# cbs228/sameold

Hardware: AMD Instinct MI355X
Metric: Msamples/s demodulated (batched 22.05 kHz channels) + % HBM roofline, 1/8 GPU (higher is better)
Workload: dtype f32

## Files before the change

sameold_amd/csrc/same_batch.cpp:

```cpp
#include <hip/hip_runtime.h>

#include <algorithm>
#include <chrono>
#include <cstdarg>
#include <cstdio>
#include <cstdlib>
#include <condition_variable>
#include <cstring>
#include <deque>
#include <functional>
#include <mutex>
#include <new>
#include <string>
#include <thread>
#include <utility>
#include <vector>

#include "../../include/same_rx.h"
#include "same_config.h"
#include "same_device.h"
#include "same_hipmem.h"
#include "same_launch.h"
#include "same_resets.h"
#include "same_transport.h"

namespace {

thread_local std::string g_last_error;

int fail(int code, const char *fmt, ...)
{
    char buf[512];
    va_list ap;
    va_start(ap, fmt);
    vsnprintf(buf, sizeof(buf), fmt, ap);
    va_end(ap);
    g_last_error = buf;
    return code;
}

#define HIP_TRY(expr)                                                                      \
    do {                                                                                   \
        hipError_t _e = (expr);                                                            \
        if (_e != hipSuccess)                                                              \
            return fail(SAME_EHIP, "%s failed: %s (%s:%d)", #expr, hipGetErrorString(_e),  \
                        __FILE__, __LINE__);                                               \
    } while (0)

}

struct QEvent {
    uint32_t kind, channel;
    uint64_t sample_counter, symbol_count;
    uint32_t len, aux, aux2;
    uint32_t n_bytes;
    uint64_t payload;
};
static_assert(sizeof(QEvent) == 48, "compact event record");
template <typename T>
struct PodQueue {
    T *buf = nullptr;
    size_t n = 0, cap = 0;
    size_t base = 0;
    ~PodQueue() { std::free(buf); }
    PodQueue() = default;
    PodQueue(const PodQueue &) = delete;
    PodQueue &operator=(const PodQueue &) = delete;
    size_t size() const { return n; }
    T *data() { return buf; }
    const T *data() const { return buf; }
    void clear() { base += n; n = 0; }
    size_t compact(size_t head)
    {
        if (head == 0) return 0;
        if (head < n) std::memmove(buf, buf + head, (n - head) * sizeof(T));
        n -= head;
        base += head;
        return 0;
    }
    T *grow(size_t extra)
    {
        if (n + extra > cap) {
            const size_t want = (n + extra) + (n + extra) / 2 + 64;
            void *p = std::realloc(buf, want * sizeof(T));
            if (!p) return nullptr;
            buf = static_cast<T *>(p);
            cap = want;
        }
        T *at = buf + n;
        n += extra;
        return at;
    }
};
using EventQueue = PodQueue<QEvent>;
struct AudioChunk {
    uint32_t channel, flags;
    uint64_t sample_counter, n;
    uint64_t at;
};
using ByteArena = PodQueue<uint8_t>;
#ifdef SAME_HOST_PROF
#include <x86intrin.h>
static uint64_t g_hp[8];
static const char *const g_hp_name[8] = {"range sort", "poll synthesis", "queue record + payload", "transport: burst", "transport: other", "after_event", "stitch scan", "-"};
struct HpScope { int k; uint64_t t0; explicit HpScope(int k_) : k(k_), t0(__rdtsc()) {} ~HpScope() { g_hp[k] += __rdtsc() - t0; } };
#define HP(k) HpScope hp_scope_##k(k)
#else
#define HP(k) do {} while (0)
#endif
struct HarvestPart {
    std::vector<QEvent> out;
    std::vector<uint8_t> bytes;
    std::vector<uint32_t> rearm;
    std::vector<uint32_t> bursts;
};
static void materialise(const QEvent &q, const uint8_t *arena, size_t arena_base, same_rx_event *ev)
{
    std::memset(ev, 0, sizeof(*ev));
    ev->kind = q.kind; ev->channel = q.channel; ev->sample_counter = q.sample_counter; ev->symbol_count = q.symbol_count;
    ev->len = q.len; ev->aux = q.aux; ev->aux2 = q.aux2;
    if (q.n_bytes) std::memcpy(ev->bytes, arena + (q.payload - arena_base), q.n_bytes);
}

using same::TickSynth;

class WorkerPool {
public:
    ~WorkerPool()
    {
        { std::lock_guard<std::mutex> g(mu_); stop_ = true; }
        cv_.notify_all();
        for (std::thread &t : threads_) t.join();
    }
    void run(size_t n, const std::function<void(size_t)> &fn)
    {
        if (n <= 1) { if (n) fn(0); return; }
        while (threads_.size() + 1 < n) threads_.emplace_back([this] { loop(); });
        {
            std::lock_guard<std::mutex> g(mu_);
            fn_ = &fn; next_ = 0; count_ = n; pending_ = n; ++generation_;
        }
        cv_.notify_all();
        work();
        std::unique_lock<std::mutex> lk(mu_);
        done_.wait(lk, [this] { return pending_ == 0; });
        fn_ = nullptr;
    }

private:
    void work()
    {
        for (;;) {
            size_t i;
            const std::function<void(size_t)> *fn;
            {
                std::lock_guard<std::mutex> g(mu_);
                if (!fn_ || next_ >= count_) return;
                i = next_++; fn = fn_;
            }
            (*fn)(i);
            std::lock_guard<std::mutex> g(mu_);
            if (--pending_ == 0) done_.notify_all();
        }
    }
    void loop()
    {
        uint64_t seen = 0;
        for (;;) {
            {
                std::unique_lock<std::mutex> lk(mu_);
                cv_.wait(lk, [&] { return stop_ || generation_ != seen; });
                if (stop_) return;
                seen = generation_;
            }
            work();
        }
    }
    std::vector<std::thread> threads_;
    std::mutex mu_;
    std::condition_variable cv_, done_;
    const std::function<void(size_t)> *fn_ = nullptr;
    size_t next_ = 0, count_ = 0, pending_ = 0;
    uint64_t generation_ = 0;
    bool stop_ = false;
};

struct same_batch {
    same_rx_builder builder{};
    same::Params P{};
    same::State S{};
    int device = 0;
    uint32_t flags = 0;
    uint64_t counter = 0;
    hipStream_t own_stream = nullptr;
    hipStream_t last_stream = nullptr;
    same::DevBuf<float4> d_taps;
    same::DevBuf<void> d_state_blob;
    struct Slot {
        same::DevBuf<same::DevEvent> d_events;
        uint32_t event_cap() const { return (uint32_t)d_events.size(); }
        same::DevBuf<uint32_t> d_sort;
        same::PinnedBuf<uint32_t> h_sort;
        same::DevBuf<same::DevEvent> d_sorted;
        uint32_t sort_bins = 0;
        same::DevBuf<uint8_t> d_bursts;
        uint32_t burst_cap() const { return (uint32_t)(d_bursts.size() / same::kBurstCap); }
        same::DevBuf<uint32_t> d_counters;
        same::MappedBuf<uint32_t> h_counters;
        same::Event ev_start, ev_stop, ev_done, ev_planned;
        same::Event ev_k0, ev_k1;
        bool have_k = false;
        bool timed = false;
        same::PinnedBuf<void> h_events, h_bursts;
        bool in_flight = false;
        uint64_t seq = 0;
        uint64_t end_counter = 0;
        bool chunked = false;
        same::ChunkGeom geom{};
        uint64_t end_blocks = 0;
        same::DevBuf<uint64_t> d_handover;
        same::PinnedBuf<uint64_t> h_handover;
        bool per_channel = false;
        same::DevBuf<uint32_t> d_geom;
        same::PinnedBuf<uint32_t> h_geom;
        same::CoherentBuf<uint32_t> h_reset;
        same::CoherentBuf<uint32_t> h_counts;
        same::PinnedBuf<uint64_t> h_wake_up;
        bool dev_transport = false;
        same::CoherentBuf<same::DevMessage> h_near;
        uint32_t near_cap() const { return (uint32_t)h_near.size(); }
        same::DevBuf<same::DevMessage> d_msgs;
        uint32_t msg_cap() const { return (uint32_t)d_msgs.size(); }
        same::PinnedBuf<void> h_msgs;
        bool captured = false;
        same::DevBuf<same::cap::Span> d_spans;
        uint32_t span_cap() const { return (uint32_t)d_spans.size(); }
        same::DevBuf<float> d_pool;
        same::DevBuf<same::cap::Cursors> d_cap_cur;
        same::MappedBuf<same::cap::Cursors> h_cap_cur;
        same::PinnedBuf<void> h_spans, h_pool;
    } slot[2];
    struct TimePar {
        bool enabled = false;
        uint32_t max_chunks = 0, min_own = 0, warmup = 0;
        uint32_t cap_columns = 0;
        uint32_t carved_columns = 0;
        int carved_family = -1;
        same::Params Pv{};
        same::State Sv{};
        same::DevBuf<void> blob;
        same::DevBuf<void> blob_fresh;
        size_t fresh_bytes = 0;
        same::DevBuf<same::StateArrayDesc> d_desc_in, d_desc_out;
        uint32_t n_desc = 0;
        same::DevBuf<uint32_t> d_final_col;
        same::DevBuf<float> d_energy;
        same::DevBuf<float> d_hist;
        same::Event ev_plan_prev; bool plan_recorded = false;
        int knob_plan_stream = 0;
        int sort_mode = -1;
        uint32_t last_chunks = 1;
        bool last_per_channel = false;
        same::Family family = same::Family::kPipe;
        int knob_prologue = 0;
        std::vector<int64_t> sym_off;
        std::vector<TickSynth> synth;
    } tp;
    uint64_t launch_seq = 0;
    hipStream_t copy_stream = nullptr;
    struct Windowed {
        bool on = false;
        uint32_t window = 0;
        uint32_t fill = 0;
        same::DevBuf<void> d_buf;
        same::Event ev_buf;
        hipStream_t buf_stream = nullptr; bool buf_used = false;
        same::Event ev_read[2];
        uint64_t n_reads = 0;
        hipStream_t read_stream = nullptr;
    } inv;
    hipStream_t plan_stream = nullptr;
    float last_ms = 0.0f;
    bool overflowed = false;
    std::string record_path;
    bool kernel_fault = false;
    same::Request want;
    same::Mode mode;
    same::Choice plain;
    same::Params Pfm{};
    same::Family last_family = same::Family::kGeneric;
    bool sym_launched = false;
    bool debug = false;
    int host_threads = 0;
    same::DevBuf<void> d_stage, d_stage2;
    same::DevBuf<void> d_upload;
    same::DevBuf<void> d_zero;
    same::Event ev_order;
    bool timing = false;
    bool have_timing = false;
    float last_demod_ms = 0.0f;
    EventQueue queue;
    size_t queue_head = 0;
    ByteArena arena;
    std::vector<same_rx_event> peeked;
    bool peeked_valid = false;
    bool peeked_release = false;
    size_t peeked_head = 0;
    std::vector<size_t> burst_seq;
    size_t burst_seq_head = 0;
    std::vector<HarvestPart> parts;
    WorkerPool workers;
    std::vector<same::TransportHot> thot;
    std::vector<same::TransportCold> tcold;
    same::TransportRef tr(uint32_t c) { return same::TransportRef(thot[c], tcold[c]); }
    same::PinnedBuf<uint64_t> h_wake;
    bool wake_ordered = false;
    std::vector<uint32_t> ragged_by;
    bool messages_only = false;
    bool dev_transport = false;
    bool last_dev_transport = false;
    same::DevBuf<void> d_thot, d_tcold;
    same::ResetLedger resets;
    std::vector<uint32_t> reset_list, reset_now, reset_cols;
    struct Audio {
        size_t per_launch = 0;
        same::DevBuf<same::cap::Rec> d_rec;
        std::vector<uint8_t> open;
        uint64_t flush_at = UINT64_MAX;
        PodQueue<AudioChunk> queue;
        size_t head = 0;
        PodQueue<float> samples;
        std::vector<same_audio_chunk> view;
    } audio;
};

static void release_stale_view(same_batch *rx);

namespace {

struct Carver {
    size_t off = 0;
    template <typename T> size_t take(size_t n)
    {
        off = (off + 255) & ~size_t(255);
        size_t o = off;
        off += n * sizeof(T);
        return o;
    }
};

#define SAME_STATE_ARRAYS(X, P)                                                                            \
    X(dc_ff_ring, float, (P).dc_len) X(dc_fb_ring, float, (P).dc_len)                                        \
    X(dc_sum0, float, 1) X(dc_sum1, float, 1) X(agc_gain, float, 1)                                          \
    X(win_ring, float, (P).win_ring)                                                                         \
    X(ted_clock, uint32_t, 1) X(until_next_ted, float, 1)                                                    \
    X(ted_h0, float, 1) X(ted_h1, float, 1) X(ted_h2, float, 1)                                              \
    X(period_avg, float, 1) X(period_inst, float, 1)                                                         \
    X(sq_data, uint32_t, 1) X(sq_power, float, 1) X(sq_phist, uint32_t, 1)                                   \
    X(sq_fill, uint32_t, 1) X(sq_clock, int32_t, 1) X(sq_symbols, uint64_t, 1)                               \
    X(sq_hist, float, same::kSquelchHist)                                                                    \
    X(eq_ffc, float, (P).eq_nff) X(eq_fbc, float, (P).eq_nfb)                                                \
    X(eq_ffw, float, (P).eq_nff) X(eq_fbw, float, (P).eq_nfb)                                                \
    X(eq_word, uint32_t, 1) X(eq_count, uint32_t, 1)                                                         \
    X(eq_snap_ffc, float, (P).eq_nff) X(eq_snap_fbc, float, (P).eq_nfb)                                      \
    X(eq_snap_ffw, float, (P).eq_nff) X(eq_snap_fbw, float, (P).eq_nfb)                                      \
    X(fr_word, uint32_t, 1) X(fr_count, uint32_t, 1) X(fr_invalid, uint32_t, 1) X(fr_len, uint32_t, 1)       \
    X(flags, uint32_t, 1)                                                                                    \
    X(tk_next, uint64_t, 1) X(tk_last, uint64_t, 1) X(tk_ring, uint64_t, same::kTickRing)                    \
    X(tk_n, uint32_t, 1) X(wake_sample, uint64_t, 1) X(wake_fired, uint64_t, 1)

size_t carve_state(const same::Params &P, char *base, same::State &S)
{
    const size_t C = P.n_channels;
    Carver cv;
#define CARVE(field, type, count) \
    do { size_t o = cv.take<type>(count); if (base) S.field = reinterpret_cast<type *>(base + o); } while (0)
#define CARVE_ROWS(field, type, rows) CARVE(field, type, (size_t)(rows) * C);
    SAME_STATE_ARRAYS(CARVE_ROWS, P)
#undef CARVE_ROWS
    CARVE(fr_msg, uint8_t, (size_t)same::kBurstCap * C);
    if (P.trace_cap) {
        CARVE(trace_n, uint32_t, C);
        CARVE(trace, float, (size_t)P.trace_cap * 4 * C);
        CARVE(trace_idx, uint64_t, (size_t)P.trace_cap * C);
    }
#undef CARVE
    return (cv.off + 255) & ~size_t(255);
}

void list_state_arrays(const same::Params &P, const same::State &src, const same::State &dst,
                       std::vector<same::StateArrayDesc> &out)
{
    out.clear();
#define DESC_ROWS(field, type, rows)                                                                     \
    out.push_back(same::StateArrayDesc{reinterpret_cast<char *>(src.field), reinterpret_cast<char *>(dst.field), \
                                       (uint32_t)(rows), (uint32_t)(sizeof(type) / 4)});
    SAME_STATE_ARRAYS(DESC_ROWS, P)
#undef DESC_ROWS
    static_assert(same::kBurstCap % 4 == 0, "framer rows are copied in words");
    out.push_back(same::StateArrayDesc{reinterpret_cast<char *>(src.fr_msg), reinterpret_cast<char *>(dst.fr_msg), 1u,
                                       (uint32_t)(same::kBurstCap / 4)});
}

void read_knobs(same_batch *rx)
{
    auto num = [](const char *name, int unset) { const char *e = std::getenv(name); return e ? std::atoi(e) : unset; };
    auto tri = [](const char *name) { const char *e = std::getenv(name); return e ? (std::atoi(e) ? 1 : -1) : 0; };
    rx->P.knob_pipe = tri("SAME_PIPE");
    rx->P.knob_pipe_lanes = num("SAME_PIPE_LANES", 0);
    rx->P.knob_pipe_split = tri("SAME_PIPE_SPLIT");
#ifdef SAME_PROFILE
    rx->P.knob_mirror = tri("SAME_MIRROR");
    rx->P.knob_pipe_share = tri("SAME_PIPE_SHARE");
    rx->P.knob_prio = num("SAME_PIPE_PRIO", 0);
#endif
    rx->P.knob_fast_dense = tri("SAME_FAST_DENSE");
    rx->P.knob_sym = tri("SAME_SYM");
    rx->want.sym_max_channels = (uint32_t)std::max(0, num("SAME_SYM_MAX", 1 << 30));
    rx->debug = std::getenv("SAME_DEBUG") != nullptr;
    { const char *e = std::getenv("SAME_RECORD_HARVEST"); rx->record_path = e ? e : ""; }
    rx->host_threads = std::max(0, num("SAME_HOST_THREADS", 0));
    rx->tp.sort_mode = num("SAME_TP_SORT", -1);
    rx->tp.knob_plan_stream = tri("SAME_TP_PLAN_STREAM");
    rx->tp.knob_prologue = tri("SAME_TP_PROLOGUE");
    rx->want.knob_relaxed = tri("SAME_RELAXED");
    { const char *e = std::getenv("SAME_RELAXED_KERNEL"); rx->P.knob_relaxed_kernel = !e ? 0 : (std::strcmp(e, "solo") == 0 ? 1 : (std::strcmp(e, "duo") == 0 ? 2 : 0)); }
    { const char *e = std::getenv("SAME_TP_KERNEL"); rx->want.knob_tp_kernel = !e ? 0 : (std::strcmp(e, "wave") == 0 ? 2 : (std::strcmp(e, "pipe") == 0 ? 1 : 0)); }
}

int ensure_output(same_batch *rx, same_batch::Slot &sl, size_t n_samples, same::Output &O, size_t n_columns = 0)
{
    const size_t n_ch = n_columns ? n_columns : rx->P.n_channels;
    const double symbols = (double)n_samples * 520.83 / (double)rx->P.input_rate;
    const size_t per_chan_events = (size_t)(symbols / 8.0) + 16;
    const size_t per_chan_bursts = (size_t)(symbols / 160.0) + 4;
    size_t ecap = std::min<size_t>(per_chan_events * n_ch, 0x7fffffffu / sizeof(same::DevEvent));
    size_t bcap = std::min<size_t>(per_chan_bursts * n_ch, 0x7fffffffu / same::kBurstCap);
    HIP_TRY(sl.d_events.ensure(ecap));
    HIP_TRY(sl.d_bursts.ensure(bcap * same::kBurstCap));
    if (rx->dev_transport && !n_columns) {
        HIP_TRY(sl.d_msgs.ensure(std::min<size_t>(bcap + 2 * n_ch, 0x7fffffffu / sizeof(same::DevMessage))));
        if (!sl.h_near) HIP_TRY(sl.h_near.ensure(std::max<uint32_t>(4096u, (uint32_t)(n_ch / 4u))));
        if (rx->audio.per_launch)
            HIP_TRY(sl.d_spans.ensure(std::min<size_t>(n_ch + (size_t)sl.near_cap() + sl.msg_cap(), 0x7fffffffu / sizeof(same::cap::Span))));
    }
    HIP_TRY(sl.d_sorted.ensure(sl.d_events.size()));
    HIP_TRY(sl.d_sort.ensure(2 * n_ch + 1 + same::event_sort_extra_words((uint32_t)n_ch)));
    HIP_TRY(sl.h_sort.ensure(n_ch + 1));
    sl.sort_bins = (uint32_t)n_ch;
    O.events = sl.d_events; O.event_cap = sl.event_cap();
    O.bursts = sl.d_bursts; O.burst_cap = sl.burst_cap();
    O.n_events = sl.d_counters; O.n_bursts = sl.d_counters + 1; O.overflow = sl.d_counters + 2;
    return SAME_OK;
}

template <typename SampleT>
hipError_t launch_family(same::Family f, const same::Params &P, const same::State &S, const same::Output &O, const float4 *taps, const SampleT *x,
                         uint32_t n_blocks, uint64_t counter0, hipStream_t stream, const same::PipeChunks &pc = same::PipeChunks{})
{
    switch (f) {
    case same::Family::kSym: return same::launch_demod_sym(P, S, O, taps, x, n_blocks, counter0, stream, pc);
    case same::Family::kPipeFastmath: return same::launch_demod_pipe(P, S, O, taps, x, n_blocks, counter0, stream, pc, true);
    case same::Family::kPipe: return same::launch_demod_pipe(P, S, O, taps, x, n_blocks, counter0, stream, pc, false);
    case same::Family::kWaveRelaxed: return same::launch_demod_relaxed(P, S, O, taps, x, n_blocks, counter0, stream, pc);
    case same::Family::kFast: return same::launch_demod_fast(P, S, O, taps, x, n_blocks, counter0, stream);
    case same::Family::kGeneric: break;
    }
    return hipErrorInvalidValue;
}

void reset_channel_host(same_batch *rx, uint32_t c, uint64_t pos)
{
    if (!rx->thot.empty()) rx->tr(c).reset();
    if (rx->tp.enabled) {
        rx->tp.sym_off[c] = 0;
        rx->tp.synth[c].reset();
        rx->tp.synth[c].a_t = pos;
    }
    if (rx->h_wake) rx->h_wake[c] = 0;
}

int launch_pending_resets(same_batch *rx, same_batch::Slot &sl, hipStream_t stream)
{
    if (rx->resets.device.empty()) return SAME_OK;
    std::vector<uint32_t> &cols = rx->reset_cols;
    rx->resets.take_device(cols);
    const uint32_t n = (uint32_t)cols.size();
    if (n > sl.h_reset.size()) HIP_TRY(sl.h_reset.ensure(std::max<uint32_t>(256u, n + n / 2u)));
    std::memcpy(sl.h_reset, cols.data(), (size_t)n * sizeof(uint32_t));
    hipError_t e = same::launch_reset_columns(rx->P, rx->S, sl.h_reset.dev(), n, stream);
    if (e == hipSuccess && rx->dev_transport)
        e = same::launch_transport_reset(rx->d_thot, rx->d_tcold, rx->P.n_channels, sl.h_reset.dev(), n, 0, stream, rx->audio.d_rec);
    if (e != hipSuccess) return fail(SAME_EHIP, "channel reset launch failed: %s", hipGetErrorString(e));
    return SAME_OK;
}

void prepare_queue_append(same_batch *rx)
{
    rx->peeked_valid = false;
    release_stale_view(rx);
    if (rx->queue_head && rx->queue_head >= rx->queue.size() - rx->queue_head) {
        rx->queue_head = rx->queue.compact(rx->queue_head);
        size_t keep_from = rx->arena.base + rx->arena.size();
        for (size_t i = 0; i < rx->queue.size(); ++i)
            if (rx->queue.data()[i].n_bytes) { keep_from = (size_t)rx->queue.data()[i].payload; break; }
        rx->arena.compact(keep_from - rx->arena.base);
    }
}

struct HarvestTimes { std::chrono::steady_clock::time_point sorted, replayed; uint32_t n_threads = 1; };
struct HarvestInput {
    const uint32_t *first;
    same::DevEvent *events;
    const uint8_t *bursts;
    const uint64_t *handover;
    const uint32_t *geom;
};
int harvest_host(same_batch *rx, same_batch::Slot &sl, const HarvestInput &in, uint32_t n_events, uint32_t n_bursts, std::vector<uint32_t> &rearm,
                 HarvestTimes &times)
{
    const bool dbg = rx->debug;
    const same::DevEvent *evs = in.events;
    const uint8_t *bursts = in.bursts;
    const uint32_t n_ch = rx->P.n_channels;
    const uint32_t n_bins = sl.chunked ? sl.geom.n_chunks * n_ch : n_ch;
    std::vector<uint32_t> first(in.first, in.first + n_bins + 1u);
    same::DevEvent *evs_mut = in.events;
    const uint32_t n_real = first[n_bins];
    if (n_real > n_events) return fail(SAME_EHIP, "internal: event sort counted %u of %u events", n_real, n_events);
    struct Identity { uint32_t operator[](uint32_t i) const { return i; } } order;
    if (dbg && sl.chunked && sl.per_channel) {
        const same::ChunkGeom &g = sl.geom;
        const uint32_t *own = in.geom, *rows = in.geom + n_bins;
        double len_sum = 0, run_sum = 0; uint64_t len_max = 0, run_max = 0, n_len = 0, n_run = 0, n_inf = 0, n_late = 0;
        uint32_t worst_c = 0;
        for (uint32_t k = 0; k + 1u < g.n_chunks; ++k)
            for (uint32_t c = 0; c < n_ch; ++c) {
                const uint64_t end = own[(size_t)(k + 1u) * n_ch + c], len = end - rows[(size_t)k * n_ch + c];
                len_sum += (double)len; if (len > len_max) { len_max = len; worst_c = c; } ++n_len;
                const uint64_t h = in.handover[(size_t)k * n_ch + c];
                if (h == same::kNoHandover) { ++n_inf; continue; }
                const uint64_t run = h - g.counter0 > end ? h - g.counter0 - end : 0;
                run_sum += (double)run; run_max = std::max(run_max, run); ++n_run; n_late += run > 2u * g.block_len;
            }
        std::fprintf(stderr, "[same] longest piece on channel %u, its cuts:", worst_c);
        for (uint32_t k = 0; k < g.n_chunks; ++k) std::fprintf(stderr, " %u", own[(size_t)k * n_ch + worst_c]);
        std::fprintf(stderr, "\n");
        std::fprintf(stderr, "[same] per-channel chunks: length mean %.0f max %llu samples; run-on mean %.0f max %llu, %llu of %llu columns ran on "
                             "more than two blocks, %llu never handed over\n", len_sum / std::max<uint64_t>(n_len, 1), (unsigned long long)len_max,
                     run_sum / std::max<uint64_t>(n_run, 1), (unsigned long long)run_max, (unsigned long long)n_late, (unsigned long long)n_run,
                     (unsigned long long)n_inf);
    }
    std::vector<uint32_t> chan_first;
    if (sl.chunked) {
        chan_first.assign(n_ch + 1u, 0u);
        for (uint32_t k = 0; k < sl.geom.n_chunks; ++k)
            for (uint32_t c = 0; c < n_ch; ++c) chan_first[c + 1u] += first[k * n_ch + c + 1u] - first[k * n_ch + c];
        for (uint32_t c = 0; c < n_ch; ++c) chan_first[c + 1u] += chan_first[c];
    }
    const std::vector<uint32_t> &cfirst = sl.chunked ? chan_first : first;
    const bool link_only = (rx->flags & SAME_BATCH_LINK_ONLY) != 0;
    const bool tp = rx->tp.enabled;
    times.sorted = std::chrono::steady_clock::now();

    using Part = HarvestPart;
    const double sps = (double)rx->P.input_rate / 520.83;
    const uint64_t interburst = same::max_interburst_symbols(), history = same::max_history_duration();
    const bool msgs_only = rx->messages_only;
    auto push_transport = [&](Part &part, const same_rx_event &tev, uint32_t c) {
        if (msgs_only && tev.kind != SAME_TRANSPORT_MSG_START && tev.kind != SAME_TRANSPORT_MSG_END) return;
        QEvent q{};
        q.kind = tev.kind; q.channel = c; q.sample_counter = rx->resets.rebase(c, tev.sample_counter); q.symbol_count = tev.symbol_count;
        q.len = tev.len; q.aux = tev.aux; q.aux2 = tev.aux2;
        q.n_bytes = std::min<uint32_t>(tev.len, SAME_EVENT_MAX_BYTES);
        if (tev.kind != SAME_TRANSPORT_MSG_START) q.n_bytes = 0;
        q.payload = part.bytes.size();
        if (q.n_bytes) part.bytes.insert(part.bytes.end(), tev.bytes, tev.bytes + q.n_bytes);
        part.out.push_back(q);
    };
    auto feed = [&](Part &part, same_rx_event &tev, const same::DevEvent &d, uint32_t c, int64_t off) {
        const uint64_t sym = (uint64_t)((int64_t)d.symbol_count + off);
        auto poll = [&](uint64_t psym, uint64_t pt) {
            if (rx->tr(c).on_link_event(same::kDevTick, pt, psym, nullptr, 0, rx->P.input_rate, &tev)) push_transport(part, tev, c);
        };
        if (tp && !link_only) {
            HP(1);
            rx->tp.synth[c].run_until(sym, d.sample_counter, sps, rx->tr(c).force_eom_at(), poll);
        }
        QEvent q{};
        const uint8_t *payload = nullptr;
        {
        HP(2);
        q.kind = d.kind; q.channel = c; q.sample_counter = rx->resets.rebase(c, d.sample_counter); q.symbol_count = sym;
        if (d.kind == SAME_LINK_BURST) {
            q.len = d.burst_len;
            if (d.burst_slot < n_bursts) {
                q.n_bytes = std::min<uint32_t>(d.burst_len, SAME_EVENT_MAX_BYTES);
                payload = bursts + (size_t)d.burst_slot * same::kBurstCap;
                q.payload = part.bytes.size();
                if (!msgs_only) part.bytes.insert(part.bytes.end(), payload, payload + q.n_bytes);
            } else {
                q.len = 0;
            }
            if (!msgs_only) part.bursts.push_back((uint32_t)part.out.size());
        }
        if (d.kind <= SAME_LINK_BURST && !msgs_only) part.out.push_back(q);
        }
        if (!link_only) {
#ifdef SAME_HOST_PROF
            HpScope hp_tr(d.kind == SAME_LINK_BURST ? 3 : 4);
#endif
            if (rx->tr(c).on_link_event(d.kind, d.sample_counter, sym, payload, q.n_bytes, rx->P.input_rate, &tev)) push_transport(part, tev, c);
            if (!tp && rx->tr(c).force_eom_dirty()) part.rearm.push_back(c);
        }
        { HP(5); if (tp && d.kind <= SAME_LINK_BURST) rx->tp.synth[c].after_event(d.kind, sym, d.sample_counter, interburst, history); }
    };
    auto stitch = [&](Part &part, same_rx_event &ev, uint32_t c) {
        const same::ChunkGeom &g = sl.geom;
        const uint64_t *hand = in.handover;
        const uint32_t *own = sl.per_channel ? in.geom : nullptr, *rows = sl.per_channel ? in.geom + n_bins : nullptr;
        auto owner_of = [&](uint64_t h) -> uint32_t {
            if (!own) return g.owner_of(h);
            uint32_t k = 0;
            while (k + 1u < g.n_chunks && g.counter0 + own[(size_t)(k + 1u) * n_ch + c] <= h) ++k;
            return k;
        };
        TickSynth &ts = rx->tp.synth[c];
        int64_t off = rx->tp.sym_off[c];
        uint32_t cur = 0;
        uint64_t keep_after = 0;
        for (;;) {
            const uint32_t col = cur * n_ch + c;
            const uint64_t h = hand[col];
            const uint64_t upto = std::min(h, sl.end_blocks);
            bool rebased = cur == 0;
            for (uint32_t i = first[col]; i < first[col + 1u]; ++i) {
                const same::DevEvent &d = evs[order[i]];
                if (d.sample_counter <= keep_after) continue;
                if (d.sample_counter > upto) break;
                if (!rebased) {
                    const int64_t est = (int64_t)ts.a_sym + (int64_t)((double)(d.sample_counter - ts.a_t) / sps + 0.5);
                    off = est - (int64_t)d.symbol_count;
                    rebased = true;
                }
                feed(part, ev, d, c, off);
            }
            if (!rebased) {
                const uint64_t row0 = rows ? g.counter0 + rows[col] : g.counter0 + (uint64_t)cur * g.stride_blocks * g.block_len;
                const int64_t est_end = (int64_t)ts.a_sym + (int64_t)((double)(sl.end_blocks - ts.a_t) / sps + 0.5);
                off = est_end - (int64_t)((double)(sl.end_blocks - row0) / sps + 0.5);
            }
            if (h == same::kNoHandover) break;
            const uint32_t nxt = owner_of(h);
            if (nxt <= cur) break;
            const uint32_t ncol = nxt * n_ch + c;
            uint32_t st = 0, j = first[ncol];
            for (; j < first[ncol + 1u] && evs[order[j]].sample_counter <= h; ++j)
                if (evs[order[j]].kind <= SAME_LINK_BURST) st = evs[order[j]].kind;
            keep_after = h;
            if (st == SAME_LINK_READING || st == SAME_LINK_BURST) {
                for (; j < first[ncol + 1u]; ++j)
                    if (evs[order[j]].kind == SAME_LINK_NO_CARRIER) { keep_after = evs[order[j]].sample_counter; break; }
            } else if (st == SAME_LINK_SEARCHING && ts.link == SAME_LINK_NO_CARRIER) {
                same::DevEvent inj{};
                inj.channel = ncol; inj.kind = SAME_LINK_SEARCHING; inj.sample_counter = h;
                inj.symbol_count = ts.a_sym + (uint64_t)((double)(h > ts.a_t ? h - ts.a_t : 0) / sps + 0.5);
                inj.burst_slot = 0xffffffffu;
                feed(part, ev, inj, c, 0);
            }
            cur = nxt;
        }
        for (uint32_t i = first[c]; i < first[c + 1u]; ++i)
            if (evs[order[i]].sample_counter > sl.end_blocks) feed(part, ev, evs[order[i]], c, off);
        rx->tp.sym_off[c] = off;
    };
    auto run_range = [&](uint32_t c0, uint32_t c1, Part &part) {
        part.out.clear(); part.bytes.clear(); part.rearm.clear(); part.bursts.clear();
        part.out.reserve((size_t)(cfirst[c1] - cfirst[c0]) * 3 / 2 + 4);
        same_rx_event ev;
        std::memset(&ev, 0, sizeof(ev));
        for (uint32_t c = c0; c < c1; ++c) {
            if (!link_only && c + 1u < c1) {
                __builtin_prefetch(&rx->thot[c + 1u]);
                if (!sl.chunked) {
                    bool burst = false;
                    for (uint32_t k = first[c + 1u]; k < first[c + 2u]; ++k) burst |= evs[k].kind == SAME_LINK_BURST;
                    const char *nx = reinterpret_cast<const char *>(&rx->tcold[c + 1u]);
                    if (burst) for (size_t o = 0; o < sizeof(same::TransportCold); o += 64) __builtin_prefetch(nx + o);
                }
            }
            { HP(0);
            for (uint32_t col = c; col < n_bins; col += n_ch)
                if (first[col + 1u] - first[col] > 1u)
                    std::sort(evs_mut + first[col], evs_mut + first[col + 1u],
                              [](const same::DevEvent &a, const same::DevEvent &b) { return a.channel < b.channel; });
            }
            if (sl.chunked) stitch(part, ev, c);
            else
                for (uint32_t k = first[c]; k < first[c + 1u]; ++k)
                    feed(part, ev, evs[order[k]], c, tp ? rx->tp.sym_off[c] : 0);
            if (tp && !link_only) {
                TickSynth &ts = rx->tp.synth[c];
                if (ts.link == SAME_LINK_NO_CARRIER && sl.end_counter > ts.a_t) {
                    const uint64_t sym_end = ts.a_sym + (uint64_t)((double)(sl.end_counter - ts.a_t) / sps);
                    auto poll = [&](uint64_t psym, uint64_t pt) {
                        if (rx->tr(c).on_link_event(same::kDevTick, pt, psym, nullptr, 0, rx->P.input_rate, &ev)) push_transport(part, ev, c);
                    };
                    ts.run_until(sym_end + 1u, sl.end_counter + 1u, sps, rx->tr(c).force_eom_at(), poll);
                }
            }
        }
    };
    uint32_t n_threads = 1;
    if (n_real >= 16384u && n_ch >= 64u) {
        const unsigned hw = std::thread::hardware_concurrency();
        n_threads = std::min<uint32_t>({32u, std::max(16u, hw / 8u), hw ? hw : 1u, n_ch / 32u});
        if (rx->host_threads > 0) n_threads = (uint32_t)rx->host_threads;
    }
    if (rx->parts.size() < n_threads) rx->parts.resize(n_threads);
    std::vector<Part> &parts = rx->parts;
    for (Part &p : parts) { p.out.clear(); p.bytes.clear(); p.rearm.clear(); p.bursts.clear(); }
    if (n_threads == 1) {
        run_range(0, n_ch, parts[0]);
    } else {
        std::vector<uint32_t> cut(n_threads + 1u, n_ch);
        cut[0] = 0;
        for (uint32_t t = 1; t < n_threads; ++t) {
            const uint32_t target = (uint32_t)((uint64_t)n_real * t / n_threads);
            cut[t] = (uint32_t)(std::lower_bound(cfirst.begin(), cfirst.end(), target) - cfirst.begin());
            cut[t] = std::min(std::max(cut[t], cut[t - 1u]), n_ch);
        }
        rx->workers.run(n_threads, [&](size_t t) { run_range(cut[t], cut[t + 1u], parts[t]); });
    }
    times.replayed = std::chrono::steady_clock::now();
    times.n_threads = n_threads;
    size_t total = 0, total_bytes = 0;
    for (const Part &p : parts) { total += p.out.size(); total_bytes += p.bytes.size(); }
    prepare_queue_append(rx);
    QEvent *dst = rx->queue.grow(total);
    if (total && !dst) return fail(SAME_ENOMEM, "event queue");
    uint8_t *bdst = rx->arena.grow(total_bytes);
    if (total_bytes && !bdst) return fail(SAME_ENOMEM, "event payloads");
    {
        size_t at = 0, bat = 0;
        if (rx->burst_seq_head > 4096 && rx->burst_seq_head * 2 > rx->burst_seq.size()) {
            rx->burst_seq.erase(rx->burst_seq.begin(), rx->burst_seq.begin() + (std::ptrdiff_t)rx->burst_seq_head);
            rx->burst_seq_head = 0;
        }
        const size_t seq0 = rx->queue.base + (size_t)(dst - rx->queue.data());
        const size_t byte0 = rx->arena.base + (size_t)(bdst - rx->arena.data());
        struct Job { QEvent *q; uint8_t *b; Part *p; size_t byte_off; };
        std::vector<Job> jobs;
        for (size_t t = 0; t < parts.size(); ++t) {
            Part &p = parts[t];
            if (p.out.empty()) continue;
            for (uint32_t i : p.bursts) rx->burst_seq.push_back(seq0 + at + i);
            jobs.push_back(Job{dst + at, bdst + bat, &p, byte0 + bat});
            at += p.out.size(); bat += p.bytes.size();
        }
        rx->workers.run(jobs.size(), [&](size_t j) {
            const Job &job = jobs[j];
            for (QEvent &q : job.p->out) q.payload += job.byte_off;
            std::memcpy(job.q, job.p->out.data(), job.p->out.size() * sizeof(QEvent));
            if (!job.p->bytes.empty()) std::memcpy(job.b, job.p->bytes.data(), job.p->bytes.size());
// ... 46 lines not shown
        const uint64_t keep_from = A.queue.size() ? A.queue.data()[0].at : A.samples.base + A.samples.size();
        A.samples.compact((size_t)(keep_from - A.samples.base));
    }
    AudioChunk *dst = A.queue.grow(n_chunks);
    if (n_chunks && !dst) return nullptr;
    float *sdst = A.samples.grow(n_samples);
    if (n_samples && !sdst) { A.queue.n -= n_chunks; return nullptr; }
    *samples_at = sdst;
    *at = A.samples.base + (A.samples.size() - n_samples);
    return dst;
}

int audio_end_reset(same_batch *rx, const std::vector<uint32_t> &chans, uint64_t pos)
{
    same_batch::Audio &A = rx->audio;
    if (!A.per_launch) return SAME_OK;
    size_t n = 0;
    for (uint32_t c : chans) n += A.open[c];
    if (!n) return SAME_OK;
    float *sdst = nullptr;
    uint64_t at = 0;
    AudioChunk *dst = audio_grow(rx, n, 0, &sdst, &at);
    if (!dst) return fail(SAME_ENOMEM, "audio queue");
    for (uint32_t c : chans) {
        if (!A.open[c]) continue;
        *dst++ = AudioChunk{c, SAME_AUDIO_END_RESET, rx->resets.rebase(c, pos), 0, at};
        A.open[c] = 0;
    }
    return SAME_OK;
}

int harvest_audio(same_batch *rx, same_batch::Slot &sl)
{
    sl.captured = false;
    same_batch::Audio &A = rx->audio;
    const same::cap::Cursors cur = *sl.h_cap_cur.get();
    if (cur.overflow) rx->overflowed = true;
    const uint32_t n_spans = std::min(cur.n_spans, sl.span_cap());
    if (!n_spans) return SAME_OK;
    const size_t used = (size_t)std::min<unsigned long long>(cur.pool_used, (unsigned long long)A.per_launch);
    HIP_TRY(grow_pinned(sl.h_spans, (size_t)n_spans * sizeof(same::cap::Span)));
    HIP_TRY(hipMemcpyAsync(sl.h_spans, sl.d_spans, (size_t)n_spans * sizeof(same::cap::Span), hipMemcpyDeviceToHost, rx->copy_stream));
    if (used) {
        HIP_TRY(grow_pinned(sl.h_pool, used * sizeof(float)));
        HIP_TRY(hipMemcpyAsync(sl.h_pool, sl.d_pool, used * sizeof(float), hipMemcpyDeviceToHost, rx->copy_stream));
    }
    HIP_TRY(hipStreamSynchronize(rx->copy_stream));
    const same::cap::Span *sp = static_cast<const same::cap::Span *>(sl.h_spans.get());
    const float *pool = static_cast<const float *>(sl.h_pool.get());
    std::vector<uint32_t> order(n_spans);
    size_t n_samples = 0;
    for (uint32_t i = 0; i < n_spans; ++i) {
        order[i] = i;
        if (sp[i].n && sp[i].off + sp[i].n <= used) n_samples += sp[i].n;
    }
    std::sort(order.begin(), order.end(), [&](uint32_t a, uint32_t b) { return sp[a].channel != sp[b].channel ? sp[a].channel < sp[b].channel : a < b; });
    float *sdst = nullptr;
    uint64_t at = 0;
    AudioChunk *dst = audio_grow(rx, n_spans, n_samples, &sdst, &at);
    if (!dst) return fail(SAME_ENOMEM, "audio queue");
    for (uint32_t k = 0; k < n_spans; ++k) {
        const same::cap::Span &s = sp[order[k]];
        const uint32_t n = s.n && s.off + s.n <= used ? s.n : 0;
        uint32_t flags = s.flags;
        if (n < s.n) flags |= SAME_AUDIO_TRUNCATED;
        dst[k] = AudioChunk{s.channel, flags, rx->resets.rebase(s.channel, s.counter), n, at};
        if (n) { std::memcpy(sdst, pool + s.off, (size_t)n * sizeof(float)); sdst += n; at += n; }
        if (flags & SAME_AUDIO_FIRST) A.open[s.channel] = 1;
        if (flags & (SAME_AUDIO_END_MESSAGE | SAME_AUDIO_END_FLUSH | SAME_AUDIO_END_RESET)) A.open[s.channel] = 0;
    }
    if (rx->debug)
        std::fprintf(stderr, "[same] audio: %u chunks, %zu samples (pool %zu of %zu)%s\n", n_spans, n_samples, used, A.per_launch,
                     cur.overflow ? ", truncated" : "");
    return SAME_OK;
}

int harvest_messages(same_batch *rx, same_batch::Slot &sl, std::chrono::steady_clock::time_point t_begin,
                     std::chrono::steady_clock::time_point t_waited)
{
    const uint32_t n_msgs = std::min(sl.h_counters[3], sl.near_cap() + sl.msg_cap());
    const uint32_t n_near = std::min(n_msgs, sl.near_cap()), n_far = n_msgs - n_near;
    const size_t far_bytes = (size_t)n_far * sizeof(same::DevMessage);
    if (n_far) {
        HIP_TRY(grow_pinned(sl.h_msgs, far_bytes));
        HIP_TRY(hipMemcpyAsync(sl.h_msgs, sl.d_msgs, far_bytes, hipMemcpyDeviceToHost, rx->copy_stream));
        HIP_TRY(hipStreamSynchronize(rx->copy_stream));
    }
    auto t_copied = std::chrono::steady_clock::now();
    const same::DevMessage *far = static_cast<const same::DevMessage *>(sl.h_msgs.get());
    auto rec = [&](uint32_t i) -> const same::DevMessage & { return i < n_near ? sl.h_near[i] : far[i - n_near]; };
    std::vector<uint32_t> order(n_msgs);
    size_t n_bytes = 0;
    for (uint32_t i = 0; i < n_msgs; ++i) {
        order[i] = i;
        if (rec(i).kind == SAME_TRANSPORT_MSG_START) n_bytes += std::min<uint32_t>(rec(i).len, same::kDevMessageText);
    }
    std::sort(order.begin(), order.end(), [&](uint32_t a, uint32_t b) {
        const same::DevMessage &x = rec(a), &y = rec(b);
        return x.channel != y.channel ? x.channel < y.channel : x.seq < y.seq;
    });
    prepare_queue_append(rx);
    QEvent *dst = rx->queue.grow(n_msgs);
    if (n_msgs && !dst) return fail(SAME_ENOMEM, "event queue");
    uint8_t *bdst = rx->arena.grow(n_bytes);
    if (n_bytes && !bdst) return fail(SAME_ENOMEM, "event payloads");
    size_t at = n_bytes ? rx->arena.base + (size_t)(bdst - rx->arena.data()) : 0;
    for (uint32_t k = 0; k < n_msgs; ++k) {
        const same::DevMessage &d = rec(order[k]);
        QEvent q{};
        q.kind = d.kind; q.channel = d.channel; q.sample_counter = rx->resets.rebase(d.channel, d.sample_counter);
        q.symbol_count = d.symbol_count; q.len = d.len; q.aux = d.aux; q.aux2 = d.aux2;
        if (d.kind == SAME_TRANSPORT_MSG_START && d.len) {
            q.n_bytes = std::min<uint32_t>(d.len, same::kDevMessageText);
            q.payload = at;
            std::memcpy(bdst, d.text, q.n_bytes);
            bdst += q.n_bytes; at += q.n_bytes;
        }
        dst[k] = q;
    }
    if (sl.captured) {
        const int arc = harvest_audio(rx, sl);
        if (arc) return arc;
    }
    const int si = (int)(&sl - rx->slot);
    rx->resets.shift_due(si);
    rx->resets.done_shift(si);
    if (const int arc = audio_end_reset(rx, rx->resets.slot[si & 1].channels, rx->resets.rec_pos(si))) return arc;
    for (uint32_t c : rx->resets.host_due(si)) reset_channel_host(rx, c, rx->resets.rec_pos(si));
    rx->resets.done_host(si);
    if (rx->debug) {
        auto t_end = std::chrono::steady_clock::now();
        auto ms = [](auto a, auto b) { return std::chrono::duration<double, std::milli>(b - a).count(); };
        std::fprintf(stderr, "[same] harvest timing: wait %.2f ms, copy %.2f ms, %u messages queued in %.2f ms (transport layer on the device)\n",
                     ms(t_begin, t_waited), ms(t_waited, t_copied), n_msgs, ms(t_copied, t_end));
    }
    return SAME_OK;
}

int upload_wake_ordered(same_batch *rx, same_batch::Slot &sl)
{
    const uint32_t C = rx->P.n_channels;
    HIP_TRY(sl.h_wake_up.ensure(C));
    same_batch::Slot &other = rx->slot[(&sl - rx->slot) ^ 1];
    const int oi = (int)(&other - rx->slot);
    for (uint32_t c = 0; c < C; ++c) {
        const uint64_t w = rx->h_wake[c];
        sl.h_wake_up[c] = w && other.in_flight ? w + rx->resets.pending_shift(oi, c) : w;
    }
    if (other.in_flight) {
        HIP_TRY(hipMemcpyAsync(rx->S.wake_sample, sl.h_wake_up, (size_t)C * sizeof(uint64_t), hipMemcpyHostToDevice, rx->last_stream));
        HIP_TRY(hipEventRecord(other.ev_done, rx->last_stream));
    } else {
        HIP_TRY(hipMemcpyAsync(rx->S.wake_sample, sl.h_wake_up, (size_t)C * sizeof(uint64_t), hipMemcpyHostToDevice, rx->copy_stream));
        HIP_TRY(hipStreamSynchronize(rx->copy_stream));
    }
    return SAME_OK;
}

int harvest_slot(same_batch *rx, same_batch::Slot &sl)
{
    if (!sl.in_flight) return SAME_OK;
    const bool dbg = rx->debug;
    auto t_begin = std::chrono::steady_clock::now();
    HIP_TRY(hipEventSynchronize(sl.ev_done));
    sl.in_flight = false;
    if (sl.timed) {
        HIP_TRY(hipEventElapsedTime(&rx->last_ms, sl.ev_start, sl.ev_stop));
        rx->last_demod_ms = rx->last_ms;
        if (sl.have_k) HIP_TRY(hipEventElapsedTime(&rx->last_demod_ms, sl.ev_k0, sl.ev_k1));
        rx->have_timing = true;
    }
    auto t_waited = std::chrono::steady_clock::now();
    const uint32_t n_events = std::min(sl.h_counters[0], sl.event_cap());
    if (dbg)
        std::fprintf(stderr, "[same] harvest: %u device events (%u bursts), cap %u/%u\n", sl.h_counters[0],
                     sl.h_counters[1], sl.event_cap(), sl.burst_cap());
    const uint32_t n_bursts = std::min(sl.h_counters[1], sl.burst_cap());
    if (sl.h_counters[2] & (3u | same::kMessageLogOverflow)) rx->overflowed = true;
    if (sl.h_counters[2] & 4u) rx->kernel_fault = true;
    if (sl.dev_transport) return harvest_messages(rx, sl, t_begin, t_waited);
    const size_t ev_bytes = (size_t)n_events * sizeof(same::DevEvent), bu_bytes = (size_t)n_bursts * same::kBurstCap;
    HIP_TRY(grow_pinned(sl.h_events, ev_bytes));
    HIP_TRY(grow_pinned(sl.h_bursts, bu_bytes));
    const uint32_t n_ch = rx->P.n_channels;
    const uint32_t n_bins = sl.chunked ? sl.geom.n_chunks * n_ch : n_ch;
    if (n_bins != sl.sort_bins) return fail(SAME_EINVAL, "internal: event sort made for %u columns, launch has %u", sl.sort_bins, n_bins);
    HIP_TRY(hipMemcpyAsync(sl.h_sort, sl.d_sort + n_bins, ((size_t)n_bins + 1) * sizeof(uint32_t), hipMemcpyDeviceToHost, rx->copy_stream));
    if (n_events) HIP_TRY(hipMemcpyAsync(sl.h_events, sl.d_sorted, ev_bytes, hipMemcpyDeviceToHost, rx->copy_stream));
    HIP_TRY(hipStreamSynchronize(rx->copy_stream));
    if (n_bursts) HIP_TRY(hipMemcpyAsync(sl.h_bursts, sl.d_bursts, bu_bytes, hipMemcpyDeviceToHost, rx->copy_stream));
    if (sl.chunked) {
        HIP_TRY(hipMemcpyAsync(sl.h_handover, sl.d_handover, (size_t)n_bins * sizeof(uint64_t), hipMemcpyDeviceToHost, rx->copy_stream));
        if (sl.per_channel)
            HIP_TRY(hipMemcpyAsync(sl.h_geom, sl.d_geom, (size_t)2 * n_bins * sizeof(uint32_t), hipMemcpyDeviceToHost, rx->copy_stream));
    }
    if (n_bursts || sl.chunked) HIP_TRY(hipStreamSynchronize(rx->copy_stream));
    auto t_copied = std::chrono::steady_clock::now();
    if (!rx->record_path.empty()) { const int rrc = record_harvest(rx, sl, n_events, n_bursts, rx->record_path.c_str()); if (rrc != SAME_OK) return rrc; }
    std::vector<uint32_t> rearm;
    HarvestTimes times;
    const HarvestInput in{sl.h_sort, static_cast<same::DevEvent *>(sl.h_events.get()), static_cast<const uint8_t *>(sl.h_bursts.get()),
                          sl.h_handover, sl.h_geom};
    int rc = harvest_host(rx, sl, in, n_events, n_bursts, rearm, times);
    if (rc) return rc;
    {
        const int si = (int)(&sl - rx->slot);
        const same::ResetLedger::SlotShift &sh = rx->resets.shift_due(si);
        if (!rx->thot.empty())
            for (size_t i = 0; i < sh.channels.size(); ++i)
                if (rx->tr(sh.channels[i]).shift_force_eom(sh.by[i])) rearm.push_back(sh.channels[i]);
        rx->resets.done_shift(si);
    }
    {
        const int si = (int)(&sl - rx->slot);
        const std::vector<uint32_t> &due = rx->resets.host_due(si);
        for (uint32_t c : due) reset_channel_host(rx, c, rx->resets.rec_pos(si));
        rx->resets.done_host(si);
    }
    if (!rearm.empty()) {
        if (!rx->h_wake) {
            HIP_TRY(rx->h_wake.ensure(rx->P.n_channels));
            std::memset(rx->h_wake, 0, (size_t)rx->P.n_channels * sizeof(uint64_t));
        }
        for (uint32_t c : rearm) rx->h_wake[c] = rx->tr(c).force_eom_at();
        if (rx->wake_ordered) {
            int rc2 = upload_wake_ordered(rx, sl);
            if (rc2) return rc2;
        } else {
        HIP_TRY(hipMemcpyAsync(rx->S.wake_sample, rx->h_wake, (size_t)rx->P.n_channels * sizeof(uint64_t), hipMemcpyHostToDevice, rx->copy_stream));
        HIP_TRY(hipStreamSynchronize(rx->copy_stream));
        }
    }
    if (dbg) {
        auto t_end = std::chrono::steady_clock::now();
        auto ms = [](auto a, auto b) { return std::chrono::duration<double, std::milli>(b - a).count(); };
        std::fprintf(stderr, "[same] harvest timing: wait %.2f ms, copy %.2f ms, sort %.2f ms, replay on %u threads %.2f ms, "
                             "queue %.2f ms\n",
                     ms(t_begin, t_waited), ms(t_waited, t_copied), ms(t_copied, times.sorted), times.n_threads,
                     ms(times.sorted, times.replayed), ms(times.replayed, t_end));
    }
    return SAME_OK;
}

int harvest(same_batch *rx)
{
    same_batch::Slot *order[2] = {&rx->slot[0], &rx->slot[1]};
    if (order[0]->seq > order[1]->seq) std::swap(order[0], order[1]);
    for (same_batch::Slot *sl : order) {
        int rc = harvest_slot(rx, *sl);
        if (rc) return rc;
    }
    return SAME_OK;
}

uint32_t plan_chunks(same_batch *rx, size_t n, same::ChunkGeom &geom, same::PipeChunks &pc, uint32_t column_cap = same::kTpColumnCap, bool channel_major = false)
{
    same_batch::TimePar &tp = rx->tp;
    const uint32_t C = rx->P.n_channels;
    const double sps = (double)rx->P.input_rate / 520.83;
    auto fill = [&](uint32_t K, uint32_t fb) -> bool {
        const uint32_t warm = tp.warmup ? tp.warmup : (uint32_t)(64.0 * sps + 0.5);
        const uint32_t WB = (warm + fb - 1u) / fb;
        const uint64_t TB = n / fb;
        if (TB <= WB) return false;
        const uint64_t SB = (TB - WB) / K;
        const uint64_t min_own = tp.min_own ? tp.min_own : 4ull * WB * fb;
        if (SB == 0 || SB * fb < min_own) return false;
        geom.counter0 = rx->counter;
        geom.n_chunks = K; geom.block_len = fb; geom.stride_blocks = (uint32_t)SB; geom.warmup_blocks = WB;
        pc.n_chunks = K; pc.in_channels = C; pc.stride_blocks = (uint32_t)SB; pc.nominal_blocks = (uint32_t)SB + WB;
        pc.handover = nullptr;
        return true;
    };
    const same::TpRule rule = same::tp_rule(rx->P, rx->mode, rx->want, tp.max_chunks, column_cap, channel_major);
    for (uint32_t K = rule.k_max; K >= 2u; --K) {
        same::Choice c;
        if (same::tp_candidate(rx->P, rule, K, c) && fill(K, c.block_len)) { tp.family = c.family; return K; }
    }
    return 1;
}

int ensure_handover(same_batch::Slot &sl, uint32_t columns)
{
    HIP_TRY(sl.d_handover.ensure(columns));
    HIP_TRY(sl.h_handover.ensure(columns));
    return SAME_OK;
}

int ensure_wide_state(same_batch *rx, uint32_t columns)
{
    same_batch::TimePar &tp = rx->tp;
    if (tp.carved_columns == columns && tp.carved_family == (int)tp.family) return SAME_OK;
    int rc = harvest(rx);
    if (rc) return rc;
    HIP_TRY(hipDeviceSynchronize());
    tp.Pv = same::wide_params(rx->P, columns, same::is_fastmath(tp.family), same::tp_more_than_one_round(columns));
    if (columns > tp.cap_columns) {
        tp.cap_columns = 0;
        HIP_TRY(tp.blob.reset());
        HIP_TRY(tp.blob_fresh.reset());
        const size_t bytes = carve_state(tp.Pv, nullptr, tp.Sv);
        HIP_TRY(tp.blob.ensure(bytes));
        HIP_TRY(hipMemset(tp.blob, 0, bytes));
        HIP_TRY(tp.blob_fresh.ensure(bytes));
        tp.cap_columns = columns;
    }
    const size_t blob_bytes = carve_state(tp.Pv, (char *)tp.blob.get(), tp.Sv);
    {
        same::State Sf{};
        carve_state(tp.Pv, (char *)tp.blob_fresh.get(), Sf);
        HIP_TRY(hipMemset(tp.blob_fresh, 0, blob_bytes));
        HIP_TRY(same::launch_init_state(tp.Pv, Sf, 0, nullptr, 0));
        HIP_TRY(hipDeviceSynchronize());
        tp.fresh_bytes = (size_t)(reinterpret_cast<char *>(tp.Sv.fr_msg) - static_cast<char *>(tp.blob.get()));
    }
    std::vector<same::StateArrayDesc> in, out;
    list_state_arrays(rx->P, rx->S, tp.Sv, in);
    list_state_arrays(rx->P, tp.Sv, rx->S, out);
    tp.n_desc = (uint32_t)in.size();
    HIP_TRY(tp.d_desc_in.ensure(in.size()));
    HIP_TRY(tp.d_desc_out.ensure(out.size()));
    HIP_TRY(tp.d_final_col.ensure(rx->P.n_channels));
    HIP_TRY(hipMemcpy(tp.d_desc_in, in.data(), in.size() * sizeof(same::StateArrayDesc), hipMemcpyHostToDevice));
    HIP_TRY(hipMemcpy(tp.d_desc_out, out.data(), out.size() * sizeof(same::StateArrayDesc), hipMemcpyHostToDevice));
    tp.carved_columns = columns;
    tp.carved_family = (int)tp.family;
    return SAME_OK;
}

struct Ragged {
    const uint32_t *counts = nullptr;
    uint32_t m = 0;
    uint32_t row_off = 0;
};

struct RaggedLaunch {
    uint32_t row0 = 0;
    size_t n_lock = 0;
};


int begin_launch(same_batch *rx, same_batch::Slot &sl, const same_batch::Slot &prev, hipStream_t stream)
{
    int rc = harvest_slot(rx, sl);
    if (rc) return rc;
    if (prev.in_flight && rx->last_stream != stream) HIP_TRY(hipStreamWaitEvent(stream, prev.ev_done, 0));
    return launch_pending_resets(rx, sl, stream);
}

int begin_timing(same_batch *rx, same_batch::Slot &sl, hipStream_t stream)
{
    sl.timed = rx->timing;
    if (sl.timed) HIP_TRY(hipEventRecord(sl.ev_start, stream));
    return SAME_OK;
}

int tp_reserve(same_batch *rx, same_batch::Slot &sl, uint32_t columns, size_t n, const same::PipeChunks &pc, uint32_t block_len, same::Output &O)
{
    int rc = ensure_wide_state(rx, columns);
    if (rc) return rc;
    rc = ensure_output(rx, sl, std::min<size_t>(n, 3 * (size_t)pc.nominal_blocks * block_len + 65536), O, columns);
    if (rc) return rc;
    return ensure_handover(sl, columns);
}

int tp_start(same_batch *rx, same_batch::Slot &sl, uint32_t columns, const char *layout, hipStream_t stream, bool *sort_bins_empty)
{
    same_batch::TimePar &tp = rx->tp;
    const uint32_t C = rx->P.n_channels;
    *sort_bins_empty = false;
    if (tp.knob_prologue >= 0) {
        HIP_TRY(same::launch_tp_prologue(tp.blob, tp.blob_fresh, tp.fresh_bytes, sl.d_handover, sl.d_sort, columns, sl.d_counters, stream));
        *sort_bins_empty = sl.sort_bins == columns;
    } else {
        HIP_TRY(same::launch_counters(sl.d_counters, sl.h_counters.dev(), 0, stream));
        HIP_TRY(same::launch_init_state(tp.Pv, tp.Sv, 0, stream, C));
        HIP_TRY(same::launch_fill_u64(sl.d_handover, columns, same::kNoHandover, stream));
    }
    if (rx->debug) std::fprintf(stderr, "[same] time-parallel launch: %u columns (%s), start-up: %s\n", columns, layout,
                                tp.knob_prologue >= 0 ? "prologue kernel" : "separate launches");
    HIP_TRY(same::launch_copy_state_columns(tp.d_desc_in, tp.n_desc, C, columns, nullptr, C, stream));
    return SAME_OK;
}

int tp_hand_back(same_batch *rx, same_batch::Slot &sl, const same::ChunkGeom &geom, const uint32_t *own_start, hipStream_t stream)
{
    same_batch::TimePar &tp = rx->tp;
    const uint32_t C = rx->P.n_channels;
    if (own_start) HIP_TRY(same::launch_chunk_final_column_pc(sl.d_handover, own_start, C, geom.n_chunks, rx->counter, tp.d_final_col, stream));
    else HIP_TRY(same::launch_chunk_final_column(sl.d_handover, C, geom, tp.d_final_col, stream));
    HIP_TRY(same::launch_copy_state_columns(tp.d_desc_out, tp.n_desc, geom.n_chunks * C, C, tp.d_final_col, C, stream));
    return SAME_OK;
}

template <typename SampleT>
int demod_tail(same_batch *rx, const same::Output &O, const SampleT *rows, size_t n, uint64_t counter0, hipStream_t stream)
{
    const hipError_t e = same::launch_demod(rx->P, rx->S, O, rx->d_taps, rows, (uint32_t)n, counter0, stream);
    if (e != hipSuccess) return fail(SAME_EHIP, "demod kernel launch failed: %s", hipGetErrorString(e));
    return SAME_OK;
}
int demod_tail_corner(same_batch *rx, const same::Output &O, const float *corner, size_t pitch, size_t r, uint64_t counter0, hipStream_t stream)
{
    const uint32_t C = rx->P.n_channels;
    HIP_TRY(rx->d_stage.ensure(r * C * sizeof(float)));
    HIP_TRY(rx->d_stage2.ensure(r * C * sizeof(float)));
    float *staged = static_cast<float *>(rx->d_stage.get()), *rows = static_cast<float *>(rx->d_stage2.get());
    HIP_TRY(hipMemcpy2DAsync(staged, r * sizeof(float), corner, pitch * sizeof(float), r * sizeof(float), C, hipMemcpyDeviceToDevice, stream));
    const hipError_t e = same::launch_transpose(staged, rows, C, (uint32_t)r, stream);
    if (e != hipSuccess) return fail(SAME_EHIP, "demod kernel launch failed: %s", hipGetErrorString(e));
    return demod_tail(rx, O, rows, r, counter0, stream);
}

template <typename SampleT>
int end_launch(same_batch *rx, same_batch::Slot &sl, same_batch::Slot &prev, hipStream_t stream, const SampleT *rows, size_t n,
               bool sort_bins_empty, const RaggedLaunch *rl = nullptr)
{
    if (sl.timed) HIP_TRY(hipEventRecord(sl.ev_stop, stream));
    HIP_TRY(same::launch_event_sort(sl.d_events, sl.d_counters, sl.event_cap(), sl.sort_bins, sl.d_sort, sl.d_sort + sl.sort_bins,
                                    sl.d_sorted, stream, sort_bins_empty));
    sl.dev_transport = rx->dev_transport && !sl.chunked;
    rx->last_dev_transport = sl.dev_transport;
    if (sl.dev_transport) {
        same::TransportLaunch T{};
        T.n_channels = rx->P.n_channels; T.input_rate = rx->P.input_rate;
        T.first = sl.d_sort + sl.sort_bins; T.sorted = sl.d_sorted; T.counters = sl.d_counters;
        T.bursts = sl.d_bursts; T.burst_cap = sl.burst_cap();
        T.hot = rx->d_thot; T.cold = rx->d_tcold; T.wake_sample = rx->S.wake_sample;
        T.near = sl.h_near.dev(); T.near_cap = sl.near_cap();
        T.log = sl.d_msgs; T.log_cap = sl.msg_cap(); T.log_cursor = sl.d_counters + 3; T.overflow = sl.d_counters + 2;
        sl.captured = rx->audio.per_launch != 0;
        if (sl.captured) {
            same::cap::Launch &K = T.cap;
            const uint64_t fa = rx->audio.flush_at;
            K.start = rx->counter; K.n_rows = (uint32_t)n;
            K.flush_row = fa >= rx->counter + n ? same::cap::kNoFlush : (uint32_t)(fa > rx->counter ? fa - rx->counter : 0);
            K.rec = rx->audio.d_rec; K.spans = sl.d_spans; K.span_cap = sl.span_cap();
            K.n_spans = &sl.d_cap_cur->n_spans; K.pool_used = &sl.d_cap_cur->pool_used; K.pool_cap = rx->audio.per_launch;
            K.overflow = &sl.d_cap_cur->overflow;
        }
        if (rl && rl->n_lock < n)
            HIP_TRY(same::launch_transport_ragged(T, sl.h_counts.dev(), rl->row0, (uint32_t)n, stream));
        else
            HIP_TRY(same::launch_transport(T, stream));
        if (sl.captured) {
            const hipError_t e = same::launch_capture(sl.d_spans, sl.d_cap_cur, sl.span_cap(), sl.d_pool, rx->audio.per_launch, rows,
                                                      rx->P.n_channels, (uint32_t)n, sl.h_cap_cur.dev(), stream);
            if (e != hipSuccess) return fail(SAME_EHIP, "capture kernel launch failed: %s", hipGetErrorString(e));
        }
    }
    HIP_TRY(same::launch_counters(sl.d_counters, sl.h_counters.dev(), 1, stream));
    HIP_TRY(hipEventRecord(sl.ev_done, stream));
    sl.in_flight = true;
    sl.seq = ++rx->launch_seq;
    rx->last_stream = stream;
    if (rl) rx->resets.shift(rx->ragged_by.data(), rx->counter + n, (int)(&sl - rx->slot));
    rx->counter += n;
    sl.end_counter = rx->counter;
    return harvest_slot(rx, prev);
}

template <typename SampleT>
int process_time_major_launches(same_batch *rx, const SampleT *d_x, size_t n_samples, hipStream_t stream, const Ragged *rg = nullptr)
{
    const size_t kMaxChunk = std::min<size_t>((size_t)1 << 22, (size_t)rx->P.input_rate * 45);
    size_t done = 0;
    while (done < n_samples) {
        const size_t n = std::min(kMaxChunk, n_samples - done);
        same_batch::Slot &sl = rx->slot[rx->launch_seq & 1];
        same_batch::Slot &prev = rx->slot[(rx->launch_seq & 1) ^ 1];
        int rc = begin_launch(rx, sl, prev, stream);
        if (rc) return rc;
        size_t n_lock = n;
        if (rg) {
            const size_t row0 = (size_t)rg->row_off + done;
            n_lock = rg->m > row0 ? std::min<size_t>(rg->m - row0, n) : 0;
            const uint32_t C = rx->P.n_channels;
            HIP_TRY(sl.h_counts.ensure(C));
            std::memcpy(sl.h_counts, rg->counts, (size_t)C * sizeof(uint32_t));
            rx->ragged_by.resize(C);
            for (uint32_t c = 0; c < C; ++c) {
                const size_t have = rg->counts[c] > row0 ? std::min<size_t>(rg->counts[c] - row0, n) : 0;
                rx->ragged_by[c] = (uint32_t)(n - have);
            }
        }
        same::ChunkGeom geom{};
        same::PipeChunks pc{};
        const uint32_t n_chunks = rg ? 1u : plan_chunks(rx, n, geom, pc);
        rx->tp.last_chunks = n_chunks;
        sl.have_k = false;
        bool sort_bins_empty = false;
        same::Output O{};
        if (n_chunks > 1u) {
            const uint32_t C = rx->P.n_channels, columns = n_chunks * C;
            const size_t fbk = geom.block_len;
            rc = tp_reserve(rx, sl, columns, n, pc, geom.block_len, O);
            if (rc) return rc;
            pc.handover = sl.d_handover;
            same_batch::TimePar &tp = rx->tp;
            rc = begin_timing(rx, sl, stream);
            if (rc) return rc;
            rc = tp_start(rx, sl, columns, "time-major", stream, &sort_bins_empty);
            if (rc) return rc;
            const SampleT *xp = d_x + done * C;
            const uint32_t total_blocks = (uint32_t)(n / fbk);
            const hipError_t e = launch_family(tp.family, tp.Pv, tp.Sv, O, rx->d_taps, xp, total_blocks, rx->counter, stream, pc);
            rx->last_family = tp.family;
            if (e != hipSuccess) return fail(SAME_EHIP, "time-parallel demod kernel launch failed: %s", hipGetErrorString(e));
            rc = tp_hand_back(rx, sl, geom, nullptr, stream);
            if (rc) return rc;
            const size_t n_whole = (size_t)total_blocks * fbk;
            if (n_whole < n && (rc = demod_tail(rx, O, xp + n_whole * C, n - n_whole, rx->counter + n_whole, stream)) != SAME_OK) return rc;
            sl.chunked = true; sl.per_channel = false;
            sl.geom = geom;
            sl.end_blocks = rx->counter + n_whole;
            rx->tp.last_per_channel = false;
        } else {
        sl.chunked = false; sl.per_channel = false;
        rc = ensure_output(rx, sl, n, O);
        if (rc) return rc;
        HIP_TRY(same::launch_counters(sl.d_counters, sl.h_counters.dev(), 0, stream));
        rc = begin_timing(rx, sl, stream);
        if (rc) return rc;
        const SampleT *xp = d_x + done * rx->P.n_channels;
        hipError_t e = hipSuccess;
        const same::Choice &plain = rx->plain;
        const size_t fb = plain.block_len;
        const size_t n_fast = fb ? (n_lock / fb) * fb : 0;
        if (n_fast) {
            e = launch_family(plain.family, same::is_fastmath(plain.family) ? rx->Pfm : rx->P, rx->S, O, rx->d_taps, xp, (uint32_t)(n_fast / fb), rx->counter, stream);
            if (e != hipSuccess) return fail(SAME_EHIP, "%s launch failed: %s", same::family_name(plain.family, rx->P.block_len), hipGetErrorString(e));
            rx->sym_launched |= plain.family == same::Family::kSym;
        }
        rx->last_family = plain.family == same::Family::kSym && !rx->sym_launched ? same::Family::kPipeFastmath : plain.family;
        if (n_fast < n_lock &&
            (rc = demod_tail(rx, O, xp + n_fast * rx->P.n_channels, n_lock - n_fast, rx->counter + n_fast, stream)) != SAME_OK) return rc;
        if (n_lock < n) {
            e = same::launch_demod_ragged(rx->P, rx->S, O, rx->d_taps, xp + n_lock * rx->P.n_channels, (uint32_t)(n - n_lock), sl.h_counts.dev(),
                                          (uint32_t)(rg->row_off + done + n_lock), rx->counter + n_lock, stream);
            if (e != hipSuccess) return fail(SAME_EHIP, "ragged demod kernel launch failed: %s", hipGetErrorString(e));
        }
        }
        const RaggedLaunch rl{rg ? (uint32_t)(rg->row_off + done) : 0u, n_lock};
        rc = end_launch(rx, sl, prev, stream, d_x + done * rx->P.n_channels, n, sort_bins_empty, rg ? &rl : nullptr);
        if (rc) return rc;
        done += n;
    }
    return SAME_OK;
}

constexpr uint32_t kInvWindow = 18432;
constexpr uint32_t kInvWindowTimeParallel = 73728;
static int inv_buffer_wait(same_batch *rx, hipStream_t stream)
{
    same_batch::Windowed &iv = rx->inv;
    if (iv.buf_used && iv.buf_stream != stream) HIP_TRY(hipStreamWaitEvent(stream, iv.ev_buf, 0));
    return SAME_OK;
}
static int inv_buffer_done(same_batch *rx, hipStream_t stream)
{
    same_batch::Windowed &iv = rx->inv;
    HIP_TRY(iv.ev_buf.ensure());
    HIP_TRY(hipEventRecord(iv.ev_buf, stream));
    iv.buf_stream = stream; iv.buf_used = true;
    return SAME_OK;
}
static int inv_copy(const float *d_x, float *dst, size_t n, hipStream_t stream)
{
    HIP_TRY(hipMemcpyAsync(dst, d_x, n * sizeof(float), hipMemcpyDeviceToDevice, stream));
    return SAME_OK;
}
static int inv_copy(const int16_t *d_x, float *dst, size_t n, hipStream_t stream)
{
    const hipError_t e = same::launch_cast_i16_f32(d_x, dst, n, stream);
    if (e != hipSuccess) return fail(SAME_EHIP, "cast launch failed: %s", hipGetErrorString(e));
    return SAME_OK;
}
template <typename SampleT>
static int inv_append(same_batch *rx, const SampleT *d_x, size_t n, hipStream_t stream)
{
    same_batch::Windowed &iv = rx->inv;
    const size_t C = rx->P.n_channels;
    HIP_TRY(iv.d_buf.ensure((size_t)iv.window * C * sizeof(float)));
    int rc = inv_buffer_wait(rx, stream);
    if (rc) return rc;
    rc = inv_copy(d_x, static_cast<float *>(iv.d_buf.get()) + (size_t)iv.fill * C, n * C, stream);
    if (rc) return rc;
    iv.fill += (uint32_t)n;
    return inv_buffer_done(rx, stream);
}
static int inv_launch_waiting(same_batch *rx, hipStream_t stream)
{
    same_batch::Windowed &iv = rx->inv;
    if (!iv.fill) return SAME_OK;
    int rc = inv_buffer_wait(rx, stream);
    if (rc) return rc;
    const uint32_t n = iv.fill;
    iv.fill = 0;
    rc = process_time_major_launches<float>(rx, static_cast<const float *>(iv.d_buf.get()), n, stream);
    if (rc) return rc;
    return inv_buffer_done(rx, stream);
}
static int inv_reads_begin(same_batch *rx, hipStream_t stream)
{
    same_batch::Windowed &iv = rx->inv;
    if (iv.n_reads && iv.read_stream != stream) HIP_TRY(hipStreamWaitEvent(stream, iv.ev_read[(iv.n_reads - 1) & 1], 0));
    return SAME_OK;
}
static int inv_reads_end(same_batch *rx, hipStream_t stream)
{
    same_batch::Windowed &iv = rx->inv;
    same::Event &ev = iv.ev_read[iv.n_reads & 1];
    if (!ev) HIP_TRY(ev.ensure());
    else HIP_TRY(hipEventSynchronize(ev));
    HIP_TRY(hipEventRecord(ev, stream));
    iv.read_stream = stream;
    ++iv.n_reads;
    return SAME_OK;
}
static int inv_reads_wait(same_batch *rx)
{
    same_batch::Windowed &iv = rx->inv;
    if (iv.n_reads) HIP_TRY(hipEventSynchronize(iv.ev_read[(iv.n_reads - 1) & 1]));
    return SAME_OK;
}
template <typename SampleT>
int process_time_major(same_batch *rx, const SampleT *d_x, size_t n_samples, hipStream_t stream)
{
    same_batch::Windowed &iv = rx->inv;
    if (!iv.on) return process_time_major_launches(rx, d_x, n_samples, stream);
    const size_t C = rx->P.n_channels;
    size_t pos = 0;
    if (iv.fill) {
        const size_t take = std::min<size_t>(iv.window - iv.fill, n_samples);
        int rc = inv_append(rx, d_x, take, stream);
        if (rc) return rc;
        pos = take;
        if (iv.fill < iv.window) return SAME_OK;
        rc = inv_launch_waiting(rx, stream);
        if (rc) return rc;
    }
    while (n_samples - pos >= iv.window) {
        int rc = process_time_major_launches(rx, d_x + pos * C, iv.window, stream);
        if (rc) return rc;
        pos += iv.window;
    }
    if (pos < n_samples) return inv_append(rx, d_x + pos * C, n_samples - pos, stream);
    return SAME_OK;
}

int process_channel_major_native(same_batch *rx, const float *d_x, size_t n, hipStream_t stream)
{
    same_batch::TimePar &tp = rx->tp;
    if (!tp.enabled || n > ((size_t)1 << 22)) return 0;
    if (rx->P.ntaps != 42u) return 0;
    same::ChunkGeom geom{};
    same::PipeChunks pc{};
    const uint32_t n_chunks = plan_chunks(rx, n, geom, pc, same::tp_native_column_cap(rx->P, rx->mode, tp.max_chunks), true);
    if (n_chunks < 2u) return 0;
    const uint32_t C = rx->P.n_channels, columns = n_chunks * C, fb = geom.block_len;
    const bool wave = tp.family == same::Family::kWaveRelaxed;
    const same::Params Pv = same::wide_params(rx->P, columns, same::is_fastmath(tp.family), true);
    const size_t n_call = n;
    n -= n % fb;
    if (n_call % 4 != 0 || ((uintptr_t)d_x & 15u) != 0u || n < 64u * (size_t)same::tp_scout_block() || n / same::tp_scout_block() > 7000u || n_chunks > 63u || C % same::kWave != 0u) return 0;
    if (wave ? fb % 2 != 0 : (fb % 4 != 0 || same::pipe_workgroup_channels(Pv) != (uint32_t)same::kWave)) return 0;
    same_batch::Slot &sl = rx->slot[rx->launch_seq & 1];
    same_batch::Slot &prev = rx->slot[(rx->launch_seq & 1) ^ 1];
    int rc = begin_launch(rx, sl, prev, stream);
    if (rc) return rc;
    same::Output O{};
    rc = tp_reserve(rx, sl, columns, n, pc, fb, O);
    if (rc) return rc;
    HIP_TRY(sl.d_geom.ensure((size_t)5 * columns + 3 * (columns / same::kWave)));
    HIP_TRY(sl.h_geom.ensure((size_t)2 * columns));
    same::TpPlan plan{};
    plan.channels = C; plan.n_chunks = n_chunks; plan.block_len = fb;
    {
        const double sps = (double)rx->P.input_rate / 520.83;
        const uint32_t warm = tp.warmup ? tp.warmup : (uint32_t)(40.0 * sps + 0.5);
        plan.warmup_samples = std::min(geom.warmup_blocks, (warm + fb - 1u) / fb) * fb;
    }
    plan.whole_samples = (uint32_t)n; plan.in_samples = n_call;
    plan.scout_blocks = (uint32_t)(n / same::tp_scout_block());
    HIP_TRY(tp.d_energy.ensure((size_t)C * plan.scout_blocks));
    uint32_t *d_own = sl.d_geom, *d_row0 = sl.d_geom + columns, *d_nom = sl.d_geom + 2 * (size_t)columns,
             *d_perm = sl.d_geom + 3 * (size_t)columns, *d_wg = sl.d_geom + 4 * (size_t)columns,
             *d_wg2 = d_wg + columns / same::kWave, *d_perm2 = d_wg2 + 2 * (columns / same::kWave);
    const bool pair_groups = tp.sort_mode == 2 && tp.family == same::Family::kSym;
    const int sort_mode = pair_groups ? 0 : (tp.sort_mode >= 0 ? (tp.sort_mode ? 1 : 0) : (same::tp_more_than_one_round(columns) ? 1 : 0));
    rc = begin_timing(rx, sl, stream);
    if (rc) return rc;
    const bool lpt = sort_mode != 0 || pair_groups;
    const bool side = stream == rx->own_stream && tp.knob_plan_stream >= 0;
    hipStream_t ps = side ? rx->plan_stream : stream;
    if (tp.plan_recorded) HIP_TRY(hipStreamWaitEvent(ps, tp.ev_plan_prev, 0));
    HIP_TRY(same::launch_tp_plan(d_x, plan, tp.d_energy, d_own, d_row0, d_nom, d_perm, d_wg, sort_mode != 0, ps,
                                 lpt ? d_perm2 : nullptr, lpt ? d_wg2 : nullptr, pair_groups));
    HIP_TRY(tp.ev_plan_prev.ensure());
    HIP_TRY(hipEventRecord(tp.ev_plan_prev, ps));
    tp.plan_recorded = true;
    if (side) {
        HIP_TRY(hipEventRecord(sl.ev_planned, ps));
        HIP_TRY(hipStreamWaitEvent(stream, sl.ev_planned, 0));
    }
    if (lpt) { d_perm = d_perm2; d_wg = d_wg2; }
    bool sort_bins_empty = false;
    rc = tp_start(rx, sl, columns, "channel-major", stream, &sort_bins_empty);
    if (rc) return rc;
    pc.handover = sl.d_handover;
    pc.col_row0 = d_row0; pc.col_nominal = d_nom; pc.wg_blocks = d_wg; pc.col_perm = (sort_mode != 0 || pair_groups) ? d_perm : nullptr;
    pc.in_samples = n_call; pc.whole_samples = (uint32_t)n;
    pc.hist_scratch = nullptr;
    if (pc.col_perm && tp.family == same::Family::kSym) {
        HIP_TRY(tp.d_hist.ensure((size_t)columns * same::kSquelchHist));
        pc.hist_scratch = tp.d_hist;
    }
    sl.have_k = sl.timed;
    if (sl.timed) HIP_TRY(hipEventRecord(sl.ev_k0, stream));
    const hipError_t e = launch_family(tp.family, tp.Pv, tp.Sv, O, rx->d_taps, d_x, (uint32_t)(n / fb), rx->counter, stream, pc);
    rx->last_family = tp.family;
    if (e != hipSuccess) return fail(SAME_EHIP, "time-parallel demod kernel launch failed: %s", hipGetErrorString(e));
    if (sl.timed) HIP_TRY(hipEventRecord(sl.ev_k1, stream));
    rc = tp_hand_back(rx, sl, geom, d_own, stream);
    if (rc) return rc;
    if (n < n_call && (rc = demod_tail_corner(rx, O, d_x + n, n_call, n_call - n, rx->counter + n, stream)) != SAME_OK) return rc;
    sl.chunked = true; sl.per_channel = true;
    sl.geom = geom;
    sl.end_blocks = rx->counter + n;
    tp.last_chunks = n_chunks; tp.last_per_channel = true;
    rc = end_launch<float>(rx, sl, prev, stream, nullptr, n_call, sort_bins_empty);
    return rc ? rc : 1;
}
int process_channel_major_native(same_batch *, const int16_t *, size_t, hipStream_t) { return 0; }

template <typename SampleT, typename Launch>
int transpose_in_slabs(same_batch *rx, const SampleT *d_x, size_t pitch, size_t n_rows, hipStream_t stream, Launch &&launch)
{
    const uint32_t C = rx->P.n_channels;
    for (same_batch::Slot &sl : rx->slot)
        if (sl.in_flight && rx->last_stream != stream) HIP_TRY(hipStreamWaitEvent(stream, sl.ev_done, 0));
    const size_t slab = std::min<size_t>(n_rows, (size_t)65520);
    HIP_TRY(rx->d_stage2.ensure(slab * C * sizeof(SampleT)));
    for (size_t t0 = 0; t0 < n_rows; t0 += slab) {
        const size_t n = std::min(slab, n_rows - t0);
        HIP_TRY(rx->d_stage.ensure(n * C * sizeof(SampleT)));
        SampleT *staged = static_cast<SampleT *>(rx->d_stage.get()), *rows = static_cast<SampleT *>(rx->d_stage2.get());
        HIP_TRY(hipMemcpy2DAsync(staged, n * sizeof(SampleT), d_x + t0, pitch * sizeof(SampleT), n * sizeof(SampleT), C,
                                 hipMemcpyDeviceToDevice, stream));
        const hipError_t e = same::launch_transpose(staged, rows, C, (uint32_t)n, stream);
        if (e != hipSuccess) return fail(SAME_EHIP, "transpose launch failed: %s", hipGetErrorString(e));
        const int rc = launch(rows, n, t0);
        if (rc) return rc;
    }
    return SAME_OK;
}

template <typename SampleT>
int process_device_on(same_batch *rx, const SampleT *d_x, size_t n_samples, uint32_t layout, hipStream_t stream);
template <typename SampleT>
int process_device_any(same_batch *rx, const SampleT *d_x, size_t n_samples, uint32_t layout, void *hip_stream)
{
    if (!rx || (!d_x && n_samples)) return fail(SAME_EINVAL, "null argument");
    if (n_samples == 0) return SAME_OK;
    HIP_TRY(hipSetDevice(rx->device));
    hipStream_t stream = hip_stream == SAME_STREAM_OWN ? rx->own_stream : (hipStream_t)hip_stream;
    if (!rx->inv.on) return process_device_on(rx, d_x, n_samples, layout, stream);
    int rc = inv_reads_begin(rx, stream);
    if (rc == SAME_OK) rc = process_device_on(rx, d_x, n_samples, layout, stream);
    const int rc_end = inv_reads_end(rx, stream);
    return rc ? rc : rc_end;
}
template <typename SampleT>
int process_device_on(same_batch *rx, const SampleT *d_x, size_t n_samples, uint32_t layout, hipStream_t stream)
{
    if (layout == SAME_LAYOUT_TIME_MAJOR) return process_time_major(rx, d_x, n_samples, stream);
    if (layout != SAME_LAYOUT_CHANNEL_MAJOR) return fail(SAME_EINVAL, "unknown layout %u", layout);
    const int done = rx->inv.on ? 0 : process_channel_major_native(rx, d_x, n_samples, stream);
    if (done) return done < 0 ? done : SAME_OK;
    return transpose_in_slabs(rx, d_x, n_samples, n_samples, stream,
                              [&](const SampleT *rows, size_t n, size_t) { return process_time_major(rx, rows, n, stream); });
}

template <typename SampleT, typename Process>
int upload_in_slabs(same_batch *rx, const SampleT *h_x, size_t pitch, size_t n_rows, uint32_t layout, Process &&process)
{
    const size_t C = rx->P.n_channels;
    const size_t slab = std::max<size_t>(1, std::min<size_t>(n_rows, ((size_t)256 << 20) / (C * sizeof(SampleT))));
    HIP_TRY(rx->d_upload.ensure(slab * C * sizeof(SampleT)));
    SampleT *d_in = static_cast<SampleT *>(rx->d_upload.get());
    int rc = SAME_OK;
    for (size_t t0 = 0; t0 < n_rows && rc == SAME_OK; t0 += slab) {
        const size_t n = std::min(slab, n_rows - t0);
        if (rx->inv.on && (rc = inv_reads_wait(rx)) != SAME_OK) break;
        const hipError_t e = layout == SAME_LAYOUT_TIME_MAJOR
                                 ? hipMemcpy(d_in, h_x + t0 * C, n * C * sizeof(SampleT), hipMemcpyHostToDevice)
                                 : hipMemcpy2D(d_in, n * sizeof(SampleT), h_x + t0, pitch * sizeof(SampleT), n * sizeof(SampleT), C,
                                               hipMemcpyHostToDevice);
        if (e != hipSuccess) { rc = fail(SAME_EHIP, "upload failed: %s", hipGetErrorString(e)); break; }
        rc = process(d_in, n, t0);
        if (rc == SAME_OK) rc = harvest(rx);
    }
    if (rc == SAME_OK && rx->kernel_fault) return fail(SAME_EKERNEL, "a demodulation kernel's wavefronts lost step (internal hand-over timed out)");
    if (rc == SAME_OK && rx->overflowed) return fail(SAME_EOVERFLOW, "event/burst pool overflow");
    return rc;
}

template <typename SampleT>
int process_host_any(same_batch *rx, const SampleT *h_x, size_t n_samples, uint32_t layout)
{
    if (!rx || (!h_x && n_samples)) return fail(SAME_EINVAL, "null argument");
    if (n_samples == 0) return SAME_OK;
    HIP_TRY(hipSetDevice(rx->device));
    return upload_in_slabs(rx, h_x, n_samples, n_samples, layout, [&](const SampleT *d_in, size_t n, size_t) {
        return process_device_any(rx, d_in, n, layout, SAME_STREAM_OWN);
    });
}

int ragged_check(same_batch *rx, size_t n_rows, const uint32_t *counts, uint32_t layout, uint32_t *m_out, uint32_t *M_out)
{
    if (!rx) return fail(SAME_EINVAL, "null handle");
    if (!counts) return fail(SAME_EINVAL, "null counts");
    if (layout != SAME_LAYOUT_TIME_MAJOR && layout != SAME_LAYOUT_CHANNEL_MAJOR) return fail(SAME_EINVAL, "unknown layout %u", layout);
    if (rx->tp.enabled) return fail(SAME_EINVAL, "ragged calls: a SAME_BATCH_TIME_PARALLEL batch plans its cuts over one common row range");
    if (rx->inv.on) return fail(SAME_EINVAL, "ragged calls: SAME_BATCH_CALL_INVARIANT windows begin at positions of one common stream");
    if (rx->P.trace_cap) return fail(SAME_EINVAL, "ragged calls: SAME_BATCH_TRACE_SYMBOLS records batch sample positions");
    if (n_rows > 0xffffffffull) return fail(SAME_EINVAL, "ragged calls: n_rows beyond 2^32 - 1");
    uint32_t m = UINT32_MAX, M = 0;
    for (uint32_t c = 0; c < rx->P.n_channels; ++c) {
        if (counts[c] > n_rows) return fail(SAME_EINVAL, "counts[%u] = %u exceeds n_rows = %zu; nothing was consumed", c, counts[c], n_rows);
        m = std::min(m, counts[c]); M = std::max(M, counts[c]);
    }
    *m_out = m; *M_out = M;
    return SAME_OK;
}

template <typename SampleT>
int process_ragged_on(same_batch *rx, const SampleT *d_x, size_t pitch, size_t n_buf, size_t row_base, const uint32_t *counts,
                      uint32_t m, uint32_t M, uint32_t layout, hipStream_t stream)
{
    const size_t n_p = std::min<size_t>(M, row_base + n_buf) - row_base;
    Ragged rg; rg.counts = counts; rg.m = m;
    if (layout == SAME_LAYOUT_TIME_MAJOR) {
        if (m == M) return process_time_major_launches(rx, d_x, n_p, stream);
        rg.row_off = (uint32_t)row_base;
        return process_time_major_launches(rx, d_x, n_p, stream, &rg);
    }
    return transpose_in_slabs(rx, d_x, pitch, n_p, stream, [&](const SampleT *rows, size_t n, size_t t0) {
        if (m == M) return process_time_major_launches(rx, rows, n, stream);
        rg.row_off = (uint32_t)(row_base + t0);
        return process_time_major_launches(rx, rows, n, stream, &rg);
    });
}

template <typename SampleT>
int process_ragged_device(same_batch *rx, const SampleT *d_x, size_t n_rows, const uint32_t *counts, uint32_t layout, void *hip_stream)
{
    uint32_t m = 0, M = 0;
    int rc = ragged_check(rx, n_rows, counts, layout, &m, &M);
    if (rc) return rc;
    if (M == 0) return SAME_OK;
    if (!d_x) return fail(SAME_EINVAL, "null argument");
    if (m == M && M == n_rows) return process_device_any(rx, d_x, n_rows, layout, hip_stream);
    HIP_TRY(hipSetDevice(rx->device));
    hipStream_t stream = hip_stream == SAME_STREAM_OWN ? rx->own_stream : (hipStream_t)hip_stream;
    if (m != M) rx->wake_ordered = true;
    return process_ragged_on(rx, d_x, n_rows, n_rows, 0, counts, m, M, layout, stream);
}

template <typename SampleT>
int process_ragged_host(same_batch *rx, const SampleT *h_x, size_t n_rows, const uint32_t *counts, uint32_t layout)
{
    uint32_t m = 0, M = 0;
    int rc = ragged_check(rx, n_rows, counts, layout, &m, &M);
    if (rc) return rc;
    if (M == 0) return SAME_OK;
    if (!h_x) return fail(SAME_EINVAL, "null argument");
    if (m == M && M == n_rows) return process_host_any(rx, h_x, n_rows, layout);
    HIP_TRY(hipSetDevice(rx->device));
    if (m != M) rx->wake_ordered = true;
    rc = harvest(rx);
    if (rc) return rc;
    return upload_in_slabs(rx, h_x, n_rows, M, layout, [&](const SampleT *d_in, size_t n, size_t t0) {
        return process_ragged_on(rx, d_in, n, n, t0, counts, m, M, layout, rx->own_stream);
    });
}

}

extern "C" {

const char *same_last_error(void) { return g_last_error.c_str(); }

#ifndef SAME_SOURCE_HASH
#define SAME_SOURCE_HASH "unknown"
#endif
const char *same_rx_source_hash(void) { return "SAME_SOURCE_HASH=" SAME_SOURCE_HASH; }

int same_batch_new(const same_rx_builder *b, uint32_t n_channels, int device, uint32_t flags,
                   same_batch **out)
{
    if (!b || !out || n_channels == 0) return fail(SAME_EINVAL, "null builder/out or zero channels");
    *out = nullptr;
    int ndev = 0;
    if (hipGetDeviceCount(&ndev) != hipSuccess || ndev <= 0)
        return fail(SAME_ENODEVICE, "no HIP device visible (this library has no CPU path)");
    if (device < 0 || device >= ndev) return fail(SAME_ENODEVICE, "device %d out of range (%d visible)", device, ndev);
    same_batch *rx = new (std::nothrow) same_batch;
    if (!rx) return fail(SAME_ENOMEM, "out of memory");
    rx->builder = *b;
    rx->device = device;
    rx->flags = flags;
    rx->inv.on = (flags & SAME_BATCH_CALL_INVARIANT) != 0;
    rx->inv.window = (flags & SAME_BATCH_TIME_PARALLEL) ? kInvWindowTimeParallel : kInvWindow;
    if (const char *e = std::getenv("SAME_INV_WINDOW")) { const long v = std::atol(e); if (v >= 64 && v <= (1 << 22)) rx->inv.window = (uint32_t)v; }
    std::vector<float> taps;
    int rc = same::derive_params(*b, n_channels, rx->P, taps);
    if (rc) { delete rx; return fail(rc, "builder rejected (code %d)", rc); }
    read_knobs(rx);
    rx->P.trace_cap = (flags & SAME_BATCH_TRACE_SYMBOLS) ? 4096u : 0u;
    if ((flags & SAME_BATCH_TIME_PARALLEL) && (flags & SAME_BATCH_TRACE_SYMBOLS)) {
        delete rx;
        return fail(SAME_EINVAL, "SAME_BATCH_TIME_PARALLEL cannot record a symbol trace");
    }
    if ((flags & SAME_BATCH_MESSAGES_ONLY) && (flags & SAME_BATCH_LINK_ONLY)) {
        delete rx;
        return fail(SAME_EINVAL, "SAME_BATCH_MESSAGES_ONLY needs the transport layer that SAME_BATCH_LINK_ONLY skips");
    }
    rx->tp.enabled = (flags & SAME_BATCH_TIME_PARALLEL) != 0;
    rx->messages_only = (flags & SAME_BATCH_MESSAGES_ONLY) != 0;
    rx->dev_transport = rx->messages_only && !rx->tp.enabled;
    rx->P.ticks = ((flags & SAME_BATCH_LINK_ONLY) || rx->tp.enabled) ? 0u : 1u;
    rx->P.tick_interburst = (uint32_t)same::max_interburst_symbols();
    rx->P.tick_history = (uint32_t)same::max_history_duration();

    auto cleanup = [&](int code) { same_batch_free(rx); return code; };
#define TRY_OR_CLEAN(expr)                                                                     \
    do {                                                                                       \
        hipError_t _e = (expr);                                                                \
        if (_e != hipSuccess)                                                                  \
            return cleanup(fail(SAME_EHIP, "%s failed: %s", #expr, hipGetErrorString(_e)));    \
    } while (0)
    TRY_OR_CLEAN(hipSetDevice(device));
    hipDeviceProp_t prop;
    TRY_OR_CLEAN(hipGetDeviceProperties(&prop, device));
    if (std::strncmp(prop.gcnArchName, "gfx950", 6) != 0)
        return cleanup(fail(SAME_ENODEVICE, "device %d is %s; this build carries gfx950 code only", device, prop.gcnArchName));
    rx->want.relaxed = (flags & SAME_BATCH_RELAXED) != 0;
    rx->want.time_parallel = rx->tp.enabled;
    rx->want.generic = (flags & SAME_BATCH_GENERIC_KERNEL) != 0;
    rx->mode = same::select_mode(rx->P, rx->want);
    rx->plain = same::select_plain(rx->P, rx->mode, rx->want);
    rx->Pfm = same::fm_params(rx->P);
    rx->last_family = same::strict_family(rx->P, rx->mode);
    if (same::demod_lds_bytes(rx->P) > 160 * 1024)
        return cleanup(fail(SAME_EINVAL, "configuration needs %zu bytes of LDS per wavefront (limit 160 KiB)", same::demod_lds_bytes(rx->P)));
    TRY_OR_CLEAN(hipStreamCreateWithFlags(&rx->own_stream, hipStreamNonBlocking));
    TRY_OR_CLEAN(hipStreamCreateWithFlags(&rx->copy_stream, hipStreamNonBlocking));
    TRY_OR_CLEAN(hipStreamCreateWithFlags(&rx->plan_stream, hipStreamNonBlocking));
    TRY_OR_CLEAN(rx->ev_order.ensure());
    for (auto &sl : rx->slot) {
        TRY_OR_CLEAN(sl.ev_start.ensure(hipEventDefault));
        TRY_OR_CLEAN(sl.ev_stop.ensure(hipEventDefault));
        TRY_OR_CLEAN(sl.ev_k0.ensure(hipEventDefault));
        TRY_OR_CLEAN(sl.ev_k1.ensure(hipEventDefault));
        TRY_OR_CLEAN(sl.ev_done.ensure());
        TRY_OR_CLEAN(sl.ev_planned.ensure());
        TRY_OR_CLEAN(sl.d_counters.ensure(4));
        TRY_OR_CLEAN(sl.h_counters.ensure(4));
    }
    static_assert(sizeof(float4) == 4 * sizeof(float), "the taps are uploaded in fours");
    TRY_OR_CLEAN(rx->d_taps.ensure(taps.size() / 4));
    TRY_OR_CLEAN(hipMemcpy(rx->d_taps, taps.data(), taps.size() * sizeof(float), hipMemcpyHostToDevice));
    const size_t state_bytes = carve_state(rx->P, nullptr, rx->S);
    TRY_OR_CLEAN(rx->d_state_blob.ensure(state_bytes));
    TRY_OR_CLEAN(hipMemset(rx->d_state_blob, 0, state_bytes));
    carve_state(rx->P, (char *)rx->d_state_blob.get(), rx->S);
    TRY_OR_CLEAN(same::launch_init_state(rx->P, rx->S, 0, rx->own_stream));
    if (rx->dev_transport) {
        TRY_OR_CLEAN(rx->d_thot.ensure((size_t)n_channels * same::transport_hot_bytes()));
        TRY_OR_CLEAN(rx->d_tcold.ensure((size_t)n_channels * same::transport_cold_bytes()));
        TRY_OR_CLEAN(hipMemsetAsync(rx->d_tcold, 0, (size_t)n_channels * same::transport_cold_bytes(), rx->own_stream));
        TRY_OR_CLEAN(same::launch_transport_reset(rx->d_thot, rx->d_tcold, n_channels, nullptr, 0, 1, rx->own_stream));
    }
    TRY_OR_CLEAN(hipStreamSynchronize(rx->own_stream));
#undef TRY_OR_CLEAN
    if (!(flags & SAME_BATCH_LINK_ONLY) && !rx->dev_transport) { rx->thot.resize(n_channels); rx->tcold.resize(n_channels); }
    if (rx->tp.enabled) { rx->tp.sym_off.assign(n_channels, 0); rx->tp.synth.assign(n_channels, TickSynth{}); }
    rx->resets.init(n_channels);
    *out = rx;
    return SAME_OK;
}

void same_batch_free(same_batch *rx)
{
    if (!rx) return;
    (void)hipSetDevice(rx->device);
    if (rx->last_stream) (void)hipStreamSynchronize(rx->last_stream);
    const hipStream_t streams[3] = {rx->copy_stream, rx->plan_stream, rx->own_stream};
    delete rx;
    for (hipStream_t st : streams)
        if (st) (void)hipStreamDestroy(st);
}

int same_batch_reset(same_batch *rx)
{
    if (!rx) return fail(SAME_EINVAL, "null handle");
    HIP_TRY(hipSetDevice(rx->device));
    int rc = harvest(rx);
    if (rc) return rc;
    hipError_t e = same::launch_init_state(rx->P, rx->S, 1, rx->own_stream);
    if (e == hipSuccess && rx->dev_transport)
        e = same::launch_transport_reset(rx->d_thot, rx->d_tcold, rx->P.n_channels, nullptr, 0, 0, rx->own_stream, rx->audio.d_rec);
    if (e != hipSuccess) return fail(SAME_EHIP, "reset launch failed: %s", hipGetErrorString(e));
    HIP_TRY(hipStreamSynchronize(rx->own_stream));
    rx->counter = 0;
    rx->inv.fill = 0;
    rx->queue.clear(); rx->queue_head = 0;
    rx->arena.clear();
    rx->peeked_valid = false; rx->peeked_release = false; rx->peeked_head = 0;
    std::vector<same_rx_event>().swap(rx->peeked);
    rx->burst_seq.clear(); rx->burst_seq_head = 0;
    for (uint32_t c = 0; c < (uint32_t)rx->thot.size(); ++c) rx->tr(c).reset();
// ... 582 lines not shown
```

sameold_amd/csrc/same_device.h:

```cpp
#pragma once

#include <stddef.h>
#include <stdint.h>

namespace same {

constexpr int kWave = 64;
constexpr int kMaxEqTaps = 16;
constexpr int kBurstCap = 288;
constexpr int kSquelchHist = 64;
constexpr int kMaxTaps = 512;

struct Params {
    uint32_t n_channels;
    uint32_t input_rate;
    uint32_t dc_len;
    float dc_inv_len;
    float dc_k;
    float agc_bw, agc_min, agc_max, agc_gain0;
    uint32_t ntaps;
    uint32_t win_ring;
    float samples_per_ted, period_min, period_max;
    float alpha_unlocked, beta_unlocked, alpha_locked, beta_locked;
    uint32_t sync_word, sq_max_errors;
    float sq_power_open, sq_power_close, sq_bw;
    uint32_t eq_nff, eq_nfb;
    float eq_relaxation, eq_regularization;
    uint32_t fr_max_prefix_errors, fr_max_invalid;
    uint32_t block_len;
    uint32_t trace_cap;
    uint32_t ticks;
    uint32_t tick_interburst;
    uint32_t tick_history;
    int32_t knob_pipe;
    int32_t knob_pipe_lanes;
    int32_t knob_pipe_split;
    int32_t knob_mirror;
    int32_t knob_fast_dense;
    int32_t knob_pipe_share;
    int32_t knob_relaxed_kernel;
    int32_t knob_sym;
    int32_t knob_prio;
};

enum : uint32_t {
    F_AGC_LOCKED = 1u << 0,
    F_TED_PHASE = 1u << 1,
    F_BW_LOCKED = 1u << 2,
    F_SQ_LOCK = 1u << 3,
    F_EQ_MODE_SHIFT = 4,
    F_EQ_MODE_MASK = 3u << 4,
    F_FR_STATE_SHIFT = 6,
    F_FR_STATE_MASK = 3u << 6,
    F_LINK_SHIFT = 8,
    F_LINK_MASK = 3u << 8,
    F_TICK_AGAIN = 1u << 10,
    F_EQ_BITS_SHIFT = 16,
    F_EQ_BITS_MASK = 0xffu << 16,
};
constexpr int kTickRing = 8;

struct State {
    float *dc_ff_ring;
    float *dc_fb_ring;
    float *dc_sum0, *dc_sum1;
    float *agc_gain;
    float *win_ring;
    uint32_t *ted_clock;
    float *until_next_ted;
    float *ted_h0, *ted_h1, *ted_h2;
    float *period_avg, *period_inst;
    uint32_t *sq_data;
    float *sq_power;
    uint32_t *sq_phist;
    uint32_t *sq_fill;
    int32_t *sq_clock;
    uint64_t *sq_symbols;
    float *sq_hist;
    float *eq_ffc, *eq_fbc;
    float *eq_ffw, *eq_fbw;
    uint32_t *eq_word, *eq_count;
    float *eq_snap_ffc, *eq_snap_fbc, *eq_snap_ffw, *eq_snap_fbw;
    uint32_t *fr_word, *fr_count, *fr_invalid, *fr_len;
    uint8_t *fr_msg;
    uint32_t *flags;
    uint64_t *tk_next;
    uint64_t *tk_last;
    uint64_t *tk_ring;
    uint32_t *tk_n;
    uint64_t *wake_sample;
    uint64_t *wake_fired;
    uint32_t *trace_n;
    float *trace;
    uint64_t *trace_idx;
};

struct PipeChunks {
    uint32_t n_chunks;
    uint32_t in_channels;
    uint32_t stride_blocks;
    uint32_t nominal_blocks;
    uint64_t *handover;
    const uint32_t *col_row0;
    const uint32_t *col_nominal;
    const uint32_t *wg_blocks;
    const uint32_t *col_perm;
    float *hist_scratch;
    uint64_t in_samples;
    uint32_t whole_samples;
};

struct ChunkGeom {
    uint64_t counter0;
    uint32_t n_chunks, block_len, stride_blocks, warmup_blocks;
#if defined(__HIPCC__)
    __host__ __device__
#endif
    uint32_t owner_of(uint64_t h) const
    {
        const uint64_t blocks = (h - counter0) / block_len;
        if (blocks < warmup_blocks) return 0u;
        const uint64_t k = (blocks - warmup_blocks) / stride_blocks;
        return k >= n_chunks ? n_chunks - 1u : (uint32_t)k;
    }
#if defined(__HIPCC__)
    __host__ __device__
#endif
    uint64_t own_start(uint32_t k) const
    { return k == 0u ? counter0 : counter0 + ((uint64_t)k * stride_blocks + warmup_blocks) * block_len; }
};
constexpr uint64_t kNoHandover = ~0ull;

struct StateArrayDesc { char *src; char *dst; uint32_t rows; uint32_t elem_words; };

constexpr uint32_t kDevEventNone = 0xffffffffu;
struct DevEvent {
    uint32_t channel;
    uint32_t kind;
    uint64_t sample_counter;
    uint64_t symbol_count;
    uint32_t burst_len;
    uint32_t burst_slot;
};

constexpr uint32_t kDevMessageText = 272;
struct DevMessage {
    uint32_t channel;
    uint32_t kind;
    uint64_t sample_counter;
    uint64_t symbol_count;
    uint32_t len, aux, aux2;
    uint32_t seq;
    uint8_t text[kDevMessageText];
};

struct Output {
    DevEvent *events;
    uint32_t *n_events;
    uint32_t event_cap;
    uint8_t *bursts;
    uint32_t *n_bursts;
    uint32_t burst_cap;
    uint32_t *overflow;
};

}
```

sameold_amd/csrc/same_kernels_sym.hip:

```cpp
#include <hip/hip_runtime.h>

#include <cmath>
#include <cstdlib>
#include <mutex>
#include <set>
#include <type_traits>
#include <utility>

#include "same_dev_common.h"
#include "same_device.h"
#include "same_fast_common.h"
#include "same_launch.h"
#include "same_pipe_common.h"
#include "same_profile.h"
#include "same_relaxed_common.h"

namespace same {

constexpr int kSymSub = 36;
constexpr uint32_t kSymDrain = 5u;
constexpr uint32_t kSymOffMask = 255u;
template <int NT> struct SymGeom;
template <> struct SymGeom<42> { static constexpr int DCL = 16, NSUB = 1, HALVES = 2; };
template <> struct SymGeom<92> { static constexpr int DCL = 35, NSUB = 2, HALVES = 1; };
// ... 555 lines not shown
        for (uint32_t m = 1; m <= G; ++m) {
            const uint32_t g = (uint32_t)(counter1 - (uint64_t)m) & (G - 1u);
            const uint32_t j = wnext >= m ? wnext - m : wnext + (uint32_t)RING - m;
            float *row = S.win_ring + (size_t)g * C;
            row[c] = wcol[j * LP];
        }
    }
};

enum : uint32_t { YM_VALID = 1u, YM_READY = 2u, YM_ADJUSTED = 4u, YM_READING = 8u, YM_DROP = 16u, YM_BYTE_SHIFT = 8, YM_OFF_SHIFT = 16 };
enum : uint32_t { FB_VALID = 1u, FB_AGC = 2u, FB_BW = 4u, FB_END = 8u, FB_SQLOCK = 16u };

template <int NFF, int NFB>
struct SymSquelch {
    Lane L;
    uint32_t nsym;
    float ffc[NFF], ffw[NFF], fbc[NFB], fbw[NFB];
    float sffc[NFF], sffw[NFF], sfbc[NFB], sfbw[NFB];
    char *hbase;
    uint32_t hcol4, hrow4;
    float nxt0 = 0.0f, nxt1 = 0.0f;
    __device__ __forceinline__ float *hptr(uint32_t slot) const { return reinterpret_cast<float *>(hbase + (size_t)(__umul24(slot, hrow4) + hcol4)); }

    __device__ __forceinline__ void eq_reset()
    {
#pragma unroll
        for (int i = 0; i < NFF; ++i) { ffc[i] = (i == 0) ? 1.0f : 0.0f; ffw[i] = 0.0f; }
#pragma unroll
        for (int i = 0; i < NFB; ++i) { fbc[i] = (i == 0) ? 1.0f : 0.0f; fbw[i] = 0.0f; }
    }
    __device__ __forceinline__ void end()
    {
        L.flags &= ~(F_AGC_LOCKED | F_SQ_LOCK | F_BW_LOCKED);
        L.sq_clock = -1;
        eq_reset();
    }
    __device__ __forceinline__ uint32_t eq_step_masked(const Params &P, bool act, float in0, float in1)
    {
        const uint32_t mode = (L.flags & F_EQ_MODE_MASK) >> F_EQ_MODE_SHIFT;
        float w[NFF];
        if constexpr (NFF >= 2) {
#pragma unroll
            for (int i = 0; i + 2 < NFF; ++i) w[i] = ffw[i + 2];
            w[NFF - 2] = in0; w[NFF - 1] = in1;
        } else {
            w[0] = in1;
        }
        float f0 = 0.0f, f1 = 0.0f, q0 = 0.0f, q1 = 0.0f;
#pragma unroll
        for (int i = 0; i < NFF; ++i) {
            if (i & 1) { f1 = __builtin_fmaf(w[NFF - 1 - i], ffc[i], f1); q1 = __builtin_fmaf(w[i], w[i], q1); }
            else { f0 = __builtin_fmaf(w[NFF - 1 - i], ffc[i], f0); q0 = __builtin_fmaf(w[i], w[i], q0); }
        }
        constexpr auto fb_zero = [](int widx) { return ((NFB - 1 - widx) & 1) == 0; };
        float fbs = 0.0f, qb = 0.0f;
#pragma unroll
        for (int i = 0; i < NFB; ++i) {
            if (!fb_zero(NFB - 1 - i)) fbs = __builtin_fmaf(fbw[NFB - 1 - i], fbc[i], fbs);
            if (!fb_zero(i)) qb = __builtin_fmaf(fbw[i], fbw[i], qb);
        }
        const float sym_val = (f0 + f1) - fbs;
        const bool training = act & (mode == 2u), evolve = act & (mode != 0u);
        const float sym_est = (mode == 2u) ? ((L.eq_word & 1u) ? 1.0f : -1.0f) : rs_signum(sym_val);
        const float err = evolve ? sym_est - sym_val : 0.0f;
        L.eq_word = training ? L.eq_word >> 1 : L.eq_word;
        L.eq_count = training ? L.eq_count + 1u : L.eq_count;
        const uint32_t mode1 = (training && L.eq_count >= 32u) ? 1u : mode;
        const float gf = P.eq_relaxation * __builtin_amdgcn_rcpf(P.eq_regularization + (q0 + q1));
        const float gb = P.eq_relaxation * __builtin_amdgcn_rcpf(P.eq_regularization + qb);
        const float ge = gf * err, gn = -(gb * err);
#pragma unroll
        for (int i = 0; i < NFF; ++i) ffc[i] = __builtin_fmaf(ge, w[NFF - 1 - i], ffc[i]);
#pragma unroll
        for (int i = 0; i < NFB; ++i) { if (!fb_zero(NFB - 1 - i)) fbc[i] = __builtin_fmaf(gn, fbw[NFB - 1 - i], fbc[i]); }
#pragma unroll
        for (int i = 0; i < NFF; ++i) ffw[i] = act ? w[i] : ffw[i];
        if constexpr (NFB >= 2) {
#pragma unroll
            for (int i = 0; i + 2 < NFB; ++i) fbw[i] = act ? fbw[i + 2] : fbw[i];
            fbw[NFB - 2] = act ? sym_est : fbw[NFB - 2];
            fbw[NFB - 1] = act ? 0.0f : fbw[NFB - 1];
        } else {
            fbw[0] = act ? 0.0f : fbw[0];
        }
        L.flags = (L.flags & ~F_EQ_MODE_MASK) | (mode1 << F_EQ_MODE_SHIFT);
        return sym_est >= 0.0f ? 1u : 0u;
    }
    __device__ __forceinline__ void end_masked(bool m)
    {
        L.flags = m ? (L.flags & ~(F_AGC_LOCKED | F_SQ_LOCK | F_BW_LOCKED)) : L.flags;
        L.sq_clock = m ? -1 : L.sq_clock;
#pragma unroll
        for (int i = 0; i < NFF; ++i) { ffc[i] = m ? ((i == 0) ? 1.0f : 0.0f) : ffc[i]; ffw[i] = m ? 0.0f : ffw[i]; }
#pragma unroll
        for (int i = 0; i < NFB; ++i) { fbc[i] = m ? ((i == 0) ? 1.0f : 0.0f) : fbc[i]; fbw[i] = m ? 0.0f : fbw[i]; }
    }
    __device__ __forceinline__ uint32_t symbol_masked(const Params &P, bool valid, float zero, float sym, uint32_t off, uint32_t *fb)
    {
        const uint32_t before = L.flags & (F_AGC_LOCKED | F_BW_LOCKED);
        const uint32_t slot = (2u * nsym) & 63u;
        const float eq_in0 = nxt0, eq_in1 = nxt1;
        {
            float *pn = hptr((slot + 18u) & 63u), *pw = hptr(slot);
            const float l0 = pn[0], l1 = *reinterpret_cast<float *>(reinterpret_cast<char *>(pn) + hrow4);
            nxt0 = valid ? l0 : nxt0; nxt1 = valid ? l1 : nxt1;
            if (valid) { pw[0] = zero; *reinterpret_cast<float *>(reinterpret_cast<char *>(pw) + hrow4) = sym; }
        }
        const uint32_t fill = min(64u, L.sq_fill + 2u);
        L.sq_fill = valid ? fill : L.sq_fill;
        const uint32_t data = (L.sq_data >> 1) | ((sym >= 0.0f) ? 0x80000000u : 0u);
        L.sq_data = valid ? data : L.sq_data;
        const uint32_t nerr = __popc(P.sync_word ^ data);
        const float pwr = fmaxf(__builtin_fmaf(__builtin_fmaf(sym, sym, -L.sq_power), P.sq_bw, L.sq_power), 0.0f);
        L.sq_power = valid ? pwr : L.sq_power;
        const uint32_t phist = (L.sq_phist << 1) | ((pwr >= P.sq_power_close) ? 1u : 0u);
        L.sq_phist = valid ? phist : L.sq_phist;
        nsym += valid ? 1u : 0u;
        const int32_t clock_before = L.sq_clock;
        const bool full = valid & (fill >= 64u);
        const bool locked = (L.flags & F_SQ_LOCK) != 0u;
        const bool sync_now = full & !locked & (nerr <= P.sq_max_errors) & (pwr >= P.sq_power_open);
        const bool adjusted = sync_now & (clock_before != 0);
        const bool drop = full & !sync_now & (clock_before >= 0) & ((phist & 0x80000000u) == 0u);
        int32_t clk = sync_now ? 0 : clock_before;
        clk = drop ? -1 : clk;
        const bool ready = full & (clk == 0);
        const bool reading = full & (clk > 0);
        clk = ready ? 1 : (reading ? ((clk + 1) & 7) : clk);
        L.sq_clock = clk;
        const bool act = (clock_before >= 0) & !adjusted & (ready | reading);
        if (__builtin_expect(__builtin_amdgcn_ballot_w64(act) != 0ull, 1)) {
            const uint32_t j = (uint32_t)(clock_before + 7) & 7u;
            const uint32_t ebit = eq_step_masked(P, act, eq_in0, eq_in1);
            uint32_t bits = (j == 0u) ? 0u : ((L.flags & F_EQ_BITS_MASK) >> F_EQ_BITS_SHIFT);
            bits |= ebit << j;
            L.flags = act ? ((L.flags & ~F_EQ_BITS_MASK) | (bits << F_EQ_BITS_SHIFT)) : L.flags;
        }
        uint32_t byte = (L.flags & F_EQ_BITS_MASK) >> F_EQ_BITS_SHIFT;
        const bool train = ready & adjusted;
        if (__builtin_expect(__builtin_amdgcn_ballot_w64(train) != 0ull, 0)) {
            const bool back = train & (clock_before >= 0);
#pragma unroll
            for (int i = 0; i < NFF; ++i) { ffc[i] = back ? sffc[i] : ffc[i]; ffw[i] = back ? sffw[i] : ffw[i]; }
#pragma unroll
            for (int i = 0; i < NFB; ++i) { fbc[i] = back ? sfbc[i] : fbc[i]; fbw[i] = back ? sfbw[i] : fbw[i]; }
            L.flags = train ? ((L.flags & ~F_EQ_MODE_MASK) | (2u << F_EQ_MODE_SHIFT) | F_AGC_LOCKED | F_BW_LOCKED) : L.flags;
            L.eq_word = train ? P.sync_word : L.eq_word; L.eq_count = train ? 0u : L.eq_count;
            const uint32_t head = (2u * nsym) & 63u;
            float samples[16];
#pragma unroll
            for (int i = 0; i < 16; ++i) samples[i] = *hptr((head + (uint32_t)i) & 63u);
            uint32_t tb = 0u;
#pragma unroll 1
            for (int b = 0; b < 8; ++b) tb |= eq_step_masked(P, train, samples[2 * b], samples[2 * b + 1]) << b;
            byte = train ? tb : byte;
        }
        const bool snap = ready & ((L.flags & F_SQ_LOCK) == 0u);
        if (__builtin_amdgcn_ballot_w64(snap) != 0ull) {
#pragma unroll
            for (int i = 0; i < NFF; ++i) { sffc[i] = snap ? ffc[i] : sffc[i]; sffw[i] = snap ? ffw[i] : sffw[i]; }
#pragma unroll
            for (int i = 0; i < NFB; ++i) { sfbc[i] = snap ? fbc[i] : sfbc[i]; sfbw[i] = snap ? fbw[i] : sfbw[i]; }
        }
        if (__builtin_expect(__builtin_amdgcn_ballot_w64(drop) != 0ull, 0)) end_masked(drop);
        const uint32_t after = L.flags & (F_AGC_LOCKED | F_BW_LOCKED);
        *fb = (valid & ((after != before) | drop)) ? (FB_VALID | ((after & F_AGC_LOCKED) ? FB_AGC : 0u) | ((after & F_BW_LOCKED) ? FB_BW : 0u) | (drop ? FB_END : 0u) | (off << 8)) : 0u;
        return valid ? (YM_VALID | (ready ? YM_READY : 0u) | (adjusted ? YM_ADJUSTED : 0u) | (reading ? YM_READING : 0u) | (drop ? YM_DROP : 0u) |
                        (byte << YM_BYTE_SHIFT) | (off << YM_OFF_SHIFT)) : 0u;
    }
    __device__ __forceinline__ uint32_t symbol(const Params &P, float zero, float sym, uint32_t off, uint32_t *fb)
    {
        const uint32_t before = L.flags & (F_AGC_LOCKED | F_BW_LOCKED);
        const uint32_t slot = (2u * nsym) & 63u;
        const float eq_in0 = nxt0, eq_in1 = nxt1;
        {
            float *pn = hptr((slot + 18u) & 63u), *pw = hptr(slot);
            nxt0 = pn[0]; nxt1 = *reinterpret_cast<float *>(reinterpret_cast<char *>(pn) + hrow4);
            pw[0] = zero; *reinterpret_cast<float *>(reinterpret_cast<char *>(pw) + hrow4) = sym;
        }
        const uint32_t fill = min(64u, L.sq_fill + 2u);
        L.sq_fill = fill;
        L.sq_data = (L.sq_data >> 1) | ((sym >= 0.0f) ? 0x80000000u : 0u);
        const uint32_t nerr = __popc(P.sync_word ^ L.sq_data);
        const float pwr = fmaxf(__builtin_fmaf(__builtin_fmaf(sym, sym, -L.sq_power), P.sq_bw, L.sq_power), 0.0f);
        L.sq_power = pwr;
        L.sq_phist = (L.sq_phist << 1) | ((pwr >= P.sq_power_close) ? 1u : 0u);
        nsym += 1u;
        const int32_t clock_before = L.sq_clock;
        const bool full = fill >= 64u;
        const bool locked = (L.flags & F_SQ_LOCK) != 0u;
        const bool sync_now = full & !locked & (nerr <= P.sq_max_errors) & (pwr >= P.sq_power_open);
        const bool adjusted = sync_now & (clock_before != 0);
        const bool drop = full & !sync_now & (clock_before >= 0) & ((L.sq_phist & 0x80000000u) == 0u);
        int32_t clk = sync_now ? 0 : clock_before;
        clk = drop ? -1 : clk;
        const bool ready = full & (clk == 0);
        const bool reading = full & (clk > 0);
        clk = ready ? 1 : (reading ? ((clk + 1) & 7) : clk);
        L.sq_clock = clk;
        if ((clock_before >= 0) & !adjusted & (ready | reading)) {
            const uint32_t j = (uint32_t)(clock_before + 7) & 7u;
            const uint32_t ebit = eq_symbol_relaxed<NFF, NFB>(P, L, ffc, ffw, fbc, fbw, eq_in0, eq_in1);
            uint32_t bits = (j == 0u) ? 0u : ((L.flags & F_EQ_BITS_MASK) >> F_EQ_BITS_SHIFT);
            bits |= ebit << j;
            L.flags = (L.flags & ~F_EQ_BITS_MASK) | (bits << F_EQ_BITS_SHIFT);
        }
        uint32_t byte = (L.flags & F_EQ_BITS_MASK) >> F_EQ_BITS_SHIFT;
        if (ready & adjusted) {
            if (clock_before >= 0) {
#pragma unroll
                for (int i = 0; i < NFF; ++i) { ffc[i] = sffc[i]; ffw[i] = sffw[i]; }
#pragma unroll
                for (int i = 0; i < NFB; ++i) { fbc[i] = sfbc[i]; fbw[i] = sfbw[i]; }
            }
            L.flags |= F_AGC_LOCKED | F_BW_LOCKED;
            L.flags = (L.flags & ~F_EQ_MODE_MASK) | (2u << F_EQ_MODE_SHIFT);
            L.eq_word = P.sync_word; L.eq_count = 0;
            const uint32_t head = (2u * nsym) & 63u;
            float samples[16];
#pragma unroll
            for (int i = 0; i < 16; ++i) samples[i] = *hptr((head + (uint32_t)i) & 63u);
            byte = 0u;
#pragma unroll 1
            for (int b = 0; b < 8; ++b) byte |= eq_symbol_relaxed<NFF, NFB>(P, L, ffc, ffw, fbc, fbw, samples[2 * b], samples[2 * b + 1]) << b;
        }
        if (ready & !(L.flags & F_SQ_LOCK)) {
#pragma unroll
            for (int i = 0; i < NFF; ++i) { sffc[i] = ffc[i]; sffw[i] = ffw[i]; }
#pragma unroll
            for (int i = 0; i < NFB; ++i) { sfbc[i] = fbc[i]; sfbw[i] = fbw[i]; }
        }
        if (drop) end();
        const uint32_t after = L.flags & (F_AGC_LOCKED | F_BW_LOCKED);
        *fb = (after != before || drop) ? (FB_VALID | ((after & F_AGC_LOCKED) ? FB_AGC : 0u) | ((after & F_BW_LOCKED) ? FB_BW : 0u) | (drop ? FB_END : 0u) | (off << 8)) : 0u;
        return YM_VALID | (ready ? YM_READY : 0u) | (adjusted ? YM_ADJUSTED : 0u) | (reading ? YM_READING : 0u) | (drop ? YM_DROP : 0u) |
               (byte << YM_BYTE_SHIFT) | (off << YM_OFF_SHIFT);
    }
};

struct SymFramer { uint32_t st, last, word, count, invalid, len; };
__device__ __forceinline__ uint32_t sym_framer_step(const Params &P, SymFramer &F, uint8_t *row, uint32_t m, uint32_t *burst_len, uint32_t *fb2, bool *emit)
{
    const bool valid = (m & YM_VALID) != 0u, ready = (m & YM_READY) != 0u, reading = (m & YM_READING) != 0u;
    const uint32_t byte = (m >> YM_BYTE_SHIFT) & 0xffu;
    const bool restart = (m & (YM_READY | YM_ADJUSTED)) == (YM_READY | YM_ADJUSTED);
    const uint32_t st = F.st;
    const bool burst_at_restart = restart & (st == 2u);
    const uint32_t st1 = restart ? 1u : st;
    const uint32_t word0 = restart ? 0u : F.word, count0 = restart ? 0u : F.count;
    const bool searching = ready & (st1 == 1u), rd = ready & (st1 == 2u);
    const uint32_t word = (word0 << 8) | byte, count = count0 + 1u;
    const uint32_t e0 = __popc(word ^ 0x5a435a43u);
    const uint32_t e1 = __popc(word ^ 0x4e4e4e4eu);
    const bool found = searching & (min(e0, e1) <= P.fr_max_prefix_errors);
    const bool give_up = searching & !found & (count > 21u);
    const uint32_t invalid = F.invalid + (is_allowed_byte(byte) ? 0u : 1u);
    const bool over = rd & (invalid > P.fr_max_invalid);
    const bool keep = rd & !over;
    F.word = searching ? word : word0;
    F.count = searching ? count : count0;
    F.invalid = found ? 0u : (rd ? invalid : F.invalid);
    if (found) *reinterpret_cast<uint32_t *>(row) = __builtin_bswap32(word);
    if (keep && F.len < (uint32_t)kBurstCap) row[F.len] = (uint8_t)byte;
    const bool was_reading_burst = valid & !ready & !reading & (st == 2u);
    *burst_len = (over | burst_at_restart | was_reading_burst) ? F.len : 0u;
    F.len = found ? 4u : (keep ? F.len + 1u : F.len);
    const uint32_t nst = found ? 2u : ((give_up | over) ? 0u : st1);
    const uint32_t link_ready = restart ? (burst_at_restart ? 3u : 1u) : (over ? 3u : nst);
    const uint32_t link_quiet = reading ? st : (st == 2u ? 3u : 0u);
    const uint32_t link = ready ? link_ready : link_quiet;
    F.st = ready ? nst : ((valid & !reading) ? 0u : st);
    const uint32_t fb_end = FB_VALID | FB_END | (((m >> YM_OFF_SHIFT) & kSymOffMask) << 8);
    *fb2 = ready ? (link == 2u ? (uint32_t)FB_SQLOCK : ((link == 0u || link == 3u) ? fb_end : 0u)) : 0u;
    *emit = valid & ((link != F.last) | (link == 3u));
    F.last = *emit ? link : F.last;
    return link;
}

#ifndef SYM_PRIOS
#define SYM_PRIOS 0x0031322
#endif
constexpr int sym_prio_of(int k) { return (int)((SYM_PRIOS >> (4 * (6 - k))) & 3); }
#ifndef SYM_PRIOS_HI
#define SYM_PRIOS_HI 0x3321200
#endif
template <int NT> constexpr int sym_prio(int k) { return NT == 42 ? sym_prio_of(k) : (int)((SYM_PRIOS_HI >> (4 * (6 - k))) & 3); }
template <int PRIO> __device__ __forceinline__ void sym_setprio(const Params &P)
{
#ifdef SAME_PROFILE
    const uint32_t variant = ((uint32_t)P.knob_prio >> 12) & 3u;
    if (variant == 1u) return;
    if (variant == 2u) { __builtin_amdgcn_s_setprio(PRIO >= 2 ? 3 : 0); return; }
#else
    (void)P;
#endif
    __builtin_amdgcn_s_setprio(PRIO);
}

__device__ __forceinline__ float sym_next_fire(float s)
{
    return fmaxf(floorf(s - 0.5f) + 1.0f, 1.0f);
}

struct SymKernArgs { Params P; State S; Output O; const float4 *taps; const void *x; uint32_t n_blocks; uint64_t counter0; PipeChunks K; };
typedef const __attribute__((address_space(4))) char *sym_kernarg_ptr;
template <typename T> __device__ __forceinline__ T sym_fresh_arg(sym_kernarg_ptr ka, size_t off)
{
    uint64_t p = (uint64_t)(uintptr_t)ka + off;
    asm volatile("" : "+s"(p));
    T r;
    __builtin_memcpy(&r, reinterpret_cast<const __attribute__((address_space(4))) void *>(p), sizeof(T));
    return r;
}

constexpr int kSymRoles = 6;
template <int NT, int NFF, int NFB, typename SampleT, int CMODE>
__global__ __launch_bounds__(SymGeom<NT>::HALVES * kSymRoles * kWave, NT == 42 ? 3 : 2) void demod_sym_kernel(Params P, State S_arg_, Output O_arg_, const float4 *__restrict__ taps,
                                                                         const SampleT *__restrict__ x, uint32_t n_blocks, uint64_t counter0,
                                                                         PipeChunks K)
{
    (void)S_arg_; (void)O_arg_;
    const sym_kernarg_ptr ka = (sym_kernarg_ptr)__builtin_amdgcn_kernarg_segment_ptr();
    auto fresh_state = [&]() __attribute__((always_inline)) -> State { return sym_fresh_arg<State>(ka, offsetof(SymKernArgs, S)); };
    auto fresh_output = [&]() __attribute__((always_inline)) -> Output { return sym_fresh_arg<Output>(ka, offsetof(SymKernArgs, O)); };
    using LY = SymLayout<NT>;
    constexpr int kB = LY::B, RING = LY::RING, kSB = LY::SB, kNSUB = LY::NSUB;
    constexpr uint32_t kSymHalves = (uint32_t)LY::HALVES;
    constexpr uint32_t LP = kWave;
    static_assert(CMODE == 0 || std::is_same<SampleT, float>::value, "channel-major streams are f32");
    if constexpr (CMODE == 0) { K.col_row0 = nullptr; K.col_perm = nullptr; }
    extern __shared__ float lds_all[];
    const uint32_t lane = threadIdx.x & (kWave - 1u);
    const uint32_t wave = (uint32_t)__builtin_amdgcn_readfirstlane((int)(threadIdx.x >> 6));
    constexpr uint64_t kDeal0 = 0xdcba98543210ull;
#ifdef SAME_PROFILE
    const uint32_t deal = ((uint32_t)P.knob_prio >> 14) & 3u;
    constexpr uint64_t kDeal1 = 0x805d192ab3c4ull;
    constexpr uint64_t kDeal2 = 0x08d591a2b3c4ull;
    constexpr uint64_t kDeal3 = 0x2ad51908b3c4ull;
    const uint64_t tbl = deal == 0u ? kDeal0 : (deal == 1u ? kDeal1 : (deal == 2u ? kDeal2 : kDeal3));
#else
    constexpr uint64_t tbl = kDeal0;
#endif
    const uint32_t hr = LY::HALVES == 2 ? (uint32_t)(tbl >> (4u * wave)) & 15u : wave;
    const uint32_t half = LY::HALVES == 2 ? hr >> 3 : 0u;
    const uint32_t role = hr & 7u;
    const uint32_t C = P.n_channels;
    const uint32_t vwg = blockIdx.x * kSymHalves + half;
    if (vwg * kWave >= C) return;
    float *lds = lds_all + half * (uint32_t)(LY::lds_bytes / sizeof(float));
    const uint32_t c = (K.n_chunks > 1u && K.col_perm) ? K.col_perm[vwg * kWave + lane] : vwg * kWave + lane;
    uint32_t cin = c, Cin = C, n_nominal = n_blocks;
    bool may_leave = false;
    int32_t row_l = 0;
    const SampleT *xl = nullptr;
    uint32_t avail_l = 0;
    if (K.n_chunks > 1u) {
        Cin = K.in_channels;
        if (K.col_row0) {
            const uint32_t chunk_l = c / Cin;
            cin = c - chunk_l * Cin;
            may_leave = (uint32_t)__builtin_amdgcn_readfirstlane((int)chunk_l) + 1u < K.n_chunks;
            const uint32_t row_abs = K.col_row0[c];
            xl = x + (size_t)cin * K.in_samples + row_abs;
            avail_l = (K.whole_samples - row_abs) / (uint32_t)kSB;
            n_blocks = K.wg_blocks[vwg];
            n_nominal = may_leave ? K.col_nominal[c] : n_blocks;
            const uint32_t row_first = (uint32_t)__builtin_amdgcn_readfirstlane((int)row_abs);
            counter0 += (uint64_t)row_first;
            row_l = (int32_t)(row_abs - row_first);
        } else {
            const uint32_t wgs = K.in_channels / kWave;
            const uint32_t chunk = (uint32_t)__builtin_amdgcn_readfirstlane((int)(vwg / wgs));
            cin = (vwg - chunk * wgs) * kWave + lane;
            may_leave = chunk + 1u < K.n_chunks;
            const uint32_t first_block = chunk * K.stride_blocks;
            x += (size_t)first_block * kB * Cin;
            counter0 += (uint64_t)first_block * kB;
            n_blocks -= first_block;
            n_nominal = may_leave ? K.nominal_blocks : n_blocks;
        }
    }
    lds_u32 *mail = (lds_u32 *)(lds + LY::tap_floats);
    lds_u32 *symbox = mail;
    lds_u32 *ybox = symbox + 2u * LY::sym_words;
    lds_u32 *fb1box = ybox + 2u * kWave;
    lds_u32 *fb2box = fb1box + 2u * LY::fb_words;
    lds_u32 *iobox = fb2box + 2u * LY::fb_words;
    lds_u32 *phasebox = iobox + 2u * LY::io_words;
    lds_u32 *againbox = phasebox + kWave;
    lds_u32 *flagbox = againbox + kWave;
    lds_u32 *posbox = flagbox + kWave;
    lds_u32 *sabox = posbox + 2u * kWave;
    lds_u32 *tkbox = sabox + kWave;
    lds_u32 *donebox = tkbox + kIoRingWords;
    lds_u32 *chunkbox = fb1box + kWave + 2u;
    lds_u32 *seqbox = fb1box + kWave + 4u;
    static_assert((size_t)(2u * LY::sym_words + 2u * kWave + 4u * LY::fb_words + 2u * LY::io_words + 3u * kWave + 2u * kWave + kWave + kIoRingWords + kWave + kWave) <= LY::mail_words, "mailboxes");
    float *wring = lds + LY::tap_floats + LY::mail_words;
    float *wcol = wring + lane;
    const uint64_t counter1 = counter0 + (uint64_t)n_blocks * kB;
    const uint32_t last_e_step = n_blocks + kSymDrain;
    const uint32_t last_y1_step = last_e_step + 1u, last_y2_step = last_e_step + 2u, last_a_step = last_e_step + 3u;
    const uint32_t n_steps = last_e_step + 4u;
    auto sym_index = [&](uint32_t s_e, uint32_t off) __attribute__((always_inline)) -> int64_t {
        const int64_t base = s_e <= n_blocks ? (int64_t)s_e - 2 : (int64_t)n_blocks - 3;
        return (int64_t)kB * base + (int64_t)off;
    };
    lds_u32 *prog = donebox + kWave;
    lds_u32 *pos2box = prog + kWave + (SYM_TL_WORDS + 63u) / 64u * 64u;
    lds_u32 *partbox = pos2box + 2u * kWave;
#ifdef SAME_SYM_TL
    lds_u32 *tlbox = prog + kWave;
#endif
    const uint32_t prog_idx = lane < (uint32_t)kSymRoles ? lane : 0u;
    uint32_t *const err_flags = fresh_output().n_events + 2;
    uint32_t spin_limit = 1u << 22;
    auto gave_up = [&]() __attribute__((always_inline)) -> bool { return spin_limit != (1u << 22); };
    constexpr bool kPeek = NT != 42;
    uint32_t seen = 0u;
    auto peek = [&]() __attribute__((always_inline)) { if constexpr (kPeek) seen = prog[prog_idx]; };
    auto wait_for = [&](uint32_t s, uint32_t deps, uint32_t *w_y1, uint32_t *w_y2, auto nap_) __attribute__((always_inline)) {
        constexpr int NAP = decltype(nap_)::value;
        uint32_t v = seen, spins = 0;
        if constexpr (!kPeek) v = prog[prog_idx];
        for (;;) {
            const uint32_t ok = (uint32_t)__builtin_amdgcn_ballot_w64(v >= (s << 16));
            if ((ok & deps) == deps) break;
            if (!kPeek || spins != 0u) __builtin_amdgcn_s_sleep(NAP);
            if (++spins > spin_limit) { if (lane == 0u) atomicOr(err_flags, 4u); spin_limit = 8u; break; }
            v = prog[prog_idx];
        }
        if constexpr (kPeek) seen = v;
        asm volatile("" ::: "memory");
        *w_y1 = (uint32_t)__builtin_amdgcn_readlane((int)v, 4);
        *w_y2 = (uint32_t)__builtin_amdgcn_readlane((int)v, 5);
    };
    constexpr std::integral_constant<int, 1> kNapShort{};
    constexpr std::integral_constant<int, 4> kNapLong{};
    auto flags_of_last = [&](uint32_t w, uint32_t s) __attribute__((always_inline)) -> uint32_t { return s == 0u ? 0u : (w >> (8u * ((s - 1u) & 1u))) & 0xffu; };
    auto publish = [&](uint32_t s, uint32_t flags, uint32_t flags_before) __attribute__((always_inline)) {
        asm volatile("" ::: "memory");
        if (lane == 0u) prog[role] = ((s + 1u) << 16) | (flags << (8u * (s & 1u))) | (flags_before << (8u * ((s + 1u) & 1u)));
    };
    enum : uint32_t { R_S = 1u, R_T = 2u, R_A = 4u, R_E = 8u, R_Y1 = 16u, R_Y2 = 32u };
    enum : uint32_t { Y1F_ANY = 1u, Y2F_END = 1u, Y2F_LEAVE = 2u, Y2F_LOCK = 4u };
    constexpr uint32_t kDepsS = R_T | R_A | R_E | R_Y1 | R_Y2;
    if (role == 0u && lane < (uint32_t)kSymRoles) prog[lane] = 0u;

    if (role == 0u) {
        sym_setprio<sym_prio<NT>(0)>(P);
        SymAgc<NT> M;
        { const State S = fresh_state(); M.load(P, S, c, C, counter0, wcol); }
        lds_barrier();
        P3_T0();
        uint32_t stop_at = 0xffffffffu;
        bool left = false;
        for (uint32_t s = 0; s < n_steps; ++s) {
            uint32_t w1, w2;
            SYM_TRACE(0, s, 0);
            wait_for(s, kDepsS, &w1, &w2, kNapLong);
            SYM_TRACE(0, s, 1);
            P3_LAP(p3_wait);
            const uint32_t f1 = flags_of_last(w1, s), f2 = flags_of_last(w2, s);
            if (f2 & Y2F_LEAVE) stop_at = s;
            if ((f2 & Y2F_END) && s >= 1u) {
                if (fb2box[((s - 1u) & 1u) * LY::fb_words + lane] & FB_VALID) M.locked = false;
            }
            if ((f1 & Y1F_ANY) && s >= 1u) {
                const uint32_t v = fb1box[((s - 1u) & 1u) * LY::fb_words + lane];
                if (v & FB_VALID) {
                    const bool new_locked = (v & FB_AGC) != 0u;
                    if (new_locked && !M.locked) {
                        const int64_t idx = sym_index(s - 2u, v >> 8);
                        const uint32_t b = (uint32_t)(idx / kB);
                        M.gain = M.gain_at(P, wcol, b, (int)(idx - (int64_t)b * kB));
                    }
                    M.locked = new_locked;
                }
                P3_LAP(p3_fb);
            }
            if (s < n_blocks && !PROF_SKIP(P, 64)) M.block(P, wcol, s);
            SYM_TRACE(0, s, 2);
            peek();
            publish(s, 0u, 0u);
            P3_LAP(p3_work);
            if (s == stop_at) { left = true; break; }
        }
        SYM_REPORT(0);
        if (left || gave_up()) return;
        { const State S = fresh_state(); M.store(P, S, c, C, counter1, wcol); }
    } else if (role == 1u) {
        sym_setprio<sym_prio<NT>(1)>(P);
        if constexpr (NT != 42) {
            static_assert(CMODE == 0 && kNSUB == 2, "time-major rows, two sub-blocks a step");
            SymDcRot<SampleT, NT> D;
            const uint32_t n_sub = n_blocks * (uint32_t)kNSUB;
            { const State S = fresh_state(); D.load(S, x, c, C, cin, Cin, counter0, n_sub); }
            donebox[lane] = 0u;
            D.template sub<0>(P, wcol, x, 0u, n_sub, cin, Cin);
            D.template sub<1>(P, wcol, x, 1u, n_sub, cin, Cin);
            lds_barrier();
            P3_T0();
            uint32_t stop_at = 0xffffffffu;
            auto step = [&](uint32_t s, auto ph_) __attribute__((always_inline)) -> bool {
                constexpr int PH = 2 * decltype(ph_)::value;
                uint32_t w1, w2;
                SYM_TRACE(1, s, 0);
                wait_for(s, R_A | R_E, &w1, &w2, kNapLong);
                SYM_TRACE(1, s, 1);
                P3_LAP(p3_wait);
                if (s + 1u < n_blocks && !PROF_SKIP(P, 128)) {
                    D.template sub<PH>(P, wcol, x, 2u * (s + 1u), n_sub, cin, Cin);
                    D.template sub<PH + 1>(P, wcol, x, 2u * (s + 1u) + 1u, n_sub, cin, Cin);
                }
                if (may_leave) {
                    wait_for(s, R_Y2, &w1, &w2, kNapLong);
                    if (flags_of_last(w2, s) & Y2F_LEAVE) stop_at = s;
                }
                SYM_TRACE(1, s, 2);
                peek();
                publish(s, 0u, 0u);
                P3_LAP(p3_work);
                return s == stop_at;
            };
            bool left = false;
            for (uint32_t s = 0; s < n_steps && !left; s += 3u) {
                left = step(s, std::integral_constant<int, 1>{});
                if (!left && s + 1u < n_steps) left = step(s + 1u, std::integral_constant<int, 2>{});
                if (!left && s + 2u < n_steps) left = step(s + 2u, std::integral_constant<int, 0>{});
            }
            SYM_REPORT(1);
            if (left || gave_up()) return;
            { const State S = fresh_state(); D.store(S, c, C, counter1, n_sub - 1u); }
            return;
        } else {
        using Dc = SymDc<SampleT, CMODE, NT>;
        Dc D;
        D.xl = xl; D.avail = avail_l;
        const uint32_t n_sub = n_blocks * (uint32_t)kNSUB;
        { const State S = fresh_state(); D.load(S, x, c, C, cin, Cin, counter0, n_sub); }
        donebox[lane] = 0u;
        auto sub_tm = [&](uint32_t q, auto pb_) __attribute__((always_inline)) {
            typename Dc::Pairs X;
            if constexpr (decltype(pb_)::value == 0) { D.request(D.xb, x, q + 1u, n_sub, cin, Cin); D.template take<0>(D.xa, X); }
            else { D.request(D.xa, x, q + 1u, n_sub, cin, Cin); D.template take<0>(D.xb, X); }
            D.block(P, wcol, X, q);
        };
        {
            if constexpr (CMODE == 1) {
                typename Dc::Pairs X0;
                D.request(D.xb, x, 1u, n_sub, cin, Cin);
                D.template take<9>(D.xa, X0);
                D.block(P, wcol, X0, 0u);
                D.request(D.xa, x, 2u, n_sub, cin, Cin);
            } else {
                sub_tm(0u, std::integral_constant<int, 0>{});
                if constexpr (kNSUB == 2) sub_tm(1u, std::integral_constant<int, 1>{});
            }
        }
        lds_barrier();
        P3_T0();
        uint32_t stop_at = 0xffffffffu;
        auto step = [&](uint32_t s, auto buf) __attribute__((always_inline)) -> bool {
            constexpr int BUF = decltype(buf)::value;
            uint32_t w1, w2;
            SYM_TRACE(1, s, 0);
            wait_for(s, R_A | R_E, &w1, &w2, kNapLong);
            SYM_TRACE(1, s, 1);
            P3_LAP(p3_wait);
            if constexpr (CMODE == 1) D.done = donebox[lane] != 0u;
            if (s + 1u < n_blocks && !PROF_SKIP(P, 128)) {
                if constexpr (CMODE == 1) {
                    typename Dc::Pairs X;
                    if constexpr (BUF == 0) { D.template take<9>(D.xa, X); D.block(P, wcol, X, s + 1u); D.request(D.xa, x, s + 3u, n_sub, cin, Cin); }
                    else { D.template take<9>(D.xb, X); D.block(P, wcol, X, s + 1u); D.request(D.xb, x, s + 3u, n_sub, cin, Cin); }
                } else if constexpr (kNSUB == 1) {
                    sub_tm(s + 1u, buf);
                } else {
                    sub_tm(2u * (s + 1u), std::integral_constant<int, 0>{});
                    sub_tm(2u * (s + 1u) + 1u, std::integral_constant<int, 1>{});
                }
            }
            if (may_leave) {
                wait_for(s, R_Y2, &w1, &w2, kNapLong);
                if (flags_of_last(w2, s) & Y2F_LEAVE) stop_at = s;
            }
            SYM_TRACE(1, s, 2);
            peek();
            publish(s, 0u, 0u);
            P3_LAP(p3_work);
            return s == stop_at;
        };
        bool left = false;
        for (uint32_t s = 0; s < n_steps && !left; s += 2u) {
            left = step(s, std::integral_constant<int, 1>{});
            if (!left && s + 1u < n_steps) left = step(s + 1u, std::integral_constant<int, 0>{});
        }
        SYM_REPORT(1);
        if (left || gave_up()) return;
        { const State S = fresh_state(); D.store(S, c, C, counter1); }
        }
    } else if (role == 2u) {
        sym_setprio<sym_prio<NT>(2)>(P);
        const uint32_t wcol_lds = lds_addr(wcol);
        std::conditional_t<NT == 42, SymTaps<42>, SymHalfTaps<NT, 0, NT / 4>> TP;
        TP.load(taps);
        Lane L;
        IoCtxLds X;
        X.chunk = chunkbox;
        if (lane == 0u) { chunkbox[0] = 0u; chunkbox[1] = kEvChunk; seqbox[0] = 0u; }
        X.pending_slot = 0xffffffffu;
        X.tk = tkbox + lane;
        {
            const State S = fresh_state();
            lane_load(L, S, c);
            X.ring_load(P, S, c);
        }
        const State Snone{};
        Output O{};
        { const Output Of = fresh_output(); O.events = Of.events; O.n_events = Of.n_events; O.event_cap = Of.event_cap; }
        lds_barrier();
        P3_T0();
        uint32_t stop_at = 0xffffffffu;
        bool left = false;
        for (uint32_t s = 0; s < n_steps; ++s) {
            uint32_t w1, w2;
            SYM_TRACE(2, s, 0);
            wait_for(s, R_S | R_E, &w1, &w2, kNapShort);
            SYM_TRACE(2, s, 1);
            P3_LAP(p3_wait);
            if (s >= 1u && s <= last_e_step) {
                const uint32_t n1 = posbox[(s & 1u) * kWave + lane];
                if constexpr (NT == 42) {
                    if (__builtin_amdgcn_ballot_w64(n1 != 0xffffffffu) != 0ull) {
                        const float sa1 = PROF_SKIP(P, 256) ? 0.0f : TP.template demod<RING>(wcol_lds, n1 == 0xffffffffu ? 0 : (int)n1);
                        sabox[lane] = __float_as_uint(sa1);
                        if (lane == 0u) seqbox[0] = 2u * s + 1u;
                    }
                } else {
                    const uint32_t n2 = pos2box[(s & 1u) * kWave + lane];
                    if (__builtin_amdgcn_ballot_w64(n2 != 0xffffffffu) != 0ull) {
                        float2v r2 = {0.0f, 0.0f}, i2 = {0.0f, 0.0f}, r1 = {0.0f, 0.0f}, i1 = {0.0f, 0.0f};
                        if (!PROF_SKIP(P, 256)) {
                            TP.template partial<RING>(wcol_lds, n2 == 0xffffffffu ? 0 : (int)n2, r2, i2);
                            if (__builtin_amdgcn_ballot_w64(n1 != 0xffffffffu) != 0ull) TP.template partial<RING>(wcol_lds, n1 == 0xffffffffu ? 0 : (int)n1, r1, i1);
                        }
                        lds_u32 *pb = partbox + lane;
                        pb[0] = __float_as_uint(r2.x); pb[kWave] = __float_as_uint(r2.y); pb[2 * kWave] = __float_as_uint(i2.x); pb[3 * kWave] = __float_as_uint(i2.y);
                        pb[4 * kWave] = __float_as_uint(r1.x); pb[5 * kWave] = __float_as_uint(r1.y); pb[6 * kWave] = __float_as_uint(i1.x); pb[7 * kWave] = __float_as_uint(i1.y);
                        if (lane == 0u) seqbox[0] = 2u * s + 1u;
                    }
                }
            }
            SYM_TRACE(2, s, 3);
            sym_setprio<sym_prio<NT>(3)>(P);
            wait_for(s, R_Y2, &w1, &w2, kNapLong);
            if (flags_of_last(w2, s) & Y2F_LEAVE) stop_at = s;
            if (s >= 4u && s <= last_a_step && !PROF_SKIP(P, 8)) {
                const lds_u32 *io = iobox + ((s - 1u) & 1u) * LY::io_words + lane;
                const uint32_t io0 = io[0];
                if (io0 & 1u) {
                    L.sq_symbols += 1;
                    const uint32_t link = (io0 >> 1) & 3u, off = (io0 >> 4) & kSymOffMask;
                    const bool burst = (io0 & 8u) != 0u && link == 3u;
                    uint32_t burst_len = 0;
                    if (burst) { X.pending_slot = io[kWave]; burst_len = io[2 * kWave]; }
                    const uint64_t counter = counter0 + (int64_t)row_l + (uint64_t)sym_index(s - 3u, off) + 1u;
                    symbol_io(P, L, Snone, O, X, c, link, (io0 & 8u) != 0u, counter, burst_len);
                }
            }
            if (s + 1u == n_steps) againbox[lane] = L.flags & F_TICK_AGAIN;
            SYM_TRACE(2, s, 2);
            peek();
            publish(s, 0u, 0u);
            sym_setprio<sym_prio<NT>(2)>(P);
            P3_LAP(p3_work);
            if (s == stop_at) { left = true; break; }
        }
        SYM_REPORT(2);
        X.retire(O, lane, kWave);
        if (left || gave_up()) return;
        {
            const State S = fresh_state();
            S.tk_next[c] = L.tk_next; S.tk_last[c] = L.tk_last; S.wake_fired[c] = L.wake_fired;
            X.ring_store(P, S, c);
        }
    } else if (role == 3u) {
        sym_setprio<sym_prio<NT>(4)>(P);
        const uint32_t wcol_lds = lds_addr(wcol);
        std::conditional_t<NT == 42, SymTaps<42>, SymHalfTaps<NT, NT / 4, NT / 2>> TP;
        TP.load(taps);
        Lane L;
        { const State S = fresh_state(); lane_load(L, S, c); }
        const float inv_spt = 1.0f / P.samples_per_ted;
        int cstar = next_fire_count(L.until_next_ted, L.ted_clock);
        int rel = cstar - (int)L.ted_clock - 1;
        float cstar_f = (float)cstar;
        SYM_T_DECL();
        bool pl_typeA = false, pl_ready = false, pl_single = false;
        int pl_p2 = 0;
        uint32_t pl_n2 = 0, pl_n1 = 0xffffffffu;
        float pl_rem1 = 0.0f, pl_instA = 0.0f, pl_c2 = 0.0f;
        auto plan = [&](uint32_t s) __attribute__((always_inline)) {
            pl_single = s > n_blocks;
            const uint32_t wb = (min(s, n_blocks) % (uint32_t)LY::NBLK) * (uint32_t)kB;
            pl_typeA = !pl_single && (L.flags & F_TED_PHASE) != 0u;
            pl_rem1 = L.until_next_ted - cstar_f;
            pl_instA = L.period_inst + __builtin_amdgcn_fmed3f(pl_rem1, -0.5f, 0.5f);
            pl_c2 = sym_next_fire(pl_instA);
            pl_p2 = pl_typeA ? rel + (int)pl_c2 : rel;
            pl_ready = pl_p2 < 0 && s >= 1u && s <= last_e_step;
            auto slot = [&](int p) __attribute__((always_inline)) { int n = (int)wb + p; n += n < 0 ? RING : 0; return (uint32_t)n; };
            pl_n2 = pl_ready ? slot(pl_p2) : 0u;
            pl_n1 = (pl_ready && pl_typeA) ? slot(rel) : 0xffffffffu;
            posbox[(s & 1u) * kWave + lane] = pl_n1;
            if constexpr (NT != 42) pos2box[(s & 1u) * kWave + lane] = pl_ready ? pl_n2 : 0xffffffffu;
        };
        float sa1 = 0.0f, sa2 = 0.0f;
        auto filters = [&](uint32_t seq) __attribute__((always_inline)) {
            sa1 = 0.0f; sa2 = 0.0f;
            if (__builtin_amdgcn_ballot_w64(pl_ready) != 0ull) {
                SYM_T_BEGIN();
                SYM_TCOUNT(20, 1);
                auto wait_for_a = [&]() __attribute__((always_inline)) {
                    uint32_t spins = 0;
                    while ((int32_t)(seqbox[0] - seq) < 0) {
                        __builtin_amdgcn_s_sleep(1);
                        if (++spins > spin_limit) { if (lane == 0u) atomicOr(err_flags, 4u); spin_limit = 8u; break; }
                    }
                    asm volatile("" ::: "memory");
                };
                if constexpr (NT == 42) {
                    sa2 = PROF_SKIP(P, 512) ? 0.0f : TP.template demod<RING>(wcol_lds, (int)pl_n2);
                    SYM_T_LAP(22);
                    if (__builtin_amdgcn_ballot_w64(pl_ready && pl_typeA) != 0ull) {
                        wait_for_a();
                        sa1 = __uint_as_float(sabox[lane]);
                    }
                } else {
                    float2v r2 = {0.0f, 0.0f}, i2 = {0.0f, 0.0f}, r1 = {0.0f, 0.0f}, i1 = {0.0f, 0.0f};
                    const bool any_a = __builtin_amdgcn_ballot_w64(pl_n1 != 0xffffffffu) != 0ull;
                    if (!PROF_SKIP(P, 512)) {
                        TP.template partial<RING>(wcol_lds, (int)pl_n2, r2, i2);
                        if (any_a) TP.template partial<RING>(wcol_lds, pl_n1 == 0xffffffffu ? 0 : (int)pl_n1, r1, i1);
                    }
                    SYM_T_LAP(22);
                    wait_for_a();
                    const lds_u32 *pb = partbox + lane;
                    r2 += float2v{__uint_as_float(pb[0]), __uint_as_float(pb[kWave])}; i2 += float2v{__uint_as_float(pb[2 * kWave]), __uint_as_float(pb[3 * kWave])};
                    sa2 = sym_soft_sample(r2, i2);
                    if (any_a) {
                        r1 += float2v{__uint_as_float(pb[4 * kWave]), __uint_as_float(pb[5 * kWave])}; i1 += float2v{__uint_as_float(pb[6 * kWave]), __uint_as_float(pb[7 * kWave])};
                        sa1 = sym_soft_sample(r1, i1);
                    }
                }
                SYM_T_LAP(24);
            }
        };
        auto work = [&](uint32_t s) __attribute__((always_inline)) {
            SYM_T_BEGIN();
            const bool rdy = pl_ready, tA = pl_typeA;
            const float p1 = tA ? L.h2 : L.h1, p2 = tA ? sa1 : L.h2;
            const float inst_pre = tA ? pl_instA : L.period_inst;
            const float rem = tA ? pl_instA - pl_c2 : pl_rem1;
            const uint32_t flags_new = tA ? L.flags : (L.flags ^ F_TED_PHASE);
            const bool have = (flags_new & F_TED_PHASE) != 0u;
            const float dsg = rs_signum(p1) - rs_signum(sa2);
            const float te = p2 * dsg;
            const float offset = __builtin_amdgcn_fmed3f(rem, -0.5f, 0.5f);
            const float e = __builtin_amdgcn_fmed3f(__builtin_fmaf(-offset, inv_spt, te), -1.0f, 1.0f);
            const bool bw_locked = (L.flags & F_BW_LOCKED) != 0u;
            const float alpha = bw_locked ? P.alpha_locked : P.alpha_unlocked;
            const float beta = bw_locked ? P.beta_locked : P.beta_unlocked;
            const float avg1 = __builtin_amdgcn_fmed3f(__builtin_fmaf(beta, e, L.period_avg), P.period_min, P.period_max);
            float inst1 = __builtin_fmaf(alpha, e, avg1) + offset;
            inst1 = (inst1 < 0.0f) ? avg1 : inst1;
            const float inst_new = have ? inst1 : inst_pre + offset;
            const float cs = sym_next_fire(inst_new);
            const bool take = rdy & have;
            L.h0 = rdy ? p1 : L.h0; L.h1 = rdy ? p2 : L.h1; L.h2 = rdy ? sa2 : L.h2;
            L.flags = rdy ? flags_new : L.flags;
            L.period_avg = take ? avg1 : L.period_avg;
            L.period_inst = rdy ? inst_new : L.period_inst; L.until_next_ted = rdy ? inst_new : L.until_next_ted;
            cstar_f = rdy ? cs : cstar_f;
            rel = rdy ? pl_p2 + (int)cs : rel;
            const uint32_t hdr = take ? (1u | ((uint32_t)(pl_p2 + (pl_single ? 3 * kB : 2 * kB)) << 8)) : 0u;
            SYM_T_LAP(23);
            lds_u32 *sb = symbox + (s & 1u) * LY::sym_words + lane;
            sb[0] = hdr;
            sb[kWave] = __float_as_uint(p2); sb[2 * kWave] = __float_as_uint(sa2);
            if (P.trace_cap) { sb[3 * kWave] = __float_as_uint(te); sb[4 * kWave] = __float_as_uint(inst_new); }
        };
        auto late = [&](uint32_t v) __attribute__((always_inline)) {
            if (v & FB_VALID) {
                L.flags = (L.flags & ~F_BW_LOCKED) | ((v & FB_BW) ? F_BW_LOCKED : 0u);
                if (v & FB_END) {
                    L.flags &= ~F_TED_PHASE;
                    L.h0 = 0.0f; L.h1 = 0.0f; L.h2 = 0.0f;
                    L.period_avg = P.samples_per_ted; L.period_inst = P.samples_per_ted;
                }
            }
        };
        plan(0u);
        lds_barrier();
        P3_T0();
        uint32_t stop_at = 0xffffffffu;
        bool left = false;
        for (uint32_t s = 0; s < n_steps; ++s) {
            uint32_t w1, w2;
            SYM_TRACE(3, s, 0);
            wait_for(s, R_S, &w1, &w2, kNapShort);
            SYM_TRACE(3, s, 1);
            P3_LAP(p3_wait);
            if (!PROF_SKIP(P, 32)) filters(2u * s + 1u);
            wait_for(s, R_A | R_Y1 | R_Y2, &w1, &w2, kNapShort);
            SYM_TRACE(3, s, 3);
            const uint32_t f1 = flags_of_last(w1, s), f2 = flags_of_last(w2, s);
            if (f2 & Y2F_LEAVE) stop_at = s;
            uint32_t late1 = 0u, late2 = 0u;
            if ((f1 & Y1F_ANY) && s >= 1u) late1 = fb1box[((s - 1u) & 1u) * LY::fb_words + lane];
            if ((f2 & Y2F_END) && s >= 1u) late2 = fb2box[((s - 1u) & 1u) * LY::fb_words + lane];
            if (!PROF_SKIP(P, 32)) {
                work(s);
                if (__builtin_amdgcn_ballot_w64(((late1 | late2) & FB_VALID) != 0u) != 0ull) { late(late2); late(late1); }
                if (s + 1u <= n_blocks) rel -= kB;
                plan(s + 1u);
            }
            if (s + 1u == n_steps) phasebox[lane] = L.flags & F_TED_PHASE;
            SYM_TRACE(3, s, 2);
            peek();
            publish(s, 0u, 0u);
            P3_LAP(p3_work);
            if (s == stop_at) { left = true; break; }
        }
        SYM_REPORT(3);
        SYM_T_REPORT();
        if (left || gave_up()) return;
        L.ted_clock = (uint32_t)((int)cstar_f - rel - 1);
        {
            const State S = fresh_state();
            S.until_next_ted[c] = L.until_next_ted; S.ted_clock[c] = L.ted_clock;
            S.ted_h0[c] = L.h0; S.ted_h1[c] = L.h1; S.ted_h2[c] = L.h2;
            S.period_avg[c] = L.period_avg; S.period_inst[c] = L.period_inst;
        }
    } else if (role == 4u) {
        sym_setprio<sym_prio<NT>(5)>(P);
        SymSquelch<NFF, NFB> Q;
        uint64_t symbols0;
        const bool hist_copy = K.n_chunks > 1u && K.col_perm != nullptr && K.hist_scratch != nullptr;
        {
            const State S = fresh_state();
            lane_load(Q.L, S, c);
            symbols0 = Q.L.sq_symbols;
            Q.nsym = (uint32_t)symbols0;
            Q.hbase = reinterpret_cast<char *>(hist_copy ? K.hist_scratch : S.sq_hist);
            Q.hcol4 = (hist_copy ? vwg * kWave + lane : c) * 4u;
            Q.hrow4 = C * 4u;
            if (hist_copy) {
#pragma unroll 4
                for (int i = 0; i < kSquelchHist; ++i) *Q.hptr((uint32_t)i) = S.sq_hist[(size_t)i * C + c];
            }
#pragma unroll
            for (int i = 0; i < NFF; ++i) {
                Q.ffc[i] = S.eq_ffc[i * C + c]; Q.ffw[i] = S.eq_ffw[i * C + c];
                Q.sffc[i] = S.eq_snap_ffc[i * C + c]; Q.sffw[i] = S.eq_snap_ffw[i * C + c];
            }
#pragma unroll
            for (int i = 0; i < NFB; ++i) {
                Q.fbc[i] = S.eq_fbc[i * C + c]; Q.fbw[i] = S.eq_fbw[i * C + c];
                Q.sfbc[i] = S.eq_snap_fbc[i * C + c]; Q.sfbw[i] = S.eq_snap_fbw[i * C + c];
            }
            const uint32_t pslot = (2u * Q.nsym) & 63u;
            Q.nxt0 = *Q.hptr((pslot + 16u) & 63u); Q.nxt1 = *Q.hptr((pslot + 17u) & 63u);
        }
        lds_barrier();
        P3_T0();
        uint32_t stop_at = 0xffffffffu, flags_before = 0u, last_msg = 0u;
        bool left = false;
        for (uint32_t s = 0; s < n_steps; ++s) {
            uint32_t w1, w2;
            SYM_TRACE(4, s, 0);
            wait_for(s, R_E | R_Y2 | R_S, &w1, &w2, kNapShort);
            SYM_TRACE(4, s, 1);
            P3_LAP(p3_wait);
            const uint32_t f2 = flags_of_last(w2, s);
            if (f2 & Y2F_LEAVE) stop_at = s;
            if ((f2 & (Y2F_END | Y2F_LOCK)) && s >= 1u) {
                const uint32_t from_y2 = fb2box[((s - 1u) & 1u) * LY::fb_words + lane];
                const bool superseded = (last_msg & (YM_DROP | YM_ADJUSTED)) != 0u;
#ifdef SYM_Y1_SELECT
                Q.L.flags |= ((from_y2 & FB_SQLOCK) && !superseded) ? (uint32_t)F_SQ_LOCK : 0u;
                const bool y2_end = (from_y2 & FB_END) && !superseded;
                if (__builtin_expect(__builtin_amdgcn_ballot_w64(y2_end) != 0ull, 0)) Q.end_masked(y2_end);
#else
                if ((from_y2 & FB_SQLOCK) && !superseded) Q.L.flags |= F_SQ_LOCK;
                if ((from_y2 & FB_END) && !superseded) Q.end();
#endif
            }
            last_msg = 0u;
            uint32_t flags = 0u;
            if (s >= 2u && s <= last_y1_step) {
                const lds_u32 *sb = symbox + ((s - 1u) & 1u) * LY::sym_words + lane;
                const uint32_t hdr = sb[0], zero_w = sb[kWave], sym_w = sb[2 * kWave];
                uint32_t msg = 0u, fbv = 0u;
#ifdef SYM_Y1_SELECT
                {
                    const bool valid = (hdr & 1u) && !PROF_SKIP(P, 16);
                    const uint32_t off = hdr >> 8;
                    const float zero = __uint_as_float(zero_w), sym = __uint_as_float(sym_w);
                    if (P.trace_cap && valid) {
                        const State S = fresh_state();
                        const uint64_t counter = counter0 + (int64_t)row_l + (uint64_t)sym_index(s - 1u, off) + 1u;
                        const uint32_t n = S.trace_n[c];
                        if (n < P.trace_cap) {
                            float *t = S.trace + ((size_t)c * P.trace_cap + n) * 4;
                            t[0] = zero; t[1] = sym; t[2] = __uint_as_float(sb[3 * kWave]); t[3] = __uint_as_float(sb[4 * kWave]);
                            S.trace_idx[(size_t)c * P.trace_cap + n] = counter;
                        }
                        S.trace_n[c] = n + 1;
                    }
                    msg = Q.symbol_masked(P, valid, zero, sym, off, &fbv);
                }
#else
                if ((hdr & 1u) && !PROF_SKIP(P, 16)) {
                    const uint32_t off = hdr >> 8;
                    const float zero = __uint_as_float(zero_w), sym = __uint_as_float(sym_w);
                    if (P.trace_cap) {
                        const State S = fresh_state();
                        const uint64_t counter = counter0 + (int64_t)row_l + (uint64_t)sym_index(s - 1u, off) + 1u;
                        const uint32_t n = S.trace_n[c];
                        if (n < P.trace_cap) {
                            float *t = S.trace + ((size_t)c * P.trace_cap + n) * 4;
                            t[0] = zero; t[1] = sym; t[2] = __uint_as_float(sb[3 * kWave]); t[3] = __uint_as_float(sb[4 * kWave]);
                            S.trace_idx[(size_t)c * P.trace_cap + n] = counter;
                        }
                        S.trace_n[c] = n + 1;
                    }
                    msg = Q.symbol(P, zero, sym, off, &fbv);
                }
#endif
                ybox[(s & 1u) * kWave + lane] = msg;
                last_msg = msg;
                if (__builtin_amdgcn_ballot_w64(fbv != 0u) != 0ull) {
                    uint32_t u1, u2;
                    wait_for(s, R_S, &u1, &u2, kNapLong);
                    fb1box[(s & 1u) * LY::fb_words + lane] = fbv; flags = Y1F_ANY;
                }
            }
            if (s + 1u == n_steps) flagbox[lane] = Q.L.flags & (F_AGC_LOCKED | F_BW_LOCKED | F_SQ_LOCK | F_EQ_MODE_MASK | F_EQ_BITS_MASK);
            SYM_TRACE(4, s, 2);
            peek();
            publish(s, flags, flags_before);
            flags_before = flags;
            P3_LAP(p3_work);
            if (s == stop_at) { left = true; break; }
        }
        SYM_REPORT(4);
        if (left || gave_up()) return;
        const State S = fresh_state();
        S.sq_data[c] = Q.L.sq_data; S.sq_power[c] = Q.L.sq_power; S.sq_phist[c] = Q.L.sq_phist;
        S.sq_fill[c] = Q.L.sq_fill; S.sq_clock[c] = Q.L.sq_clock; S.sq_symbols[c] = symbols0 + (uint64_t)(Q.nsym - (uint32_t)symbols0);
        S.eq_word[c] = Q.L.eq_word; S.eq_count[c] = Q.L.eq_count;
        if (hist_copy) {
#pragma unroll 4
            for (int i = 0; i < kSquelchHist; ++i) S.sq_hist[(size_t)i * C + c] = *Q.hptr((uint32_t)i);
        }
#pragma unroll
        for (int i = 0; i < NFF; ++i) {
            S.eq_ffc[i * C + c] = Q.ffc[i]; S.eq_ffw[i * C + c] = Q.ffw[i];
            S.eq_snap_ffc[i * C + c] = Q.sffc[i]; S.eq_snap_ffw[i * C + c] = Q.sffw[i];
        }
#pragma unroll
        for (int i = 0; i < NFB; ++i) {
            S.eq_fbc[i * C + c] = Q.fbc[i]; S.eq_fbw[i * C + c] = Q.fbw[i];
            S.eq_snap_fbc[i * C + c] = Q.sfbc[i]; S.eq_snap_fbw[i * C + c] = Q.sfbw[i];
        }
    } else {
        sym_setprio<sym_prio<NT>(6)>(P);
        Lane L;
        SymFramer F;
        uint8_t *fr_rows;
        { const State S0 = fresh_state(); lane_load(L, S0, c); fr_rows = S0.fr_msg; }
        F.st = fr_state(L); F.last = (L.flags & F_LINK_MASK) >> F_LINK_SHIFT;
        F.word = L.fr_word; F.count = L.fr_count; F.invalid = L.fr_invalid; F.len = L.fr_len;
        uint8_t *const row = fr_rows + (size_t)c * kBurstCap;
        Output O{};
        { const Output Of = fresh_output(); O.n_events = Of.n_events; O.bursts = Of.bursts; O.burst_cap = Of.burst_cap; }
        lds_barrier();
        P3_T0();
        uint32_t stop_at = 0xffffffffu, flags_before = 0u;
        bool left = false, lane_done = false, leave_posted = false;
        for (uint32_t s = 0; s < n_steps; ++s) {
            uint32_t w1, w2;
            SYM_TRACE(5, s, 0);
            wait_for(s, R_Y1 | R_S | R_T | R_A | R_E, &w1, &w2, kNapShort);
            SYM_TRACE(5, s, 1);
            P3_LAP(p3_wait);
            uint32_t flags = 0u;
            if (s >= 3u && s <= last_y2_step) {
                const uint32_t m = PROF_SKIP(P, 1024) ? 0u : ybox[((s - 1u) & 1u) * kWave + lane];
                uint32_t fbv = 0, burst_len = 0, io1 = 0xffffffffu;
                bool emit = false;
                const uint32_t link = sym_framer_step(P, F, row, m, &burst_len, &fbv, &emit);
                const bool want_slot = emit & (link == 3u);
                const uint32_t io0 = (m & YM_VALID) ? (1u | (link << 1) | (emit ? 8u : 0u) | (((m >> YM_OFF_SHIFT) & kSymOffMask) << 4)) : 0u;
                uint64_t pend = __builtin_amdgcn_ballot_w64(want_slot);
                lds_u32 *io = iobox + (s & 1u) * LY::io_words + lane;
                if (pend != 0ull) {
                    const uint32_t n_new = (uint32_t)__popcll(pend);
                    uint32_t base = 0;
                    if (lane == 0u) base = atomicAdd(O.n_events + 1, n_new);
                    base = (uint32_t)__builtin_amdgcn_readfirstlane((int)base);
                    uint32_t k = 0;
                    while (pend != 0ull) {
                        const int j = __builtin_ctzll(pend);
                        pend &= pend - 1ull;
                        const uint32_t b = base + k++;
                        const uint32_t cj = (uint32_t)__builtin_amdgcn_readlane((int)c, j);
                        if (b < O.burst_cap) {
                            const uint32_t *src = reinterpret_cast<const uint32_t *>(fr_rows + (size_t)cj * kBurstCap);
                            uint32_t *dst = reinterpret_cast<uint32_t *>(O.bursts + (size_t)b * kBurstCap);
                            constexpr uint32_t kWords = (uint32_t)kBurstCap / 4u, kPer = (kWords + kWave - 1u) / kWave;
                            uint32_t t[kPer];
#pragma unroll
                            for (uint32_t i = 0; i < kPer; ++i) { const uint32_t w = lane + i * kWave; t[i] = w < kWords ? src[w] : 0u; }
#pragma unroll
                            for (uint32_t i = 0; i < kPer; ++i) { const uint32_t w = lane + i * kWave; if (w < kWords) dst[w] = t[i]; }
                            if ((int)lane == j) io1 = b;
                        } else {
                            if (lane == 0u) atomicOr(O.n_events + 2, 2u);
                            if ((int)lane == j) io1 = 0xffffffffu;
                        }
                    }
                    io[kWave] = io1; io[2 * kWave] = burst_len;
                }
                io[0] = io0;
                const bool any_end = __builtin_amdgcn_ballot_w64((fbv & FB_VALID) != 0u) != 0ull;
                const bool any_lock = __builtin_amdgcn_ballot_w64((fbv & FB_SQLOCK) != 0u) != 0ull;
                if (any_end || any_lock) fb2box[(s & 1u) * LY::fb_words + lane] = fbv;
                flags = (any_end ? Y2F_END : 0u) | (any_lock ? Y2F_LOCK : 0u);
                if (may_leave && !leave_posted) {
                    const uint32_t blk = min(s - 3u, n_blocks - 1u);
                    if (!lane_done && blk + 1u >= n_nominal && F.last == 0u && (xl == nullptr || blk < avail_l)) {
                        lane_done = true;
                        K.handover[c] = counter0 + (int64_t)row_l + (uint64_t)(blk + 1u) * kB;
                        donebox[lane] = 1u;
                    }
                    if (__builtin_amdgcn_ballot_w64(!lane_done) == 0ull) { flags |= Y2F_LEAVE; leave_posted = true; stop_at = s + 1u; }
                }
            }
            SYM_TRACE(5, s, 2);
            peek();
            publish(s, flags, flags_before);
            flags_before = flags;
            P3_LAP(p3_work);
            if (s == stop_at) { left = true; break; }
        }
        SYM_REPORT(5);
        SYM_COUNT(18, 1);
        SYM_COUNT(19, left ? stop_at + 1u : n_steps);
        if (left || gave_up()) return;
        uint32_t w1, w2;
        wait_for(n_steps, R_A | R_E | R_Y1, &w1, &w2, kNapShort);
        if (gave_up()) return;
        const uint32_t flags_out = (F.st << F_FR_STATE_SHIFT) | (F.last << F_LINK_SHIFT) | (phasebox[lane] & F_TED_PHASE) | (againbox[lane] & F_TICK_AGAIN) | flagbox[lane];
        const State S1 = fresh_state();
        S1.fr_word[c] = F.word; S1.fr_count[c] = F.count; S1.fr_invalid[c] = F.invalid;
        S1.fr_len[c] = F.len; S1.flags[c] = flags_out;
    }
}

#if !defined(SAME_PROFILE) && !defined(SAME_SYM_TL)
#define SYM_SPLIT_TU 1
#endif
static_assert(SymLayout<42>::B == kSymStep22 && SymLayout<92>::B == kSymStepHi && SymLayout<84>::B == kSymStepHi && SymLayout<42>::NBLK == kSymRingSteps &&
              SymLayout<92>::NBLK == kSymRingSteps, "same_select.h decides with these steps and this ring");

template <int NT, int NFF, int NFB, typename SampleT>
static hipError_t launch_sym_one(const Params &P, const State &S, const Output &O, const float4 *taps, const SampleT *x,
                                 uint32_t n_blocks, uint64_t counter0, hipStream_t stream, const PipeChunks &K)
{
    constexpr uint32_t kSymHalves = (uint32_t)SymLayout<NT>::HALVES;
    constexpr size_t lds = (size_t)kSymHalves * SymLayout<NT>::lds_bytes;
    static_assert(lds <= 160u * 1024u, "one workgroup per CU");
    const bool cm = K.n_chunks > 1u && K.col_row0 != nullptr;
    if (cm && (!std::is_same<SampleT, float>::value || NT != 42)) return hipErrorInvalidValue;
    if (K.n_chunks > 1u && (K.in_channels % kWave) != 0u) return hipErrorInvalidValue;
    if (n_blocks == 0u) return hipSuccess;
    auto go = [&](auto kernel) -> hipError_t {
        if (lds > 64u * 1024u) {
            static std::mutex mu;
            static std::set<std::pair<const void *, int>> opted_in;
            int dev = 0;
            if (hipGetDevice(&dev) != hipSuccess) return hipErrorInvalidDevice;
            const std::pair<const void *, int> key(reinterpret_cast<const void *>(kernel), dev);
            std::lock_guard<std::mutex> lock(mu);
            if (opted_in.find(key) == opted_in.end()) {
                const hipError_t e = hipFuncSetAttribute(key.first, hipFuncAttributeMaxDynamicSharedMemorySize, (int)lds);
                if (e != hipSuccess) return e;
                opted_in.insert(key);
            }
        }
        hipLaunchKernelGGL(kernel, dim3((P.n_channels / kWave + kSymHalves - 1u) / kSymHalves), dim3(kSymHalves * kSymRoles * kWave), lds, stream, P, S, O, taps, x, n_blocks, counter0, K);
        return hipGetLastError();
    };
    if constexpr (std::is_same<SampleT, float>::value && NT == 42) {
        if (cm) return go(demod_sym_kernel<NT, NFF, NFB, float, 1>);
    }
    return go(demod_sym_kernel<NT, NFF, NFB, SampleT, 0>);
}

template <typename SampleT>
static hipError_t launch_sym_hi_t(const Params &P, const State &S, const Output &O, const float4 *taps, const SampleT *x,
                                  uint32_t n_blocks, uint64_t counter0, hipStream_t stream, const PipeChunks &K)
{
    const bool eq = P.eq_nff == 6u && P.eq_nfb == 4u;
    if (standard_rate_taps(P) == 92u)
        return eq ? launch_sym_one<92, 6, 4, SampleT>(P, S, O, taps, x, n_blocks, counter0, stream, K) : launch_sym_one<92, 1, 1, SampleT>(P, S, O, taps, x, n_blocks, counter0, stream, K);
    return eq ? launch_sym_one<84, 6, 4, SampleT>(P, S, O, taps, x, n_blocks, counter0, stream, K) : launch_sym_one<84, 1, 1, SampleT>(P, S, O, taps, x, n_blocks, counter0, stream, K);
}
#if defined(SYM_TU_HI)
#if defined(SYM_SPLIT_TU)
hipError_t launch_demod_sym_hi(const Params &P, const State &S, const Output &O, const float4 *taps, const float *x,
                               uint32_t n_blocks, uint64_t counter0, hipStream_t stream, const PipeChunks &K)
{ return launch_sym_hi_t<float>(P, S, O, taps, x, n_blocks, counter0, stream, K); }
hipError_t launch_demod_sym_hi(const Params &P, const State &S, const Output &O, const float4 *taps, const int16_t *x,
                               uint32_t n_blocks, uint64_t counter0, hipStream_t stream, const PipeChunks &K)
{ return launch_sym_hi_t<int16_t>(P, S, O, taps, x, n_blocks, counter0, stream, K); }
#endif
#else
#if defined(SYM_SPLIT_TU)
hipError_t launch_demod_sym_hi(const Params &P, const State &S, const Output &O, const float4 *taps, const float *x,
                               uint32_t n_blocks, uint64_t counter0, hipStream_t stream, const PipeChunks &K);
hipError_t launch_demod_sym_hi(const Params &P, const State &S, const Output &O, const float4 *taps, const int16_t *x,
                               uint32_t n_blocks, uint64_t counter0, hipStream_t stream, const PipeChunks &K);
#else
template <typename SampleT>
static hipError_t launch_demod_sym_hi(const Params &P, const State &S, const Output &O, const float4 *taps, const SampleT *x,
                                      uint32_t n_blocks, uint64_t counter0, hipStream_t stream, const PipeChunks &K)
{ return launch_sym_hi_t<SampleT>(P, S, O, taps, x, n_blocks, counter0, stream, K); }
#endif
template <typename SampleT>
static hipError_t launch_sym_t(const Params &P, const State &S, const Output &O, const float4 *taps, const SampleT *x,
                               uint32_t n_blocks, uint64_t counter0, hipStream_t stream, const PipeChunks &K)
{
    if (!sym_kernel_supported(P)) return hipErrorInvalidValue;
    const bool eq = P.eq_nff == 6u && P.eq_nfb == 4u;
    if (standard_rate_taps(P) == 42u)
        return eq ? launch_sym_one<42, 6, 4, SampleT>(P, S, O, taps, x, n_blocks, counter0, stream, K) : launch_sym_one<42, 1, 1, SampleT>(P, S, O, taps, x, n_blocks, counter0, stream, K);
    return launch_demod_sym_hi(P, S, O, taps, x, n_blocks, counter0, stream, K);
}
hipError_t launch_demod_sym(const Params &P, const State &S, const Output &O, const float4 *taps, const float *x,
                            uint32_t n_blocks, uint64_t counter0, hipStream_t stream, const PipeChunks &K)
{ return launch_sym_t<float>(P, S, O, taps, x, n_blocks, counter0, stream, K); }
hipError_t launch_demod_sym(const Params &P, const State &S, const Output &O, const float4 *taps, const int16_t *x,
                            uint32_t n_blocks, uint64_t counter0, hipStream_t stream, const PipeChunks &K)
{ return launch_sym_t<int16_t>(P, S, O, taps, x, n_blocks, counter0, stream, K); }
#endif

}

#if !defined(SYM_TU_HI)
SYM_PROFILE_EXPORTS()
#endif
```

sameold_amd/csrc/same_launch.h:

```cpp
#pragma once

#include <hip/hip_runtime.h>

#include "same_capture_dev.h"
#include "same_device.h"
#include "same_select.h"

namespace same {

hipError_t launch_demod(const Params &P, const State &S, const Output &O, const float4 *taps,
                        const float *x, uint32_t n_samples, uint64_t counter0, hipStream_t stream);
hipError_t launch_demod(const Params &P, const State &S, const Output &O, const float4 *taps,
                        const int16_t *x, uint32_t n_samples, uint64_t counter0, hipStream_t stream);
hipError_t launch_demod_ragged(const Params &P, const State &S, const Output &O, const float4 *taps, const float *x,
                               uint32_t n_rows, const uint32_t *counts, uint32_t row_sub, uint64_t counter0, hipStream_t stream);
hipError_t launch_demod_ragged(const Params &P, const State &S, const Output &O, const float4 *taps, const int16_t *x,
                               uint32_t n_rows, const uint32_t *counts, uint32_t row_sub, uint64_t counter0, hipStream_t stream);
hipError_t launch_demod_pipe(const Params &P, const State &S, const Output &O, const float4 *taps,
                             const float *x, uint32_t n_blocks, uint64_t counter0, hipStream_t stream,
                             const PipeChunks &chunks = PipeChunks{}, bool relaxed = false);
hipError_t launch_demod_pipe(const Params &P, const State &S, const Output &O, const float4 *taps,
                             const int16_t *x, uint32_t n_blocks, uint64_t counter0, hipStream_t stream,
                             const PipeChunks &chunks = PipeChunks{}, bool relaxed = false);
hipError_t launch_demod_sym(const Params &P, const State &S, const Output &O, const float4 *taps,
                            const float *x, uint32_t n_blocks, uint64_t counter0, hipStream_t stream,
                            const PipeChunks &chunks = PipeChunks{});
hipError_t launch_demod_sym(const Params &P, const State &S, const Output &O, const float4 *taps,
                            const int16_t *x, uint32_t n_blocks, uint64_t counter0, hipStream_t stream,
                            const PipeChunks &chunks = PipeChunks{});
hipError_t launch_demod_relaxed(const Params &P, const State &S, const Output &O, const float4 *taps,
                                const float *x, uint32_t n_blocks, uint64_t counter0, hipStream_t stream,
                                const PipeChunks &chunks = PipeChunks{});
hipError_t launch_demod_relaxed(const Params &P, const State &S, const Output &O, const float4 *taps,
                                const int16_t *x, uint32_t n_blocks, uint64_t counter0, hipStream_t stream,
                                const PipeChunks &chunks = PipeChunks{});
hipError_t launch_demod_fast(const Params &P, const State &S, const Output &O, const float4 *taps,
                             const float *x, uint32_t n_blocks, uint64_t counter0, hipStream_t stream);
hipError_t launch_demod_fast(const Params &P, const State &S, const Output &O, const float4 *taps,
                             const int16_t *x, uint32_t n_blocks, uint64_t counter0, hipStream_t stream);
hipError_t launch_counters(uint32_t *dev, uint32_t *host_mapped, int publish, hipStream_t stream);
uint32_t event_sort_extra_words(uint32_t n_bins);
hipError_t launch_event_sort(const DevEvent *ev, const uint32_t *counters, uint32_t cap, uint32_t n_bins, uint32_t *cnt, uint32_t *first,
                             DevEvent *sorted, hipStream_t stream, bool cnt_is_zero = false);
hipError_t launch_init_state(const Params &P, const State &S, int is_reset, hipStream_t stream, uint32_t first_col = 0);
hipError_t launch_reset_columns(const Params &P, const State &S, const uint32_t *cols, uint32_t n, hipStream_t stream);
hipError_t launch_copy_state_columns(const StateArrayDesc *desc, uint32_t n_desc, uint32_t src_channels,
                                     uint32_t dst_channels, const uint32_t *src_col, uint32_t n_cols, hipStream_t stream,
                                     uint32_t src_base = 0);
hipError_t launch_chunk_final_column(const uint64_t *handover, uint32_t in_channels, ChunkGeom g, uint32_t *final_col,
                                     hipStream_t stream);
hipError_t launch_chunk_final_column_pc(const uint64_t *handover, const uint32_t *own_start, uint32_t in_channels, uint32_t n_chunks,
                                        uint64_t counter0, uint32_t *final_col, hipStream_t stream);
hipError_t launch_fill_u64(uint64_t *p, size_t n, uint64_t v, hipStream_t stream);
hipError_t launch_cast_i16_f32(const int16_t *in, float *out, size_t n, hipStream_t stream);
hipError_t launch_tp_prologue(void *blob, const void *fresh, size_t bytes, uint64_t *handover, uint32_t *sort_cnt, uint32_t n_cols,
                              uint32_t *counters, hipStream_t stream);
uint32_t tp_scout_block();
struct TpPlan {
    uint32_t channels, n_chunks, block_len, warmup_samples, whole_samples;
    uint64_t in_samples;
    uint32_t scout_blocks;
};
hipError_t launch_tp_plan(const float *x, const TpPlan &g, float *energy, uint32_t *own_start, uint32_t *row0,
                          uint32_t *nominal, uint32_t *perm, uint32_t *wg_blocks, bool sorted, hipStream_t stream,
                          uint32_t *perm_out = nullptr, uint32_t *wg_blocks_out = nullptr, bool pairs = false);
hipError_t launch_transpose(const float *in, float *out, uint32_t n_channels, uint32_t n_samples,
                            hipStream_t stream);
hipError_t launch_transpose(const int16_t *in, int16_t *out, uint32_t n_channels, uint32_t n_samples,
                            hipStream_t stream);

constexpr uint32_t kMessageLogOverflow = 8u;
struct TransportLaunch {
    uint32_t n_channels, input_rate;
    const uint32_t *first;
    DevEvent *sorted;
    const uint32_t *counters;
    const uint8_t *bursts; uint32_t burst_cap;
    void *hot, *cold;
    uint64_t *wake_sample;
    DevMessage *near; uint32_t near_cap;
    DevMessage *log; uint32_t log_cap;
    uint32_t *log_cursor, *overflow;
    cap::Launch cap;
};
size_t transport_hot_bytes();
size_t transport_cold_bytes();
hipError_t launch_transport(const TransportLaunch &T, hipStream_t stream);
hipError_t launch_transport_ragged(const TransportLaunch &T, const uint32_t *counts, uint32_t row_sub, uint32_t n_rows, hipStream_t stream);
hipError_t launch_transport_reset(void *hot, void *cold, uint32_t n_channels, const uint32_t *cols, uint32_t n, int fresh,
                                  hipStream_t stream, void *capture_rec = nullptr);
hipError_t launch_capture(const cap::Span *spans, cap::Cursors *cur, uint32_t span_cap, float *pool, uint64_t pool_cap,
                          const float *x, uint32_t n_channels, uint32_t n_rows, cap::Cursors *host, hipStream_t stream);
hipError_t launch_capture(const cap::Span *spans, cap::Cursors *cur, uint32_t span_cap, float *pool, uint64_t pool_cap,
                          const int16_t *x, uint32_t n_channels, uint32_t n_rows, cap::Cursors *host, hipStream_t stream);

struct SynthParams {
    uint32_t n_channels;
    uint32_t input_rate;
    uint64_t seed;
    float noise_sigma;
    uint32_t flags;
};
hipError_t launch_synth(const SynthParams &sp, float *x, size_t n_samples, hipStream_t stream);
struct TrialParams {
    uint32_t n_trials;
    uint32_t first_trial;
    uint32_t input_rate;
    uint32_t n_grid;
    uint64_t seed;
    float ebn0_db_lo, ebn0_db_step;
};
hipError_t launch_trials(const TrialParams &tp, float *x, size_t n_samples, hipStream_t stream);
uint32_t synth_payload(uint64_t seed, uint32_t channel, uint8_t *out, uint32_t cap);

}
```

sameold_amd/csrc/same_pipe_common.h:

```cpp
#pragma once

#include <hip/hip_runtime.h>

#include "same_dev_common.h"
#include "same_device.h"

namespace same {

typedef volatile __attribute__((address_space(3))) uint32_t lds_u32;

__device__ __forceinline__ void lds_barrier()
{
    asm volatile("s_waitcnt lgkmcnt(0)\n\ts_barrier" ::: "memory");
}

__device__ __forceinline__ uint32_t burst_to_pool(const State &S, const Output &O, uint32_t c)
{
    const uint32_t b = atomicAdd(O.n_events + 1, 1u);
    if (b >= O.burst_cap) { atomicOr(O.n_events + 2, 2u); return 0xffffffffu; }
    copy_burst_row(O.bursts + (size_t)b * kBurstCap, S.fr_msg + (size_t)c * kBurstCap);
    return b;
}

constexpr uint32_t kEvChunk = 64;
struct IoCtx : TickRingGlobal {
    lds_u32 *chunk;
    uint32_t pending_slot;
    __device__ __forceinline__ void mark(int) const {}
    __device__ __forceinline__ void emit(const Params &P, const State &S, const Output &O, uint32_t c, uint32_t kind,
                                         uint64_t sample_counter, uint64_t symbols, uint32_t burst_len)
    {
        const uint64_t act = __builtin_amdgcn_ballot_w64(true);
        const uint32_t n = (uint32_t)__popcll(act);
        const uint32_t rank = __builtin_amdgcn_mbcnt_hi((uint32_t)(act >> 32), __builtin_amdgcn_mbcnt_lo((uint32_t)act, 0u));
        uint32_t base = chunk[0], used = chunk[1];
        if (used + n > kEvChunk) {
            for (uint32_t i = used + rank; i < kEvChunk; i += n)
                if (base + i < O.event_cap) { O.events[base + i].channel = 0; O.events[base + i].kind = kDevEventNone; }
            uint32_t nb = 0;
            if (rank == 0u) nb = atomicAdd(O.n_events, kEvChunk);
            base = (uint32_t)__builtin_amdgcn_readfirstlane((int)nb);
            used = 0;
        }
        const uint32_t e = base + used + rank;
        chunk[0] = base; chunk[1] = used + n;
        if (e < O.event_cap) {
            DevEvent ev;
            ev.channel = c; ev.kind = kind; ev.sample_counter = sample_counter;
            ev.symbol_count = symbols; ev.burst_len = burst_len;
            ev.burst_slot = kind == 3u ? pending_slot : 0xffffffffu;
            O.events[e] = ev;
        } else {
            atomicOr(O.n_events + 2, 1u);
        }
    }
    __device__ __forceinline__ void retire(const Output &O, uint32_t lane, uint32_t lanes)
    {
        const uint32_t base = chunk[0], used = chunk[1];
        for (uint32_t i = used + lane; i < kEvChunk; i += lanes)
            if (base + i < O.event_cap) { O.events[base + i].channel = 0; O.events[base + i].kind = kDevEventNone; }
    }
};

constexpr uint32_t kIoRingWords = (2u * (uint32_t)kTickRing + 1u) * kWave;
struct IoCtxLds : IoCtx {
    lds_u32 *tk;
    __device__ __forceinline__ uint32_t tk_count(const State &, uint32_t) const { return tk[2 * kTickRing * kWave]; }
    __device__ __forceinline__ void tk_set_count(const State &, uint32_t, uint32_t n) const { tk[2 * kTickRing * kWave] = n; }
    __device__ __forceinline__ uint64_t tk_at(const State &, uint32_t, uint32_t, uint32_t i) const
    {
        return (uint64_t)tk[2u * i * kWave] | ((uint64_t)tk[(2u * i + 1u) * kWave] << 32);
    }
    __device__ __forceinline__ void tk_set(const State &, uint32_t, uint32_t, uint32_t i, uint64_t v) const
    {
        tk[2u * i * kWave] = (uint32_t)v; tk[(2u * i + 1u) * kWave] = (uint32_t)(v >> 32);
    }
    __device__ __forceinline__ void ring_load(const Params &P, const State &S, uint32_t c)
    {
        if (!P.ticks) return;
        const TickRingGlobal G;
#pragma unroll
        for (uint32_t i = 0; i < (uint32_t)kTickRing; ++i) tk_set(S, P.n_channels, c, i, G.tk_at(S, P.n_channels, c, i));
        tk_set_count(S, c, G.tk_count(S, c));
    }
    __device__ __forceinline__ void ring_store(const Params &P, const State &S, uint32_t c) const
    {
        if (!P.ticks) return;
        const TickRingGlobal G;
#pragma unroll
        for (uint32_t i = 0; i < (uint32_t)kTickRing; ++i) G.tk_set(S, P.n_channels, c, i, tk_at(S, P.n_channels, c, i));
        G.tk_set_count(S, c, tk_count(S, c));
    }
};

}
```

Baseline: 463,300.

## Read time-parallel start state in place instead of copying into wide blob

```diff
diff --git a/sameold_amd/csrc/same_batch.cpp b/sameold_amd/csrc/same_batch.cpp
--- a/sameold_amd/csrc/same_batch.cpp
+++ b/sameold_amd/csrc/same_batch.cpp
@@ -251,6 +251,10 @@
         same::DevBuf<void> blob;
         same::DevBuf<void> blob_fresh;
         size_t fresh_bytes = 0;
+        bool fresh_full = false;
+        same::DevBuf<void> blob_fresh64;
+        same::StartStates start{};
+        int knob_start_copies = 0;
         same::DevBuf<same::StateArrayDesc> d_desc_in, d_desc_out;
         uint32_t n_desc = 0;
         same::DevBuf<uint32_t> d_final_col;
@@ -423,6 +427,7 @@
     rx->tp.sort_mode = num("SAME_TP_SORT", -1);
     rx->tp.knob_plan_stream = tri("SAME_TP_PLAN_STREAM");
     rx->tp.knob_prologue = tri("SAME_TP_PROLOGUE");
+    rx->tp.knob_start_copies = tri("SAME_TP_START_COPIES");
     rx->want.knob_relaxed = tri("SAME_RELAXED");
     { const char *e = std::getenv("SAME_RELAXED_KERNEL"); rx->P.knob_relaxed_kernel = !e ? 0 : (std::strcmp(e, "solo") == 0 ? 1 : (std::strcmp(e, "duo") == 0 ? 2 : 0)); }
     { const char *e = std::getenv("SAME_TP_KERNEL"); rx->want.knob_tp_kernel = !e ? 0 : (std::strcmp(e, "wave") == 0 ? 2 : (std::strcmp(e, "pipe") == 0 ? 1 : 0)); }
@@ -456,10 +461,11 @@
 
 template <typename SampleT>
 hipError_t launch_family(same::Family f, const same::Params &P, const same::State &S, const same::Output &O, const float4 *taps, const SampleT *x,
-                         uint32_t n_blocks, uint64_t counter0, hipStream_t stream, const same::PipeChunks &pc = same::PipeChunks{})
+                         uint32_t n_blocks, uint64_t counter0, hipStream_t stream, const same::PipeChunks &pc = same::PipeChunks{},
+                         const same::StartStates *start = nullptr)
 {
     switch (f) {
-    case same::Family::kSym: return same::launch_demod_sym(P, S, O, taps, x, n_blocks, counter0, stream, pc);
+    case same::Family::kSym: return same::launch_demod_sym(P, S, O, taps, x, n_blocks, counter0, stream, pc, start);
     case same::Family::kPipeFastmath: return same::launch_demod_pipe(P, S, O, taps, x, n_blocks, counter0, stream, pc, true);
     case same::Family::kPipe: return same::launch_demod_pipe(P, S, O, taps, x, n_blocks, counter0, stream, pc, false);
     case same::Family::kWaveRelaxed: return same::launch_demod_relaxed(P, S, O, taps, x, n_blocks, counter0, stream, pc);
@@ -1112,17 +1118,20 @@
         const size_t bytes = carve_state(tp.Pv, nullptr, tp.Sv);
         HIP_TRY(tp.blob.ensure(bytes));
         HIP_TRY(hipMemset(tp.blob, 0, bytes));
-        HIP_TRY(tp.blob_fresh.ensure(bytes));
         tp.cap_columns = columns;
     }
-    const size_t blob_bytes = carve_state(tp.Pv, (char *)tp.blob.get(), tp.Sv);
+    carve_state(tp.Pv, (char *)tp.blob.get(), tp.Sv);
+    tp.fresh_full = false;
     {
-        same::State Sf{};
-        carve_state(tp.Pv, (char *)tp.blob_fresh.get(), Sf);
-        HIP_TRY(hipMemset(tp.blob_fresh, 0, blob_bytes));
-        HIP_TRY(same::launch_init_state(tp.Pv, Sf, 0, nullptr, 0));
+        same::Params P64 = tp.Pv;
+        P64.n_channels = (uint32_t)same::kWave;
+        const size_t bytes64 = carve_state(P64, nullptr, tp.start.fresh);
+        HIP_TRY(tp.blob_fresh64.ensure(bytes64));
+        carve_state(P64, (char *)tp.blob_fresh64.get(), tp.start.fresh);
+        HIP_TRY(hipMemset(tp.blob_fresh64, 0, bytes64));
+        HIP_TRY(same::launch_init_state(P64, tp.start.fresh, 0, nullptr, 0));
         HIP_TRY(hipDeviceSynchronize());
-        tp.fresh_bytes = (size_t)(reinterpret_cast<char *>(tp.Sv.fr_msg) - static_cast<char *>(tp.blob.get()));
+        tp.start.own = rx->S;
     }
     std::vector<same::StateArrayDesc> in, out;
     list_state_arrays(rx->P, rx->S, tp.Sv, in);
@@ -1138,6 +1147,29 @@
     return SAME_OK;
 }
 
+int ensure_full_template(same_batch *rx)
+{
+    same_batch::TimePar &tp = rx->tp;
+    if (tp.fresh_full) return SAME_OK;
+    HIP_TRY(hipDeviceSynchronize());
+    same::State Sf{};
+    const size_t bytes = carve_state(tp.Pv, nullptr, Sf);
+    HIP_TRY(tp.blob_fresh.ensure(bytes));
+    carve_state(tp.Pv, (char *)tp.blob_fresh.get(), Sf);
+    HIP_TRY(hipMemset(tp.blob_fresh, 0, bytes));
+    HIP_TRY(same::launch_init_state(tp.Pv, Sf, 0, nullptr, 0));
+    HIP_TRY(hipDeviceSynchronize());
+    tp.fresh_bytes = (size_t)(reinterpret_cast<char *>(tp.Sv.fr_msg) - static_cast<char *>(tp.blob.get()));
+    tp.fresh_full = true;
+    return SAME_OK;
+}
+
+bool tp_direct_start(const same_batch *rx, bool permuted)
+{
+    const same_batch::TimePar &tp = rx->tp;
+    return tp.family == same::Family::kSym && !permuted && tp.knob_prologue >= 0 && tp.knob_start_copies <= 0;
+}
+
 struct Ragged {
     const uint32_t *counts = nullptr;
     uint32_t m = 0;
@@ -1174,12 +1206,21 @@
     return ensure_handover(sl, columns);
 }
 
-int tp_start(same_batch *rx, same_batch::Slot &sl, uint32_t columns, const char *layout, hipStream_t stream, bool *sort_bins_empty)
+int tp_start(same_batch *rx, same_batch::Slot &sl, uint32_t columns, const char *layout, hipStream_t stream, bool *sort_bins_empty, bool direct)
 {
     same_batch::TimePar &tp = rx->tp;
     const uint32_t C = rx->P.n_channels;
     *sort_bins_empty = false;
+    if (direct) {
+        tp.start.own = rx->S;
+        HIP_TRY(same::launch_tp_prologue(tp.blob, nullptr, 0, sl.d_handover, sl.d_sort, columns, sl.d_counters, stream));
+        *sort_bins_empty = sl.sort_bins == columns;
+        if (rx->debug) std::fprintf(stderr, "[same] time-parallel launch: %u columns (%s), start-up: prologue kernel, start state read in place\n", columns, layout);
+        return SAME_OK;
+    }
     if (tp.knob_prologue >= 0) {
+        const int rc = ensure_full_template(rx);
+        if (rc) return rc;
         HIP_TRY(same::launch_tp_prologue(tp.blob, tp.blob_fresh, tp.fresh_bytes, sl.d_handover, sl.d_sort, columns, sl.d_counters, stream));
         *sort_bins_empty = sl.sort_bins == columns;
     } else {
@@ -1310,11 +1351,13 @@
             same_batch::TimePar &tp = rx->tp;
             rc = begin_timing(rx, sl, stream);
             if (rc) return rc;
-            rc = tp_start(rx, sl, columns, "time-major", stream, &sort_bins_empty);
+            const bool direct = tp_direct_start(rx, false);
+            rc = tp_start(rx, sl, columns, "time-major", stream, &sort_bins_empty, direct);
             if (rc) return rc;
+            pc.start_direct = direct ? 1u : 0u;
             const SampleT *xp = d_x + done * C;
             const uint32_t total_blocks = (uint32_t)(n / fbk);
-            const hipError_t e = launch_family(tp.family, tp.Pv, tp.Sv, O, rx->d_taps, xp, total_blocks, rx->counter, stream, pc);
+            const hipError_t e = launch_family(tp.family, tp.Pv, tp.Sv, O, rx->d_taps, xp, total_blocks, rx->counter, stream, pc, &tp.start);
             rx->last_family = tp.family;
             if (e != hipSuccess) return fail(SAME_EHIP, "time-parallel demod kernel launch failed: %s", hipGetErrorString(e));
             rc = tp_hand_back(rx, sl, geom, nullptr, stream);
@@ -1516,8 +1559,10 @@
     }
     if (lpt) { d_perm = d_perm2; d_wg = d_wg2; }
     bool sort_bins_empty = false;
-    rc = tp_start(rx, sl, columns, "channel-major", stream, &sort_bins_empty);
+    const bool direct = tp_direct_start(rx, sort_mode != 0 || pair_groups);
+    rc = tp_start(rx, sl, columns, "channel-major", stream, &sort_bins_empty, direct);
     if (rc) return rc;
+    pc.start_direct = direct ? 1u : 0u;
     pc.handover = sl.d_handover;
     pc.col_row0 = d_row0; pc.col_nominal = d_nom; pc.wg_blocks = d_wg; pc.col_perm = (sort_mode != 0 || pair_groups) ? d_perm : nullptr;
     pc.in_samples = n_call; pc.whole_samples = (uint32_t)n;
@@ -1528,7 +1573,7 @@
     }
     sl.have_k = sl.timed;
     if (sl.timed) HIP_TRY(hipEventRecord(sl.ev_k0, stream));
-    const hipError_t e = launch_family(tp.family, tp.Pv, tp.Sv, O, rx->d_taps, d_x, (uint32_t)(n / fb), rx->counter, stream, pc);
+    const hipError_t e = launch_family(tp.family, tp.Pv, tp.Sv, O, rx->d_taps, d_x, (uint32_t)(n / fb), rx->counter, stream, pc, &tp.start);
     rx->last_family = tp.family;
     if (e != hipSuccess) return fail(SAME_EHIP, "time-parallel demod kernel launch failed: %s", hipGetErrorString(e));
     if (sl.timed) HIP_TRY(hipEventRecord(sl.ev_k1, stream));
diff --git a/sameold_amd/csrc/same_device.h b/sameold_amd/csrc/same_device.h
--- a/sameold_amd/csrc/same_device.h
+++ b/sameold_amd/csrc/same_device.h
@@ -108,6 +108,12 @@
     float *hist_scratch;
     uint64_t in_samples;
     uint32_t whole_samples;
+    uint32_t start_direct;
+};
+
+struct StartStates {
+    State own;
+    State fresh;
 };
 
 struct ChunkGeom {
diff --git a/sameold_amd/csrc/same_kernels_sym.hip b/sameold_amd/csrc/same_kernels_sym.hip
--- a/sameold_amd/csrc/same_kernels_sym.hip
+++ b/sameold_amd/csrc/same_kernels_sym.hip
@@ -881,7 +881,7 @@
     return fmaxf(floorf(s - 0.5f) + 1.0f, 1.0f);
 }
 
-struct SymKernArgs { Params P; State S; Output O; const float4 *taps; const void *x; uint32_t n_blocks; uint64_t counter0; PipeChunks K; };
+struct SymKernArgs { Params P; State S; Output O; const float4 *taps; const void *x; uint32_t n_blocks; uint64_t counter0; PipeChunks K; StartStates SS; };
 typedef const __attribute__((address_space(4))) char *sym_kernarg_ptr;
 template <typename T> __device__ __forceinline__ T sym_fresh_arg(sym_kernarg_ptr ka, size_t off)
 {
@@ -896,11 +896,12 @@
 template <int NT, int NFF, int NFB, typename SampleT, int CMODE>
 __global__ __launch_bounds__(SymGeom<NT>::HALVES * kSymRoles * kWave, NT == 42 ? 3 : 2) void demod_sym_kernel(Params P, State S_arg_, Output O_arg_, const float4 *__restrict__ taps,
                                                                          const SampleT *__restrict__ x, uint32_t n_blocks, uint64_t counter0,
-                                                                         PipeChunks K)
+                                                                         PipeChunks K, StartStates SS_arg_)
 {
-    (void)S_arg_; (void)O_arg_;
+    (void)S_arg_; (void)O_arg_; (void)SS_arg_;
     const sym_kernarg_ptr ka = (sym_kernarg_ptr)__builtin_amdgcn_kernarg_segment_ptr();
     auto fresh_state = [&]() __attribute__((always_inline)) -> State { return sym_fresh_arg<State>(ka, offsetof(SymKernArgs, S)); };
+#define SYM_WIDE_PTR(field_) sym_fresh_arg<decltype(State::field_)>(ka, offsetof(SymKernArgs, S) + offsetof(State, field_))
     auto fresh_output = [&]() __attribute__((always_inline)) -> Output { return sym_fresh_arg<Output>(ka, offsetof(SymKernArgs, O)); };
     using LY = SymLayout<NT>;
     constexpr int kB = LY::B, RING = LY::RING, kSB = LY::SB, kNSUB = LY::NSUB;
@@ -934,12 +935,14 @@
     int32_t row_l = 0;
     const SampleT *xl = nullptr;
     uint32_t avail_l = 0;
+    uint32_t piece = 0;
     if (K.n_chunks > 1u) {
         Cin = K.in_channels;
         if (K.col_row0) {
             const uint32_t chunk_l = c / Cin;
             cin = c - chunk_l * Cin;
-            may_leave = (uint32_t)__builtin_amdgcn_readfirstlane((int)chunk_l) + 1u < K.n_chunks;
+            piece = (uint32_t)__builtin_amdgcn_readfirstlane((int)chunk_l);
+            may_leave = piece + 1u < K.n_chunks;
             const uint32_t row_abs = K.col_row0[c];
             xl = x + (size_t)cin * K.in_samples + row_abs;
             avail_l = (K.whole_samples - row_abs) / (uint32_t)kSB;
@@ -952,6 +955,7 @@
             const uint32_t wgs = K.in_channels / kWave;
             const uint32_t chunk = (uint32_t)__builtin_amdgcn_readfirstlane((int)(vwg / wgs));
             cin = (vwg - chunk * wgs) * kWave + lane;
+            piece = chunk;
             may_leave = chunk + 1u < K.n_chunks;
             const uint32_t first_block = chunk * K.stride_blocks;
             x += (size_t)first_block * kB * Cin;
@@ -960,6 +964,17 @@
             n_nominal = may_leave ? K.nominal_blocks : n_blocks;
         }
     }
+    enum : uint32_t { kStartWide = 0u, kStartOwn = 1u, kStartFresh = 2u };
+    uint32_t start_src = (K.n_chunks > 1u && K.start_direct != 0u && K.col_perm == nullptr) ? (piece == 0u ? kStartOwn : kStartFresh) : kStartWide;
+    start_src = (uint32_t)__builtin_amdgcn_readfirstlane((int)start_src);
+    asm volatile("" : "+s"(start_src));
+    auto start_state = [&]() __attribute__((always_inline)) -> State {
+        const uint32_t off = start_src == kStartWide ? (uint32_t)offsetof(SymKernArgs, S)
+                           : (uint32_t)offsetof(SymKernArgs, SS) + (start_src == kStartOwn ? (uint32_t)offsetof(StartStates, own) : (uint32_t)offsetof(StartStates, fresh));
+        return sym_fresh_arg<State>(ka, off);
+    };
+    auto start_col = [&]() __attribute__((always_inline)) -> uint32_t { return start_src == kStartFresh ? lane : c; };
+    auto start_pitch = [&]() __attribute__((always_inline)) -> uint32_t { return start_src == kStartWide ? C : (start_src == kStartOwn ? K.in_channels : (uint32_t)kWave); };
     lds_u32 *mail = (lds_u32 *)(lds + LY::tap_floats);
     lds_u32 *symbox = mail;
     lds_u32 *ybox = symbox + 2u * LY::sym_words;
@@ -1030,7 +1045,7 @@
     if (role == 0u) {
         sym_setprio<sym_prio<NT>(0)>(P);
         SymAgc<NT> M;
-        { const State S = fresh_state(); M.load(P, S, c, C, counter0, wcol); }
+        { const State S = start_state(); M.load(P, S, start_col(), start_pitch(), counter0, wcol); }
         lds_barrier();
         P3_T0();
         uint32_t stop_at = 0xffffffffu;
@@ -1075,7 +1090,7 @@
             static_assert(CMODE == 0 && kNSUB == 2, "time-major rows, two sub-blocks a step");
             SymDcRot<SampleT, NT> D;
             const uint32_t n_sub = n_blocks * (uint32_t)kNSUB;
-            { const State S = fresh_state(); D.load(S, x, c, C, cin, Cin, counter0, n_sub); }
+            { const State S = start_state(); D.load(S, x, start_col(), start_pitch(), cin, Cin, counter0, n_sub); }
             donebox[lane] = 0u;
             D.template sub<0>(P, wcol, x, 0u, n_sub, cin, Cin);
             D.template sub<1>(P, wcol, x, 1u, n_sub, cin, Cin);
@@ -1118,7 +1133,7 @@
         Dc D;
         D.xl = xl; D.avail = avail_l;
         const uint32_t n_sub = n_blocks * (uint32_t)kNSUB;
-        { const State S = fresh_state(); D.load(S, x, c, C, cin, Cin, counter0, n_sub); }
+        { const State S = start_state(); D.load(S, x, start_col(), start_pitch(), cin, Cin, counter0, n_sub); }
         donebox[lane] = 0u;
         auto sub_tm = [&](uint32_t q, auto pb_) __attribute__((always_inline)) {
             typename Dc::Pairs X;
@@ -1192,9 +1207,19 @@
         X.pending_slot = 0xffffffffu;
         X.tk = tkbox + lane;
         {
-            const State S = fresh_state();
-            lane_load(L, S, c);
-            X.ring_load(P, S, c);
+            const State S = start_state();
+            const uint32_t cs = start_col(), Cs = start_pitch();
+            lane_load(L, S, cs);
+            X.ring_load(P, S, Cs, cs);
+            if (start_src != kStartWide) {
+                SYM_WIDE_PTR(wake_sample)[c] = L.wake_sample;
+                if (!P.ticks) {
+                    SYM_WIDE_PTR(tk_n)[c] = S.tk_n[cs];
+                    uint64_t *const ring = SYM_WIDE_PTR(tk_ring);
+#pragma unroll
+                    for (uint32_t i = 0; i < (uint32_t)kTickRing; ++i) ring[i * C + c] = S.tk_ring[i * Cs + cs];
+                }
+            }
         }
         const State Snone{};
         Output O{};
@@ -1271,7 +1296,7 @@
         std::conditional_t<NT == 42, SymTaps<42>, SymHalfTaps<NT, NT / 4, NT / 2>> TP;
         TP.load(taps);
         Lane L;
-        { const State S = fresh_state(); lane_load(L, S, c); }
+        { const State S = start_state(); lane_load(L, S, start_col()); }
         const float inv_spt = 1.0f / P.samples_per_ted;
         int cstar = next_fire_count(L.until_next_ted, L.ted_clock);
         int rel = cstar - (int)L.ted_clock - 1;
@@ -1429,29 +1454,30 @@
         uint64_t symbols0;
         const bool hist_copy = K.n_chunks > 1u && K.col_perm != nullptr && K.hist_scratch != nullptr;
         {
-            const State S = fresh_state();
-            lane_load(Q.L, S, c);
+            const State S = start_state();
+            const uint32_t cs = start_col(), Cs = start_pitch();
+            lane_load(Q.L, S, cs);
             symbols0 = Q.L.sq_symbols;
             Q.nsym = (uint32_t)symbols0;
-            Q.hbase = reinterpret_cast<char *>(hist_copy ? K.hist_scratch : S.sq_hist);
+            Q.hbase = reinterpret_cast<char *>(hist_copy ? K.hist_scratch : SYM_WIDE_PTR(sq_hist));
             Q.hcol4 = (hist_copy ? vwg * kWave + lane : c) * 4u;
             Q.hrow4 = C * 4u;
-            if (hist_copy) {
+            if (hist_copy || start_src != kStartWide) {
 #pragma unroll 4
-                for (int i = 0; i < kSquelchHist; ++i) *Q.hptr((uint32_t)i) = S.sq_hist[(size_t)i * C + c];
+                for (int i = 0; i < kSquelchHist; ++i) *Q.hptr((uint32_t)i) = S.sq_hist[(size_t)i * Cs + cs];
             }
 #pragma unroll
             for (int i = 0; i < NFF; ++i) {
-                Q.ffc[i] = S.eq_ffc[i * C + c]; Q.ffw[i] = S.eq_ffw[i * C + c];
-                Q.sffc[i] = S.eq_snap_ffc[i * C + c]; Q.sffw[i] = S.eq_snap_ffw[i * C + c];
+                Q.ffc[i] = S.eq_ffc[i * Cs + cs]; Q.ffw[i] = S.eq_ffw[i * Cs + cs];
+                Q.sffc[i] = S.eq_snap_ffc[i * Cs + cs]; Q.sffw[i] = S.eq_snap_ffw[i * Cs + cs];
             }
 #pragma unroll
             for (int i = 0; i < NFB; ++i) {
-                Q.fbc[i] = S.eq_fbc[i * C + c]; Q.fbw[i] = S.eq_fbw[i * C + c];
-                Q.sfbc[i] = S.eq_snap_fbc[i * C + c]; Q.sfbw[i] = S.eq_snap_fbw[i * C + c];
+                Q.fbc[i] = S.eq_fbc[i * Cs + cs]; Q.fbw[i] = S.eq_fbw[i * Cs + cs];
+                Q.sfbc[i] = S.eq_snap_fbc[i * Cs + cs]; Q.sfbw[i] = S.eq_snap_fbw[i * Cs + cs];
             }
             const uint32_t pslot = (2u * Q.nsym) & 63u;
-            Q.nxt0 = *Q.hptr((pslot + 16u) & 63u); Q.nxt1 = *Q.hptr((pslot + 17u) & 63u);
+            Q.nxt0 = S.sq_hist[(size_t)((pslot + 16u) & 63u) * Cs + cs]; Q.nxt1 = S.sq_hist[(size_t)((pslot + 17u) & 63u) * Cs + cs];
         }
         lds_barrier();
         P3_T0();
@@ -1560,7 +1586,21 @@
         Lane L;
         SymFramer F;
         uint8_t *fr_rows;
-        { const State S0 = fresh_state(); lane_load(L, S0, c); fr_rows = S0.fr_msg; }
+        {
+            const State S0 = start_state();
+            lane_load(L, S0, start_col());
+            fr_rows = SYM_WIDE_PTR(fr_msg);
+            if (start_src == kStartOwn) {
+                const uint4 *src = reinterpret_cast<const uint4 *>(S0.fr_msg + (size_t)c * kBurstCap);
+                uint4 *dst = reinterpret_cast<uint4 *>(fr_rows + (size_t)c * kBurstCap);
+                static_assert(kBurstCap % 48 == 0, "three 16-byte words at a time");
+                sym_static_for<kBurstCap / 48>([&](auto g_) __attribute__((always_inline)) {
+                    constexpr int g = decltype(g_)::value;
+                    const uint4 t0 = src[3 * g], t1 = src[3 * g + 1], t2 = src[3 * g + 2];
+                    dst[3 * g] = t0; dst[3 * g + 1] = t1; dst[3 * g + 2] = t2;
+                });
+            }
+        }
         F.st = fr_state(L); F.last = (L.flags & F_LINK_MASK) >> F_LINK_SHIFT;
         F.word = L.fr_word; F.count = L.fr_count; F.invalid = L.fr_invalid; F.len = L.fr_len;
         uint8_t *const row = fr_rows + (size_t)c * kBurstCap;
@@ -1658,8 +1698,10 @@
 
 template <int NT, int NFF, int NFB, typename SampleT>
 static hipError_t launch_sym_one(const Params &P, const State &S, const Output &O, const float4 *taps, const SampleT *x,
-                                 uint32_t n_blocks, uint64_t counter0, hipStream_t stream, const PipeChunks &K)
+                                 uint32_t n_blocks, uint64_t counter0, hipStream_t stream, const PipeChunks &K, const StartStates *start)
 {
+    if (K.n_chunks > 1u && K.start_direct != 0u && (start == nullptr || K.col_perm != nullptr)) return hipErrorInvalidValue;
+    const StartStates SS = start ? *start : StartStates{};
     constexpr uint32_t kSymHalves = (uint32_t)SymLayout<NT>::HALVES;
     constexpr size_t lds = (size_t)kSymHalves * SymLayout<NT>::lds_bytes;
     static_assert(lds <= 160u * 1024u, "one workgroup per CU");
@@ -1681,7 +1723,7 @@
                 opted_in.insert(key);
             }
         }
-        hipLaunchKernelGGL(kernel, dim3((P.n_channels / kWave + kSymHalves - 1u) / kSymHalves), dim3(kSymHalves * kSymRoles * kWave), lds, stream, P, S, O, taps, x, n_blocks, counter0, K);
+        hipLaunchKernelGGL(kernel, dim3((P.n_channels / kWave + kSymHalves - 1u) / kSymHalves), dim3(kSymHalves * kSymRoles * kWave), lds, stream, P, S, O, taps, x, n_blocks, counter0, K, SS);
         return hipGetLastError();
     };
     if constexpr (std::is_same<SampleT, float>::value && NT == 42) {
@@ -1692,51 +1734,53 @@
 
 template <typename SampleT>
 static hipError_t launch_sym_hi_t(const Params &P, const State &S, const Output &O, const float4 *taps, const SampleT *x,
-                                  uint32_t n_blocks, uint64_t counter0, hipStream_t stream, const PipeChunks &K)
+                                  uint32_t n_blocks, uint64_t counter0, hipStream_t stream, const PipeChunks &K, const StartStates *start)
 {
     const bool eq = P.eq_nff == 6u && P.eq_nfb == 4u;
     if (standard_rate_taps(P) == 92u)
-        return eq ? launch_sym_one<92, 6, 4, SampleT>(P, S, O, taps, x, n_blocks, counter0, stream, K) : launch_sym_one<92, 1, 1, SampleT>(P, S, O, taps, x, n_blocks, counter0, stream, K);
-    return eq ? launch_sym_one<84, 6, 4, SampleT>(P, S, O, taps, x, n_blocks, counter0, stream, K) : launch_sym_one<84, 1, 1, SampleT>(P, S, O, taps, x, n_blocks, counter0, stream, K);
+        return eq ? launch_sym_one<92, 6, 4, SampleT>(P, S, O, taps, x, n_blocks, counter0, stream, K, start) : launch_sym_one<92, 1, 1, SampleT>(P, S, O, taps, x, n_blocks, counter0, stream, K, start);
+    return eq ? launch_sym_one<84, 6, 4, SampleT>(P, S, O, taps, x, n_blocks, counter0, stream, K, start) : launch_sym_one<84, 1, 1, SampleT>(P, S, O, taps, x, n_blocks, counter0, stream, K, start);
 }
 #if defined(SYM_TU_HI)
 #if defined(SYM_SPLIT_TU)
 hipError_t launch_demod_sym_hi(const Params &P, const State &S, const Output &O, const float4 *taps, const float *x,
-                               uint32_t n_blocks, uint64_t counter0, hipStream_t stream, const PipeChunks &K)
-{ return launch_sym_hi_t<float>(P, S, O, taps, x, n_blocks, counter0, stream, K); }
+                               uint32_t n_blocks, uint64_t counter0, hipStream_t stream, const PipeChunks &K, const StartStates *start)
+{ return launch_sym_hi_t<float>(P, S, O, taps, x, n_blocks, counter0, stream, K, start); }
 hipError_t launch_demod_sym_hi(const Params &P, const State &S, const Output &O, const float4 *taps, const int16_t *x,
-                               uint32_t n_blocks, uint64_t counter0, hipStream_t stream, const PipeChunks &K)
-{ return launch_sym_hi_t<int16_t>(P, S, O, taps, x, n_blocks, counter0, stream, K); }
+                               uint32_t n_blocks, uint64_t counter0, hipStream_t stream, const PipeChunks &K, const StartStates *start)
+{ return launch_sym_hi_t<int16_t>(P, S, O, taps, x, n_blocks, counter0, stream, K, start); }
 #endif
 #else
 #if defined(SYM_SPLIT_TU)
 hipError_t launch_demod_sym_hi(const Params &P, const State &S, const Output &O, const float4 *taps, const float *x,
-                               uint32_t n_blocks, uint64_t counter0, hipStream_t stream, const PipeChunks &K);
+                               uint32_t n_blocks, uint64_t counter0, hipStream_t stream, const PipeChunks &K, const StartStates *start);
 hipError_t launch_demod_sym_hi(const Params &P, const State &S, const Output &O, const float4 *taps, const int16_t *x,
-                               uint32_t n_blocks, uint64_t counter0, hipStream_t stream, const PipeChunks &K);
+                               uint32_t n_blocks, uint64_t counter0, hipStream_t stream, const PipeChunks &K, const StartStates *start);
 #else
 template <typename SampleT>
 static hipError_t launch_demod_sym_hi(const Params &P, const State &S, const Output &O, const float4 *taps, const SampleT *x,
-                                      uint32_t n_blocks, uint64_t counter0, hipStream_t stream, const PipeChunks &K)
-{ return launch_sym_hi_t<SampleT>(P, S, O, taps, x, n_blocks, counter0, stream, K); }
+                                      uint32_t n_blocks, uint64_t counter0, hipStream_t stream, const PipeChunks &K, const StartStates *start)
+{ return launch_sym_hi_t<SampleT>(P, S, O, taps, x, n_blocks, counter0, stream, K, start); }
 #endif
 template <typename SampleT>
 static hipError_t launch_sym_t(const Params &P, const State &S, const Output &O, const float4 *taps, const SampleT *x,
-                               uint32_t n_blocks, uint64_t counter0, hipStream_t stream, const PipeChunks &K)
+                               uint32_t n_blocks, uint64_t counter0, hipStream_t stream, const PipeChunks &K, const StartStates *start)
 {
     if (!sym_kernel_supported(P)) return hipErrorInvalidValue;
     const bool eq = P.eq_nff == 6u && P.eq_nfb == 4u;
     if (standard_rate_taps(P) == 42u)
-        return eq ? launch_sym_one<42, 6, 4, SampleT>(P, S, O, taps, x, n_blocks, counter0, stream, K) : launch_sym_one<42, 1, 1, SampleT>(P, S, O, taps, x, n_blocks, counter0, stream, K);
-    return launch_demod_sym_hi(P, S, O, taps, x, n_blocks, counter0, stream, K);
+        return eq ? launch_sym_one<42, 6, 4, SampleT>(P, S, O, taps, x, n_blocks, counter0, stream, K, start) : launch_sym_one<42, 1, 1, SampleT>(P, S, O, taps, x, n_blocks, counter0, stream, K, start);
+    return launch_demod_sym_hi(P, S, O, taps, x, n_blocks, counter0, stream, K, start);
 }
 hipError_t launch_demod_sym(const Params &P, const State &S, const Output &O, const float4 *taps, const float *x,
-                            uint32_t n_blocks, uint64_t counter0, hipStream_t stream, const PipeChunks &K)
-{ return launch_sym_t<float>(P, S, O, taps, x, n_blocks, counter0, stream, K); }
+                            uint32_t n_blocks, uint64_t counter0, hipStream_t stream, const PipeChunks &K, const StartStates *start)
+{ return launch_sym_t<float>(P, S, O, taps, x, n_blocks, counter0, stream, K, start); }
 hipError_t launch_demod_sym(const Params &P, const State &S, const Output &O, const float4 *taps, const int16_t *x,
-                            uint32_t n_blocks, uint64_t counter0, hipStream_t stream, const PipeChunks &K)
-{ return launch_sym_t<int16_t>(P, S, O, taps, x, n_blocks, counter0, stream, K); }
+                            uint32_t n_blocks, uint64_t counter0, hipStream_t stream, const PipeChunks &K, const StartStates *start)
+{ return launch_sym_t<int16_t>(P, S, O, taps, x, n_blocks, counter0, stream, K, start); }
 #endif
+
+#undef SYM_WIDE_PTR
 
 }
 
diff --git a/sameold_amd/csrc/same_launch.h b/sameold_amd/csrc/same_launch.h
--- a/sameold_amd/csrc/same_launch.h
+++ b/sameold_amd/csrc/same_launch.h
@@ -24,10 +24,10 @@
                              const PipeChunks &chunks = PipeChunks{}, bool relaxed = false);
 hipError_t launch_demod_sym(const Params &P, const State &S, const Output &O, const float4 *taps,
                             const float *x, uint32_t n_blocks, uint64_t counter0, hipStream_t stream,
-                            const PipeChunks &chunks = PipeChunks{});
+                            const PipeChunks &chunks = PipeChunks{}, const StartStates *start = nullptr);
 hipError_t launch_demod_sym(const Params &P, const State &S, const Output &O, const float4 *taps,
                             const int16_t *x, uint32_t n_blocks, uint64_t counter0, hipStream_t stream,
-                            const PipeChunks &chunks = PipeChunks{});
+                            const PipeChunks &chunks = PipeChunks{}, const StartStates *start = nullptr);
 hipError_t launch_demod_relaxed(const Params &P, const State &S, const Output &O, const float4 *taps,
                                 const float *x, uint32_t n_blocks, uint64_t counter0, hipStream_t stream,
                                 const PipeChunks &chunks = PipeChunks{});
diff --git a/sameold_amd/csrc/same_pipe_common.h b/sameold_amd/csrc/same_pipe_common.h
--- a/sameold_amd/csrc/same_pipe_common.h
+++ b/sameold_amd/csrc/same_pipe_common.h
@@ -75,14 +75,15 @@
     {
         tk[2u * i * kWave] = (uint32_t)v; tk[(2u * i + 1u) * kWave] = (uint32_t)(v >> 32);
     }
-    __device__ __forceinline__ void ring_load(const Params &P, const State &S, uint32_t c)
+    __device__ __forceinline__ void ring_load(const Params &P, const State &S, uint32_t C, uint32_t c)
     {
         if (!P.ticks) return;
         const TickRingGlobal G;
 #pragma unroll
-        for (uint32_t i = 0; i < (uint32_t)kTickRing; ++i) tk_set(S, P.n_channels, c, i, G.tk_at(S, P.n_channels, c, i));
+        for (uint32_t i = 0; i < (uint32_t)kTickRing; ++i) tk_set(S, C, c, i, G.tk_at(S, C, c, i));
         tk_set_count(S, c, G.tk_count(S, c));
     }
+    __device__ __forceinline__ void ring_load(const Params &P, const State &S, uint32_t c) { ring_load(P, S, P.n_channels, c); }
     __device__ __forceinline__ void ring_store(const Params &P, const State &S, uint32_t c) const
     {
         if (!P.ticks) return;
```

Result: no change. 461,200 (-0.4%).
